# SafeRL-Lab/Massive-MARL-Benchmark

Measured on AMD Instinct MI355X. Metric: env-steps/sec (whole node), TenAnt 4096 envs/GPU, PPO rollout, higher is better.
Workload: dtype f32 (policy-layer products: fp32 operands as 2 row-scaled fp16 planes (kept to 2^-22), 3 f16 MFMA products, fp32 accumulation; error vs float64 <= the exact-fp32 MFMA kernel's, see policy_layers_error_vs_f64); 1 GPU; TenAnt num_envs=4096 per GPU, PPO rollout: ActorCritic MLP [1024,1024,512]x2 (fp32) + fused sim step (dt 0.0166, 2 substeps) + RolloutStorage + GAE every 8 steps; envs_per_gpu=4096, global_envs=4096, parallelism=env-sharded x1, no data-path collective, hipgraph=True, refresh_in_graph=True, rollouts_per_graph=1, fused_act_and_bound_slots=True, obs_planes_from_step_kernel=True, policy_head_in_step_kernel=True, critic_stream=True, critic_deferred=False, finite=True, resets_total=97569

## Files before the change

include/mms.h:

```cpp
#ifndef MMS_H
#define MMS_H

#include <stdint.h>

#ifdef __cplusplus
extern "C" {
#endif

#define MMS_ABI_VERSION 4
#define MMS_DR_FLOATS 33

enum mms_task { MMS_TASK_TEN_ANT = 0, MMS_TASK_ONE_ANT = 1, MMS_TASK_MULTI_INGENUITY = 2,
                MMS_TASK_MULTI_ANT_CIRCLE = 3 };
enum mms_dtype { MMS_F32 = 0, MMS_I64 = 1, MMS_I32 = 2, MMS_U8 = 3 };

typedef struct mms_model {
    float torso_mass, torso_ixx, torso_izz, torso_radius;
    float leg_mass, leg_ia, leg_it;
    float foot_mass, foot_ia, foot_it;
    float limb_radius, leg_len, foot_len;
    float hip_pos[4][3];
    float limb_dir[4][3];
    float ankle_axis[4][3];
    float dof_lower[8], dof_upper[8], dof_init[8], gear[8];
// ... 25 lines not shown
    float dt;
    float clip_actions, clip_obs;
    float dof_vel_scale, contact_force_scale, power_scale;
    float heading_weight, up_weight, actions_cost, energy_cost, joints_at_limit_cost;
    float death_cost, termination_height;
    float quat_reward_scale, ant_dist_reward_scale, goal_dist_reward_scale;
    float ant_start_x, ant_start_z;
    float box_start[3];
    mms_model model;
} mms_config;

typedef struct mms_tensor {
    void*   ptr;
    int64_t shape[4];
    int32_t ndim;
    int32_t dtype;
    int32_t device;
    int32_t reserved;
} mms_tensor;

typedef struct mms_engine* mms_handle;

int mms_create(const mms_config* cfg, mms_handle* out);
int mms_destroy(mms_handle h);

int mms_get_tensor(mms_handle h, const char* name, mms_tensor* out);

int mms_step(mms_handle h, void* hip_stream);

int mms_post_step(mms_handle h, void* hip_stream);

int mms_reset_all(mms_handle h, void* hip_stream);

int mms_set_state(mms_handle h, const char* name, const void* src, int src_is_host,
                  const int64_t* env_ids, int64_t n, void* hip_stream);

int mms_bind_obs_out(mms_handle h, void* dst);

int mms_bind_obs_planes16(mms_handle h, void* planes, float scale);

int mms_bind_actions(mms_handle h, const float* src);

int mms_set_dr(mms_handle h, int32_t enable);

int mms_set_obs_outputs(mms_handle h, int32_t raw, int32_t clipped);

int mms_bind_rollout_out(mms_handle h, float* rew_out, uint8_t* done_out);

int mms_marl_views(int device, const float* obs_clipped, float* obs_all, int64_t n, int32_t agents,
                   int32_t per_agent, int32_t shared, void* hip_stream);

int mms_gae_ppo(int device, const float* rewards, const uint8_t* dones, const float* values,
                const float* last_values, float* returns, float* advantages, double* stats,
                int32_t T, int64_t N, float gamma, float lam, void* hip_stream);
int mms_adv_normalize(int device, float* advantages, const double* stats, int64_t count, void* hip_stream);
#define MMS_GAE_STATS_DOUBLES (3 + 2 * 2048)
int mms_gae_ppo_normalized(int device, const float* rewards, const uint8_t* dones, const float* values, const float* last_values,
                           float* returns, float* advantages, double* stats, int32_t T, int64_t N, float gamma, float lam,
                           void* hip_stream);

int mms_layer_clock_probe(int device, uint64_t* out, int32_t slots);

int mms_gae_marl(int device, const float* rewards, const float* value_preds, const float* masks,
                 float* returns, int32_t T, int64_t N, float gamma, float lam,
                 int32_t use_norm, const float* norm_mean, const float* norm_var, void* hip_stream);

int mms_gae_marl_agents(int device, const float* rewards, const float* value_preds, const float* masks,
                        float* returns, int32_t T, int64_t N, int32_t A, float gamma, float lam,
                        int32_t use_norm, const float* norm_mean, const float* norm_var, void* hip_stream);

int mms_ppo_act(int device, const float* mean, const float* value, const float* log_std, uint64_t seed, int64_t* counters,
                int64_t row_offset, int32_t reference_scale, float* actions_out, float* act_slot, float* logp_slot,
                float* value_slot, float* mu_slot, float* sigma_slot, int64_t N, int32_t A, void* hip_stream);

int mms_ppo_heads_act(int device, const float* hidden, const float* weight, const float* bias, int32_t H, const float* value,
                      const float* vhidden, const float* vweight, const float* vbias, int32_t VH, const float* log_std, uint64_t seed,
                      int64_t* counters, int64_t row_offset, int32_t reference_scale, float* actions_out, float* act_slot,
                      float* logp_slot, float* value_slot, float* mu_slot, float* sigma_slot, int64_t N, int32_t A, void* hip_stream);

typedef struct mms_policy_head {
    const float* hidden; const float* weight; const float* bias;
    const float* vhidden; const float* vweight; const float* vbias;
    const float* log_std;
    int64_t* counters;
    float* actions_out; float* act_slot; float* logp_slot; float* value_slot; float* mu_slot; float* sigma_slot;
    uint64_t seed;
    int64_t row_offset;
    int32_t H, VH, A, reference_scale;
    const float* weight_tiles;
} mms_policy_head;
int mms_bind_policy_head(mms_handle h, const mms_policy_head* head);

int mms_sac_heads_act(int device, const float* hidden, int32_t H,
                      const float* mu_weight, const float* mu_bias, const float* ls_weight, const float* ls_bias,
                      float act_limit, float epsilon, int32_t deterministic,
                      uint64_t seed, int64_t* counters, int64_t row_offset,
                      float* actions_out, float* act_slot, float* logp_slot,
                      float* u_slot, float* mu_slot, float* log_std_slot,
                      int64_t N, int32_t A, void* hip_stream);

#define MMS_Q_MAX_H 4096
int mms_q_heads_backup(int device, int64_t M, int32_t H,
                       const float* h0, const float* w0, const float* b0, float* q0_out,
                       const float* h1, const float* w1, const float* b1, float* q1_out,
                       const float* reward, const uint8_t* done, const float* logp, float gamma, float alpha,
                       float* backup, void* hip_stream);

int mms_linear2_act(int device, int64_t M, int32_t N, int32_t K, const float* x0, const float* w0, const float* b0, float* y0,
                    const float* x1, const float* w1, const float* b1, float* y1, int32_t act, void* hip_stream);

#define MMS_MAX_GROUPS 32

int mms_linear_group_act(int device, int32_t groups, int64_t M, int32_t N, int32_t K, const float* const* x, const float* const* w,
                         const float* const* b, float* const* y, int32_t act, const float* const* ln_s, const float* const* ln_stat_in,
                         float* const* ln_part_out, void* hip_stream);

int mms_row_stats_group(int device, int32_t groups, int64_t M, int32_t slots, int32_t width, const float* const* part, float* const* stat,
                        float eps, void* hip_stream);

int mms_row_moments_group(int device, int32_t groups, int64_t M, int32_t K, int32_t x_pitch, const float* const* x, float* const* stat,
                          float eps, void* hip_stream);

int mms_layernorm_group(int device, int32_t groups, int64_t M, int32_t K, int32_t Kp, int32_t x_pitch, const float* const* x,
                        const float* const* gamma, const float* const* beta, float* const* y, float eps, void* hip_stream);

int mms_marl_heads_act(int device, int32_t groups, int64_t M, int32_t H, const float* const* h, const float* const* gamma,
                       const float* const* beta, const float* const* w, const float* const* b, const int32_t* A, const float* const* std,
                       float* const* out, float* const* logp, const int32_t* out_pitch, int64_t* const* counters, uint64_t seed,
                       int64_t row_offset, float eps, void* hip_stream);

#define MMS_P32_BYTES(rows, K) ((size_t)(rows) * (size_t)(((K) + 31) / 32) * 192)

int mms_split_planes(int device, int64_t rows, int32_t K, int32_t x_pitch, const float* x, void* planes, void* hip_stream);

int mms_split_planes_group(int device, int32_t groups, int64_t rows, int32_t K, int32_t x_pitch, const float* const* x, void* const* planes,
                           void* hip_stream);

int mms_linear_group_act_split(int device, int32_t groups, int64_t M, int32_t N, int32_t K, const void* const* x, const void* const* w,
                               const float* const* b, void* const* y, int32_t act, int32_t out_mode, const float* const* ln_s,
                               const float* const* ln_stat_in, float* const* ln_part_out, const float* const* head_w, float* const* head_part,
                               const int32_t* head_dims, void* hip_stream);

#define MMS_H32_BYTES(rows, K) ((size_t)(rows) * (size_t)(((K) + 31) / 32) * 128)

int mms_split_planes16_group(int device, int32_t groups, int64_t rows, int32_t K, int32_t x_pitch, const float* const* x, void* const* planes,
                             float* const* scale, float* const* inv, int32_t nchains, int32_t L, const float* const* chain,
                             float* const* chain_scale, float* const* chain_inv, float* const* stat, float eps, void* hip_stream);

int mms_weight_planes16_group(int device, int32_t groups, const int64_t* N, const int32_t* K, const float* const* w, void* const* planes,
                              float* const* scale, float* const* inv, float* const* l1, void* hip_stream);
int mms_chain_refresh16(int device, int32_t nchains, int32_t L, const float* const* l1, const float* const* bias, const int32_t* n,
                        float* chain, float bound0, int64_t rows, float* chain_scale, float* chain_inv, void* hip_stream);

int mms_linear_group_act_split16(int device, int32_t groups, int64_t M, int32_t N, int32_t K, const void* const* x, const void* const* w,
                                 const float* const* b, void* const* y, const float* const* x_inv, const float* const* w_inv,
                                 const float* const* y_scale, int32_t act, int32_t out_mode, const float* const* ln_s,
                                 const float* const* ln_stat_in, float* const* ln_part_out, const float* const* head_w, float* const* head_part,
                                 const int32_t* head_dims, void* hip_stream);

int mms_fold_planes16_group(int device, int32_t groups, const int64_t* N, const int32_t* K, const float* const* w, const float* const* gamma,
                            const float* const* beta, const float* const* bias, void* const* planes, float* const* inv, float* const* s,
                            float* const* c, float* const* rb, float* const* wt, void* hip_stream);
int mms_fold_scales16_group(int device, int32_t groups, const float* const* rb, const int32_t* n, int64_t M, float* const* scale1,
                            float* const* ysc, float* const* yinv, void* hip_stream);

int mms_row_stats_chan_group(int device, int32_t groups, int64_t M, int32_t slots, const float* const* part, float* const* stat, float eps,
                             void* hip_stream);

int mms_marl_heads_finish(int device, int32_t groups, int64_t M, int32_t slots, const float* const* part, const float* const* head_part,
                          const float* const* hs, const float* const* hc, const int32_t* A, const float* const* std, float* const* out,
                          float* const* logp, const int32_t* out_pitch, int64_t* const* counters, uint64_t seed, int64_t row_offset, float eps,
                          void* hip_stream);

int mms_mlp_grad(int device, int32_t layers, int64_t M, const int32_t* dims, const float* x, const float* const* h, const float* const* w,
                 const float* g, float* const* dw, float* const* db, float* const* d_out, float* const* e_out, void* workspace,
                 int64_t* ws_bytes, void* hip_stream);

int mms_mlp_grad_rop(int device, int32_t layers, int64_t M, const int32_t* dims, const float* x, const float* const* h, const float* const* w,
                     const float* const* v, const float* const* c, const float* g, const float* const* d, const float* const* e, float* rmu,
                     float* const* rdw, float* const* rdb, void* workspace, int64_t* ws_bytes, void* hip_stream);

const char* mms_last_error(mms_handle h);
int mms_abi_version(void);

#ifdef __cplusplus
}
#endif
#endif
```

massive_marl_benchmark_amd/_lib.py:

```python
import ctypes
import os

from .model import MmsConfig, MmsTensor

_HERE = os.path.dirname(os.path.abspath(__file__))
LIB_PATH = os.environ.get("MMS_LIB", os.path.join(_HERE, "lib", "libmms.so"))
LIB_CPU_PATH = os.path.join(_HERE, "lib", "libmms_cpu.so")
_lib = None
_lib_cpu = None

SYMBOLS = ["mms_create", "mms_destroy", "mms_get_tensor", "mms_step", "mms_post_step", "mms_reset_all", "mms_set_state",
           "mms_bind_obs_out", "mms_bind_obs_planes16", "mms_bind_actions", "mms_bind_policy_head", "mms_set_dr", "mms_set_obs_outputs", "mms_bind_rollout_out", "mms_ppo_act", "mms_ppo_heads_act", "mms_sac_heads_act", "mms_q_heads_backup", "mms_linear2_act", "mms_linear_group_act", "mms_split_planes", "mms_split_planes_group", "mms_linear_group_act_split", "mms_split_planes16_group", "mms_weight_planes16_group", "mms_chain_refresh16", "mms_fold_planes16_group", "mms_fold_scales16_group", "mms_linear_group_act_split16", "mms_row_stats_chan_group", "mms_marl_heads_finish", "mms_row_stats_group", "mms_row_moments_group", "mms_layernorm_group", "mms_marl_heads_act", "mms_marl_views", "mms_gae_ppo", "mms_adv_normalize", "mms_gae_ppo_normalized", "mms_layer_clock_probe", "mms_gae_marl", "mms_gae_marl_agents", "mms_mlp_grad", "mms_mlp_grad_rop",
           "mms_last_error", "mms_abi_version"]


class MmsError(RuntimeError):
    pass


def _bind(path):
    L = ctypes.CDLL(path)
    vp, ci, c64, cf = ctypes.c_void_p, ctypes.c_int, ctypes.c_int64, ctypes.c_float
    L.mms_create.argtypes = [ctypes.POINTER(MmsConfig), ctypes.POINTER(vp)]
    L.mms_destroy.argtypes = [vp]
    L.mms_get_tensor.argtypes = [vp, ctypes.c_char_p, ctypes.POINTER(MmsTensor)]
    L.mms_step.argtypes = [vp, vp]
    L.mms_post_step.argtypes = [vp, vp]
    L.mms_reset_all.argtypes = [vp, vp]
    L.mms_set_state.argtypes = [vp, ctypes.c_char_p, vp, ci, ctypes.POINTER(c64), c64, vp]
    L.mms_bind_obs_out.argtypes = [vp, vp]
    L.mms_bind_actions.argtypes = [vp, vp]
    L.mms_bind_policy_head.argtypes = [vp, vp]
    L.mms_bind_obs_planes16.argtypes = [vp, vp, cf]
    L.mms_set_obs_outputs.argtypes = [vp, ctypes.c_int32, ctypes.c_int32]
    L.mms_set_dr.argtypes = [vp, ctypes.c_int32]
    L.mms_bind_rollout_out.argtypes = [vp, vp, vp]
    L.mms_ppo_act.argtypes = [ci, vp, vp, vp, ctypes.c_uint64, vp, c64, ctypes.c_int32, vp, vp, vp, vp, vp, vp, c64, ctypes.c_int32, vp]
    L.mms_ppo_heads_act.argtypes = [ci, vp, vp, vp, ctypes.c_int32, vp, vp, vp, vp, ctypes.c_int32, vp, ctypes.c_uint64, vp, c64, ctypes.c_int32, vp, vp, vp, vp,
                                    vp, vp, c64, ctypes.c_int32, vp]
    L.mms_sac_heads_act.argtypes = [ci, vp, ctypes.c_int32, vp, vp, vp, vp, cf, cf, ctypes.c_int32, ctypes.c_uint64, vp, c64, vp, vp, vp, vp, vp, vp,
                                    c64, ctypes.c_int32, vp]
    L.mms_q_heads_backup.argtypes = [ci, c64, ctypes.c_int32, vp, vp, vp, vp, vp, vp, vp, vp, vp, vp, vp, cf, cf, vp, vp]
    L.mms_linear2_act.argtypes = [ci, c64, ctypes.c_int32, ctypes.c_int32, vp, vp, vp, vp, vp, vp, vp, vp, ctypes.c_int32, vp]
    L.mms_linear_group_act.argtypes = [ci, ctypes.c_int32, c64, ctypes.c_int32, ctypes.c_int32, vp, vp, vp, vp, ctypes.c_int32, vp, vp, vp, vp]
    L.mms_split_planes.argtypes = [ci, c64, ctypes.c_int32, ctypes.c_int32, vp, vp, vp]
    L.mms_split_planes_group.argtypes = [ci, ctypes.c_int32, c64, ctypes.c_int32, ctypes.c_int32, vp, vp, vp]
    L.mms_linear_group_act_split.argtypes = [ci, ctypes.c_int32, c64, ctypes.c_int32, ctypes.c_int32, vp, vp, vp, vp, ctypes.c_int32, ctypes.c_int32,
                                             vp, vp, vp, vp, vp, vp, vp]
    L.mms_split_planes16_group.argtypes = [ci, ctypes.c_int32, c64, ctypes.c_int32, ctypes.c_int32, vp, vp, vp, vp, ctypes.c_int32, ctypes.c_int32, vp, vp, vp, vp, cf, vp]
    L.mms_weight_planes16_group.argtypes = [ci, ctypes.c_int32, vp, vp, vp, vp, vp, vp, vp, vp]
    L.mms_fold_planes16_group.argtypes = [ci, ctypes.c_int32, vp, vp, vp, vp, vp, vp, vp, vp, vp, vp, vp, vp, vp]
    L.mms_fold_scales16_group.argtypes = [ci, ctypes.c_int32, vp, vp, c64, vp, vp, vp, vp]
    L.mms_chain_refresh16.argtypes = [ci, ctypes.c_int32, ctypes.c_int32, vp, vp, vp, vp, cf, c64, vp, vp, vp]
    L.mms_linear_group_act_split16.argtypes = [ci, ctypes.c_int32, c64, ctypes.c_int32, ctypes.c_int32, vp, vp, vp, vp, vp, vp, vp, ctypes.c_int32, ctypes.c_int32,
                                               vp, vp, vp, vp, vp, vp, vp]
    L.mms_row_stats_chan_group.argtypes = [ci, ctypes.c_int32, c64, ctypes.c_int32, vp, vp, cf, vp]
    L.mms_marl_heads_finish.argtypes = [ci, ctypes.c_int32, c64, ctypes.c_int32, vp, vp, vp, vp, vp, vp, vp, vp, vp, vp, ctypes.c_uint64, c64, cf, vp]
    L.mms_row_moments_group.argtypes = [ci, ctypes.c_int32, c64, ctypes.c_int32, ctypes.c_int32, vp, vp, cf, vp]
    L.mms_row_stats_group.argtypes = [ci, ctypes.c_int32, c64, ctypes.c_int32, ctypes.c_int32, vp, vp, cf, vp]
    L.mms_layernorm_group.argtypes = [ci, ctypes.c_int32, c64, ctypes.c_int32, ctypes.c_int32, ctypes.c_int32, vp, vp, vp, vp, cf, vp]
    L.mms_marl_heads_act.argtypes = [ci, ctypes.c_int32, c64, ctypes.c_int32, vp, vp, vp, vp, vp, vp, vp, vp, vp, vp, vp, ctypes.c_uint64, c64, cf, vp]
    L.mms_marl_views.argtypes = [ci, vp, vp, c64, ctypes.c_int32, ctypes.c_int32, ctypes.c_int32, vp]
    L.mms_gae_ppo.argtypes = [ci, vp, vp, vp, vp, vp, vp, vp, ctypes.c_int32, c64, cf, cf, vp]
    L.mms_adv_normalize.argtypes = [ci, vp, vp, c64, vp]
    L.mms_gae_ppo_normalized.argtypes = [ci, vp, vp, vp, vp, vp, vp, vp, ctypes.c_int32, c64, cf, cf, vp]
    L.mms_layer_clock_probe.argtypes = [ci, vp, ctypes.c_int32]
    L.mms_gae_marl.argtypes = [ci, vp, vp, vp, vp, ctypes.c_int32, c64, cf, cf, ctypes.c_int32, vp, vp, vp]
    L.mms_gae_marl_agents.argtypes = [ci, vp, vp, vp, vp, ctypes.c_int32, c64, ctypes.c_int32, cf, cf, ctypes.c_int32, vp, vp, vp]
    L.mms_mlp_grad.argtypes = [ci, ctypes.c_int32, c64, vp, vp, vp, vp, vp, vp, vp, vp, vp, vp, ctypes.POINTER(c64), vp]
    L.mms_mlp_grad_rop.argtypes = [ci, ctypes.c_int32, c64, vp, vp, vp, vp, vp, vp, vp, vp, vp, vp, vp, vp, vp, ctypes.POINTER(c64), vp]
    L.mms_last_error.argtypes = [vp]
    L.mms_last_error.restype = ctypes.c_char_p
    L.mms_abi_version.restype = ci
    return L


def lib():
    global _lib
    if _lib is not None:
        return _lib
    if not os.path.exists(LIB_PATH):
        raise MmsError("HIP engine library not built: %s is missing (run `python -c 'import __graft_entry__ as g; g.build()'` "
                       "or `make -C massive_marl_benchmark_amd/csrc`). There is no CPU fallback." % LIB_PATH)
    _lib = _bind(LIB_PATH)
    return _lib


def lib_cpu():
    global _lib_cpu
    if _lib_cpu is not None:
        return _lib_cpu
    if not os.path.exists(LIB_CPU_PATH):
        raise MmsError("CPU engine library not built: %s is missing (make -C massive_marl_benchmark_amd/csrc)" % LIB_CPU_PATH)
    _lib_cpu = _bind(LIB_CPU_PATH)
    return _lib_cpu


def for_device(device):
    import torch
    dev = torch.device(device)
    if dev.type == "cpu":
        return lib_cpu(), -1, None
    if dev.type != "cuda":
        raise MmsError("unsupported device %r" % (device,))
    idx = dev.index if dev.index is not None else torch.cuda.current_device()
    return lib(), idx, ctypes.c_void_p(torch.cuda.current_stream(dev).cuda_stream)


def last_error(handle=None, L=None):
    msg = (L or lib()).mms_last_error(handle)
    return msg.decode() if msg else ""


def check(rc, handle=None, what="", L=None):
    if rc != 0:
        raise MmsError("%s failed: %s" % (what, last_error(handle, L)))
```

massive_marl_benchmark_amd/algorithms/rl/ppo/module.py:

```python
import ctypes
import math

import numpy as np
import torch
import torch.nn as nn

from .... import _lib


def get_activation(act_name):
    table = {"elu": nn.ELU, "selu": nn.SELU, "relu": nn.ReLU, "crelu": nn.ReLU, "lrelu": nn.LeakyReLU, "tanh": nn.Tanh,
             "sigmoid": nn.Sigmoid}
    if act_name not in table:
        print("invalid activation function!")
        return None
    return table[act_name]()


def _mlp(in_dim, hidden, out_dim, activation):
    layers, d = [], in_dim
    for h in hidden:
        layers += [nn.Linear(d, h), activation]
        d = h
    layers.append(nn.Linear(d, out_dim))
    return nn.Sequential(*layers)


class ActorCritic(nn.Module):
    def __init__(self, obs_shape, states_shape, actions_shape, initial_std, model_cfg, asymmetric=False, seed=0, row_offset=0):
        super().__init__()
        self.asymmetric = asymmetric
        if model_cfg is None:
            actor_hidden, critic_hidden, activation = [256, 256, 256], [256, 256, 256], get_activation("selu")
        else:
            actor_hidden, critic_hidden = model_cfg["pi_hid_sizes"], model_cfg["vf_hid_sizes"]
            activation = get_activation(model_cfg["activation"])
        self.actor = _mlp(obs_shape[0], actor_hidden, actions_shape[0], activation)
        self.critic = _mlp(states_shape[0] if asymmetric else obs_shape[0], critic_hidden, 1, activation)
        self.log_std = nn.Parameter(np.log(initial_std) * torch.ones(*actions_shape))
        self.init_weights(self.actor, [np.sqrt(2)] * len(actor_hidden) + [0.01])
        self.init_weights(self.critic, [np.sqrt(2)] * len(critic_hidden) + [1.0])
        self.seed, self.row_offset = int(seed), int(row_offset)
        self._counters = None
        self._bound = None
        self._side = None
        self._trunk = None
        self._act_bufs = None
        self._value_bufs = None
        self._one_bufs = None
        self._wplanes = None
        self._split_bufs = None
        self._nets = None
        self._h16 = None
        self._addr_tag = None
        self._ver_tag = None
        self._calls = None
        self._sample_calls = None
        self._qualify = None
        self._step_engine = None
        self._head_wt = None

    _DERIVED = ("_counters", "_side", "_trunk", "_act_bufs", "_value_bufs", "_one_bufs", "_wplanes", "_split_bufs", "_nets", "_h16", "_addr_tag",
                "_ver_tag", "_calls", "_sample_calls", "_qualify", "_bound", "_step_engine", "_head_wt")

    def __deepcopy__(self, memo):
        import copy
        new = self.__class__.__new__(self.__class__)
        memo[id(self)] = new
        for k, v in self.__dict__.items():
            new.__dict__[k] = None if k in self._DERIVED else copy.deepcopy(v, memo)
        return new

    @staticmethod
    def init_weights(sequential, scales):
        for idx, module in enumerate(m for m in sequential if isinstance(m, nn.Linear)):
            torch.nn.init.orthogonal_(module.weight, gain=scales[idx])

    fuse_layers = True
    split_layers = True
    split_min_tiles = None
    split_format = "f16x2"
    fuse_head = True
    two_streams = True
    defer_value = False

    def forward(self):
        raise NotImplementedError

    def bind_rollout(self, storage=None, actions_out=None, step_engine=None):
        self._bound = (storage, actions_out)
        self._step_engine = step_engine if (storage is not None and step_engine is not None and step_engine.takes_policy_head()) else None

    def _fp32_layers_qualify(self):
        dt = self.log_std.dtype
        if self._qualify is not None and self._qualify[0] == dt:
            return self._qualify[1]
        a_lin = [m for m in self.actor if isinstance(m, nn.Linear)]
        c_lin = [m for m in self.critic if isinstance(m, nn.Linear)]
        acts = [m for m in list(self.actor) + list(self.critic) if not isinstance(m, nn.Linear)]
        ok = (len(a_lin) == len(c_lin) and len(a_lin) >= 2 and all(isinstance(m, nn.ELU) and m.alpha == 1.0 for m in acts)
              and all(la.weight.shape == lc.weight.shape and la.weight.dtype == torch.float32 and la.in_features % 4 == 0
                      and la.bias is not None and lc.bias is not None for la, lc in zip(a_lin[:-1], c_lin[:-1])))
        self._qualify = (dt, ok)
        return ok

    @staticmethod
    def _p32_bytes(rows, K):
        return rows * ((K + 31) // 32) * 192

    def _weight_planes(self, lin, L, idx, stream, force=False):
        if self._wplanes is None:
            self._wplanes = {}
        w = lin.weight.detach()
        tag = (w._version, w.data_ptr(), str(w.device))
        hit = self._wplanes.get(id(lin))
        if force or hit is None or hit[0] != tag:
            planes = hit[1] if hit is not None and hit[1].device == w.device else \
                torch.empty(self._p32_bytes(lin.out_features, lin.in_features), dtype=torch.uint8, device=w.device)
            wc = w.contiguous()
            _lib.check(L.mms_split_planes(idx, lin.out_features, lin.in_features, 0, ctypes.c_void_p(wc.data_ptr()),
                                          ctypes.c_void_p(planes.data_ptr()), stream), None, "mms_split_planes", L)
            self._wplanes[id(lin)] = (tag, planes, lin)
            return planes
        return hit[1]

    @staticmethod
    def _h32_bytes(rows, K):
        return rows * ((K + 31) // 32) * 128

    def _networks(self):
        if self._nets is None:
            self._nets = [[m for m in net if isinstance(m, nn.Linear)][:-1] for net in (self.actor, self.critic)]
        return self._nets

    def _param_tags(self):
        ps = [q for net in self._networks() for l in net for q in (l.weight, l.bias) if q is not None]
        ps += [q for q in (self.actor[-1].weight, self.actor[-1].bias, self.critic[-1].weight, self.critic[-1].bias, self.log_std) if q is not None]
        return tuple(q._version for q in ps), tuple(q.data_ptr() for q in ps)

    def _h16_state(self, dev):
        st = self._h16
        if st is not None and st["dev"] == dev:
            return st
        L, idx, _ = _lib.for_device(dev)
        nets = self._networks()
        recs, off, slices = [], 0, []
        for net in nets:
            rs = []
            for l in net:
                assert l.weight.dtype == torch.float32 and l.weight.is_contiguous() and l.bias is not None and l.weight.device == dev
                N, K = l.out_features, l.in_features
                rs.append({"lin": l, "N": N, "K": K, "planes": torch.empty(self._h32_bytes(N, K), dtype=torch.uint8, device=dev),
                           "scale": torch.empty(N, device=dev), "inv": torch.empty(N, device=dev), "l1": torch.empty(N, device=dev)})
            recs.append(rs)
            slices.append((off, max(len(net) - 1, 0)))
            off += 2 * max(len(net) - 1, 0)
        bounds = torch.zeros(max(off, 2), device=dev)
        arr = lambda ts: (ctypes.c_void_p * len(ts))(*[t.data_ptr() for t in ts])
        flat = [r for rs in recs for r in rs]
        calls = []
        if flat:
            calls.append((L.mms_weight_planes16_group, (idx, len(flat), (ctypes.c_int64 * len(flat))(*[r["N"] for r in flat]),
                                                        (ctypes.c_int32 * len(flat))(*[r["K"] for r in flat]), arr([r["lin"].weight for r in flat]),
                                                        arr([r["planes"] for r in flat]), arr([r["scale"] for r in flat]), arr([r["inv"] for r in flat]),
                                                        arr([r["l1"] for r in flat])), "mms_weight_planes16_group"))
        st = {"dev": dev, "L": L, "idx": idx, "recs": recs, "bounds": bounds, "slices": slices, "calls": calls, "given": {}, "chain_args": {}}
        self._h16 = st
        return st

    def _chain_args(self, st, members):
        members = tuple(members)
        hit = st["chain_args"].get(members)
        if hit is None:
            chain, Lh = self._chain(st, list(members))
            ent = [st["recs"][g][li] for g in members for li in range(Lh)]
            arr = lambda ts: (ctypes.c_void_p * len(ts))(*[t.data_ptr() for t in ts])
            hit = (len(members), Lh, arr([r["l1"] for r in ent]), arr([r["lin"].bias for r in ent]), (ctypes.c_int32 * len(ent))(*[r["N"] for r in ent]),
                   ctypes.c_void_p(chain.data_ptr())) if Lh else None
            st["chain_args"][members] = hit
        return hit

    def _chain(self, st, members):
        o0, Lh = st["slices"][members[0]]
        if Lh == 0:
            return None, 0
        for j, g in enumerate(members):
            assert st["slices"][g] == (o0 + 2 * Lh * j, Lh), "networks that share an input must be adjacent and equally deep"
        return st["bounds"][o0: o0 + 2 * Lh * len(members)], Lh

    def refresh(self):
        dev = self.log_std.device
        vers, addrs = self._param_tags()
        if self._addr_tag is not None and self._addr_tag != (addrs, str(dev)):
            self._h16, self._wplanes, self._split_bufs, self._calls, self._sample_calls = None, None, None, None, None
            self._head_wt = None
        self._addr_tag, self._ver_tag = (addrs, str(dev)), vers
        if self._head_wt is not None:
            self._fill_head_tiles()
        st = self._h16
        if st is not None:
            stream = _lib.for_device(st["dev"])[2]
            for fn, args, what in st["calls"]:
                _lib.check(fn(*args, stream), None, what, st["L"])
            covered = set()
            for (members, rows, scale), (_, cs, ci, alias) in st["given"].items():
                ca = self._chain_args(st, members)
                if ca is None or alias:
                    continue
                _lib.check(st["L"].mms_chain_refresh16(st["idx"], *ca, 16384.0 / scale, rows, ctypes.c_void_p(cs.data_ptr()), ctypes.c_void_p(ci.data_ptr()), stream),
                           None, "mms_chain_refresh16", st["L"])
                covered.update(members)
            depths = {Lh for _, Lh in st["slices"]}
            rest = [tuple(range(len(st["recs"])))] if len(depths) == 1 else [(g,) for g in range(len(st["recs"]))]
            for grp in rest:
                if not set(grp) <= covered:
                    ca = self._chain_args(st, grp)
                    if ca is not None:
                        _lib.check(st["L"].mms_chain_refresh16(st["idx"], *ca, 0.0, 0, None, None, stream), None, "mms_chain_refresh16", st["L"])
        if self._wplanes:
            for key in list(self._wplanes):
                tag, planes, lin = self._wplanes[key]
                if self.split_format == "bf16x3":
                    self._weight_planes(lin, *_lib.for_device(lin.weight.device), force=True)
                else:
                    self._wplanes[key] = (None, planes, lin)

    def _head_tiles(self):
        if self._head_wt is None:
            last = self.actor[-1]
            A, H = last.out_features, last.in_features
            nct = (A + 15) // 16
            pad = torch.zeros(nct * 16, H, device=last.weight.device, dtype=torch.float32)
            tiles = torch.empty(nct * (H // 4) * 64, device=last.weight.device, dtype=torch.float32)
            self._head_wt = (pad, tiles)
            self._fill_head_tiles()
        return self._head_wt[1]

    def _fill_head_tiles(self):
        pad, tiles = self._head_wt
        last = self.actor[-1]
        A, H = last.out_features, last.in_features
        with torch.no_grad():
            if A % 16 == 0:
                tiles.view(-1, H // 4, 16, 4).copy_(last.weight.detach().view(-1, 16, H // 4, 4).permute(0, 2, 1, 3))
            else:
                pad[:A].copy_(last.weight.detach())
                tiles.view(-1, H // 4, 16, 4).copy_(pad.view(-1, 16, H // 4, 4).permute(0, 2, 1, 3))

    def _ensure_fresh(self):
        storage = self._bound[0] if self._bound is not None else None
        if storage is not None and storage.step == 0:
            return self.refresh()
        vers, addrs = self._param_tags()
        if self._ver_tag != vers or self._addr_tag != (addrs, str(self.log_std.device)):
            self.refresh()

    def _split_hidden16(self, nets, inputs, tag, planes=None):
        self._ensure_fresh()
        x0 = inputs[0]
        dev, M = x0.device, x0.shape[0]
        mine = self._networks()
        members = [next(j for j, n in enumerate(mine) if n and n[0] is net[0]) for net in nets]
        fresh = self._h16 is None or self._h16["dev"] != dev
        st = self._h16_state(dev)
        if fresh:
            self.refresh()
        G, nl = len(nets), len(nets[0])
        given = planes is not None and all(x.data_ptr() == x0.data_ptr() and x.shape == x0.shape for x in inputs)
        ckey = (tag, "h", M, tuple((x.data_ptr(), x.shape[1], x.stride(0)) for x in inputs), tuple(members),
                (planes[0].data_ptr(), float(planes[1])) if given else None)
        if self._calls is None:
            self._calls = {}
        hit = self._calls.get(ckey)
        if hit is None:
            hit = self._build_calls16(st, members, inputs, tag, planes if given else None)
            self._calls[ckey] = hit
        calls, out = hit
        stream = _lib.for_device(dev)[2]
        for fn, args, what in calls:
            _lib.check(fn(*args, stream), None, what, st["L"])
        return out

    def _build_calls16(self, st, members, inputs, tag, planes):
        x0 = inputs[0]
        dev, M = x0.device, x0.shape[0]
        L, idx = st["L"], st["idx"]
        recs = [st["recs"][g] for g in members]
        G, nl = len(recs), len(recs[0])
        key = (tag, "h", M, tuple(x.shape[1] for x in inputs), str(dev), tuple(members))
        if self._split_bufs is None:
            self._split_bufs = {}
        bufs = self._split_bufs.get(key)
        f32 = lambda *sh: torch.empty(*sh, device=dev)
        u8 = lambda n: torch.empty(n, dtype=torch.uint8, device=dev)
        if bufs is None:
            bufs = {"x": [u8(self._h32_bytes(M, x.shape[1])) for x in inputs], "xs": [f32(M) for _ in range(G)], "xi": [f32(M) for _ in range(G)],
                    "cs": [f32(G, max(nl - 1, 1), M) for _ in range(G)], "ci": [f32(G, max(nl - 1, 1), M) for _ in range(G)],
                    "h": [[u8(self._h32_bytes(M, r["N"])) for _ in range(G)] for r in recs[0][:-1]],
                    "out": [f32(M, recs[0][-1]["N"]) for _ in range(G)], "keep": []}
            self._split_bufs[key] = bufs
        arr = lambda ts: (ctypes.c_void_p * len(ts))(*[t.data_ptr() for t in ts])
        src, users = [], []
        for g, x in enumerate(inputs):
            same = next((h for h in range(g) if inputs[h].data_ptr() == x.data_ptr() and inputs[h].shape == x.shape), None)
            if same is None:
                users.append([g])
                src.append((g, 0))
            else:
                first = src[same][0]
                grp = next(u for u in users if u[0] == first)
                src.append((first, len(grp)))
                grp.append(g)
        calls = []
        x_planes = {}
        for grp in users:
            g0 = grp[0]
            x = inputs[g0]
            assert x.dtype == torch.float32 and x.stride(1) == 1
            chain, Lh = self._chain(st, [members[g] for g in grp])
            nch = len(grp) if Lh else 0
            if planes is not None:
                pl, scale = planes
                scale = float(scale)
                assert pl.dtype == torch.uint8 and pl.numel() == self._h32_bytes(M, x.shape[1]) and pl.device == dev
                gm = tuple(members[g] for g in grp)
                gkey = (gm, M, scale)
                if gkey not in st["given"]:
                    host = next(((k, v) for k, v in st["given"].items() if k[1:] == (M, scale) and not v[3] and
                                 any(k[0][j:j + len(gm)] == gm for j in range(len(k[0]) - len(gm) + 1))), None)
                    if host is not None and nch:
                        j = next(j for j in range(len(host[0][0]) - len(gm) + 1) if host[0][0][j:j + len(gm)] == gm)
                        st["given"][gkey] = (host[1][0], host[1][1][j:j + len(gm)], host[1][2][j:j + len(gm)], True)
                    else:
                        xi = torch.full((M,), 1.0 / scale, device=dev)
                        cs, ci = f32(max(nch, 1), max(Lh, 1), M), f32(max(nch, 1), max(Lh, 1), M)
                        st["given"][gkey] = (xi, cs, ci, False)
                        if nch:
                            _lib.check(L.mms_chain_refresh16(idx, *self._chain_args(st, gm), 16384.0 / scale, M, ctypes.c_void_p(cs.data_ptr()),
                                                             ctypes.c_void_p(ci.data_ptr()), _lib.for_device(dev)[2]), None, "mms_chain_refresh16", L)
                xi, cs, ci, _ = st["given"][gkey]
                x_planes[g0] = (pl, xi, cs, ci)
                bufs["keep"].append(pl)
                continue
            x_planes[g0] = (bufs["x"][g0], bufs["xi"][g0], bufs["cs"][g0], bufs["ci"][g0])
            calls.append((L.mms_split_planes16_group, (idx, 1, M, x.shape[1], x.stride(0), arr([x]), arr([bufs["x"][g0]]), arr([bufs["xs"][g0]]), arr([bufs["xi"][g0]]),
                                                       nch, Lh if nch else 0, arr([chain]) if nch else None, arr([bufs["cs"][g0]]) if nch else None,
                                                       arr([bufs["ci"][g0]]) if nch else None, None, 0.0), "mms_split_planes16_group"))
            bufs["keep"].append(x)
        cur = [x_planes[src[g][0]][0] for g in range(G)]
        cur_inv = [x_planes[src[g][0]][1] for g in range(G)]
        for li in range(nl):
            last = li == nl - 1
            out = bufs["out"] if last else bufs["h"][li]
            ysc = None if last else arr([x_planes[src[g][0]][2][src[g][1], li] for g in range(G)])
            calls.append((L.mms_linear_group_act_split16, (idx, G, M, recs[0][li]["N"], recs[0][li]["K"], arr(cur), arr([recs[g][li]["planes"] for g in range(G)]),
                                                           arr([recs[g][li]["lin"].bias for g in range(G)]), arr(out), arr(cur_inv),
                                                           arr([recs[g][li]["inv"] for g in range(G)]), ysc, 1, 0 if last else 1, None, None, None, None, None, 0),
                          "mms_linear_group_act_split16"))
            if not last:
                cur, cur_inv = out, [x_planes[src[g][0]][3][src[g][1], li] for g in range(G)]
        return calls, bufs["out"]

    def _split_applies(self, M, lins, networks=2):
        if not (self.split_layers and M > 0 and M % 128 == 0 and all(l.out_features % 128 == 0 for l in lins)):
            return False
        need = self.split_min_tiles
        if need is None:
            dev = lins[0].weight.device
            need = torch.cuda.get_device_properties(dev).multi_processor_count if dev.type == "cuda" else 1
        return max(networks * (M // 128) * (l.out_features // 128) for l in lins) >= need

    def _split_hidden(self, nets, inputs, tag, planes=None):
        if self.split_format == "f16x2":
            return self._split_hidden16(nets, inputs, tag, planes)
        assert self.split_format == "bf16x3", self.split_format
        self._ensure_fresh()
        x0 = inputs[0]
        dev, M, K = x0.device, x0.shape[0], x0.shape[1]
# ... 236 lines not shown
```

massive_marl_benchmark_amd/csrc/cpu/mms_cpu.cpp:

```cpp
#include <math.h>
#include <stdio.h>
#include <stdlib.h>
#include <string.h>

#include <string>
#include <vector>

#include "../mms_host.h"
#include "../rollout_lane.h"
#include "../q_lane.h"
#include "../sac_lane.h"
#include "lane_step.h"

#define MMS_API extern "C" __attribute__((visibility("default")))

struct mms_engine : mms_host_state {};

template <typename T> static T* buf(mms_engine* e, const char* name) { return (T*)find(e, name)->ptr; }

MMS_API int mms_abi_version(void) { return MMS_ABI_VERSION; }
MMS_API const char* mms_last_error(mms_handle h) { return h ? h->err.c_str() : g_error.c_str(); }

MMS_API int mms_destroy(mms_handle h) {
    if (!h) return 0;
// ... 398 lines not shown
    if (refused(check_split_layer(false, groups, M, N, K, x, w, b, y, nullptr, nullptr, nullptr, act, out_mode, ln_s, ln_stat_in, ln_part_out, head_w, head_part, head_dims))) return 1;
    const bool ln = ln_s != nullptr;
    const int KC = (K + 31) / 32, NC = N / 32;
    for (int g = 0; g < groups; g++) {
        const uint16_t* xp = (const uint16_t*)x[g];
        const uint16_t* wp = (const uint16_t*)w[g];
        std::vector<float> wf((size_t)N * KC * 32);
        for (int64_t n = 0; n < N; n++)
            for (int k = 0; k < KC * 32; k++) wf[n * KC * 32 + k] = join3(wp + (n * KC + k / 32) * 96, k % 32);
        void* yg = out_mode != 2 ? y[g] : nullptr;
        split_layer_rows(M, N, KC, wf, b[g], act, out_mode, ln ? ln_s[g] : nullptr, ln ? ln_stat_in[g] : nullptr, ln ? ln_part_out[g] : nullptr,
                         out_mode == 2 ? head_w[g] : nullptr, out_mode == 2 ? head_part[g] : nullptr, out_mode == 2 ? head_dims[g] : 0,
                         [&](int64_t m, float* xr) { for (int k = 0; k < KC * 32; k++) xr[k] = join3(xp + (m * KC + k / 32) * 96, k % 32); },
                         [](int64_t, int) { return 1.f; },
                         [&](int64_t m, const float* row) {
                             if (out_mode == 1) {
                                 for (int n = 0; n < N; n++) {
                                     uint16_t* c = (uint16_t*)yg + (m * NC + n / 32) * 96 + n % 32;
                                     split3(row[n], c, c + 32, c + 64);
                                 }
                             } else {
                                 memcpy((float*)yg + m * N, row, (size_t)N * 4);
                             }
                         });
    }
    return 0;
}

using mms::f2h;
using mms::h2f;
static inline void pow2_scale(float bound, float& scale, float& inv) {
    int e = 14;
    if (bound > 0.f) (void)frexpf(bound, &e);
    int sh = 14 - e;
    sh = sh > 100 ? 100 : (sh < -100 ? -100 : sh);
    scale = ldexpf(1.f, sh);
    inv = ldexpf(1.f, -sh);
}
static inline void split2(float t, uint16_t* hi, uint16_t* lo) {
    *hi = f2h(t);
    *lo = f2h((t - h2f(*hi)) * 2048.f);
}
static inline float join2(const uint16_t* chunk, int j) { return h2f(chunk[j]) + h2f(chunk[32 + j]) * (1.f / 2048.f); }

static void split_planes16_rows(int32_t groups, int64_t rows, int32_t K, int32_t x_pitch, const float* const* x, void* const* planes, float* const* scale,
                                float* const* inv, int32_t nchains, int32_t L, const float* const* chain, float* const* chain_scale,
                                float* const* chain_inv, float* const* stat, float eps) {
    const int KC = (K + 31) / 32;
    for (int g = 0; g < groups; g++) {
        uint16_t* out = (uint16_t*)planes[g];
        const float* xg = x[g];
#pragma omp parallel for schedule(static)
        for (int64_t r = 0; r < rows; r++) {
            float big = 0.f;
            for (int k = 0; k < K; k++) big = fmaxf(big, fabsf(xg[r * x_pitch + k]));
            float sc, iv;
            pow2_scale(big, sc, iv);
            for (int kc = 0; kc < KC; kc++) {
                uint16_t* c = out + (r * KC + kc) * 64;
                for (int j = 0; j < 32; j++) {
                    const int k = kc * 32 + j;
                    split2(k < K ? xg[r * x_pitch + k] * sc : 0.f, c + j, c + 32 + j);
                }
            }
            if (scale[g]) scale[g][r] = sc;
            if (inv[g]) inv[g][r] = iv;
            if (stat) {
                float sum = 0.f, m2 = 0.f;
                for (int k = 0; k < K; k++) sum += xg[r * x_pitch + k];
                const float mean = sum / (float)K;
                for (int k = 0; k < K; k++) m2 += (xg[r * x_pitch + k] - mean) * (xg[r * x_pitch + k] - mean);
                stat[g][2 * r] = mean;
                stat[g][2 * r + 1] = 1.0f / sqrtf(m2 / (float)K + eps);
            }
            for (int c = 0; c < nchains; c++) {
                float bound = big;
                for (int l = 0; l < L; l++) {
                    bound = (chain[g][((size_t)c * L + l) * 2] * bound + chain[g][((size_t)c * L + l) * 2 + 1]) * 1.001f;
                    float s2, i2;
                    pow2_scale(bound, s2, i2);
                    chain_scale[g][((size_t)c * L + l) * rows + r] = s2;
                    chain_inv[g][((size_t)c * L + l) * rows + r] = i2;
                }
            }
        }
    }
}

MMS_API int mms_split_planes16_group(int device, int32_t groups, int64_t rows, int32_t K, int32_t x_pitch, const float* const* x, void* const* planes,
                                     float* const* scale, float* const* inv, int32_t nchains, int32_t L, const float* const* chain,
                                     float* const* chain_scale, float* const* chain_inv, float* const* stat, float eps, void*) {
    if (cpu_only(device)) return 1;
    if (x_pitch == 0) x_pitch = K;
    if (refused(check_split_planes16_group(groups, rows, K, x_pitch, x, planes, scale, inv, nchains, L, chain, chain_scale, chain_inv, stat))) return 1;
    split_planes16_rows(groups, rows, K, x_pitch, x, planes, scale, inv, nchains, L, chain, chain_scale, chain_inv, stat, eps);
    return 0;
}

MMS_API int mms_weight_planes16_group(int device, int32_t groups, const int64_t* N, const int32_t* K, const float* const* w, void* const* planes,
                                      float* const* scale, float* const* inv, float* const* l1, void*) {
    if (cpu_only(device)) return 1;
    if (refused(check_weight_planes16_group(groups, N, K, w, planes, scale, inv))) return 1;
    for (int g = 0; g < groups; g++) {
        if (N[g] == 0) continue;
        split_planes16_rows(1, N[g], K[g], K[g], w + g, planes + g, scale + g, inv + g, 0, 0, nullptr, nullptr, nullptr, nullptr, 0.f);
        if (!l1 || !l1[g]) continue;
        const int Kg = K[g], KC = (Kg + 31) / 32, pieces = KC * 4;
        int P = 1;
        while (P < pieces && P < 64) P <<= 1;
#pragma omp parallel for schedule(static)
        for (int64_t r = 0; r < N[g]; r++) {
            float lane[64];
            for (int sub = 0; sub < P; sub++) {
                float a = 0.f;
                for (int p = sub; p < pieces; p += P)
                    for (int j = 0; j < 8; j++) { const int k = p * 8 + j; a += (k < Kg) ? fabsf(w[g][r * Kg + k]) : 0.f; }
                lane[sub] = a;
            }
            for (int m = P >> 1; m >= 1; m >>= 1) {
                float nxt[64];
                for (int i = 0; i < P; i++) nxt[i] = lane[i] + lane[i ^ m];
                for (int i = 0; i < P; i++) lane[i] = nxt[i];
            }
            l1[g][r] = lane[0];
        }
    }
    return 0;
}

MMS_API int mms_chain_refresh16(int device, int32_t nchains, int32_t L, const float* const* l1, const float* const* bias, const int32_t* n, float* chain,
                                float bound0, int64_t rows, float* chain_scale, float* chain_inv, void*) {
    if (cpu_only(device)) return 1;
    if (refused(check_chain_refresh16(nchains, L, l1, n, chain, bound0, rows, chain_scale, chain_inv))) return 1;
    for (int e = 0; e < nchains * L; e++) {
        float m = 0.f, b = 0.f;
        for (int i = 0; i < n[e]; i++) {
            m = fmaxf(m, l1[e][i]);
            if (bias && bias[e]) b = fmaxf(b, fabsf(bias[e][i]));
        }
        chain[2 * e] = m;
        chain[2 * e + 1] = b;
    }
    for (int c = 0; c < nchains && rows > 0; c++) {
        float bound = bound0;
        for (int l = 0; l < L; l++) {
            bound = (chain[((size_t)c * L + l) * 2] * bound + chain[((size_t)c * L + l) * 2 + 1]) * 1.001f;
            float sc, iv;
            pow2_scale(bound, sc, iv);
            for (int64_t r = 0; r < rows; r++) {
                chain_scale[((size_t)c * L + l) * rows + r] = sc;
                chain_inv[((size_t)c * L + l) * rows + r] = iv;
            }
        }
    }
    return 0;
}

MMS_API int mms_fold_planes16_group(int device, int32_t groups, const int64_t* N, const int32_t* K, const float* const* w, const float* const* gamma,
                                    const float* const* beta, const float* const* bias, void* const* planes, float* const* inv, float* const* s_out,
                                    float* const* c_out, float* const* rb, float* const* wt, void*) {
    if (cpu_only(device)) return 1;
    if (refused(check_fold_planes16_group(groups, N, K, w, planes, inv))) return 1;
    for (int g = 0; g < groups; g++) {
        const int Kg = K[g], KC = (Kg + 31) / 32;
        const float* gm = gamma ? gamma[g] : nullptr;
        const float* bt = beta ? beta[g] : nullptr;
        uint16_t* out = planes ? (uint16_t*)planes[g] : nullptr;
#pragma omp parallel for schedule(static)
        for (int64_t r = 0; r < N[g]; r++) {
            const float* wr = w[g] + r * Kg;
            float big = 0.f, s = 0.f, c = 0.f, l2 = 0.f;
            for (int k = 0; k < Kg; k++) {
                const float v = gm ? wr[k] * gm[k] : wr[k];
                big = fmaxf(big, fabsf(v));
                s += v;
                l2 += v * v;
                if (bt) c += wr[k] * bt[k];
            }
            if (bias && bias[g]) c += bias[g][r];
            float sc, iv;
            pow2_scale(big, sc, iv);
            for (int kc = 0; kc < KC && out; kc++) {
                uint16_t* ch = out + (r * KC + kc) * 64;
                for (int j = 0; j < 32; j++) {
                    const int k = kc * 32 + j;
                    split2(k < Kg ? (gm ? wr[k] * gm[k] : wr[k]) * sc : 0.f, ch + j, ch + 32 + j);
                }
            }
            if (wt && wt[g])
                for (int k = 0; k < Kg; k++) wt[g][r * Kg + k] = gm ? wr[k] * gm[k] : wr[k];
            if (inv && inv[g]) inv[g][r] = iv;
            if (s_out && s_out[g]) s_out[g][r] = s;
            if (c_out && c_out[g]) c_out[g][r] = c;
            if (rb && rb[g]) rb[g][r] = sqrtf(l2) * sqrtf((float)Kg) + fabsf(c);
        }
    }
    return 0;
}

MMS_API int mms_fold_scales16_group(int device, int32_t groups, const float* const* rb, const int32_t* n, int64_t M, float* const* scale1,
                                    float* const* ysc, float* const* yinv, void*) {
    if (cpu_only(device)) return 1;
    if (refused(check_fold_scales16_group(groups, rb, n, M))) return 1;
    for (int g = 0; g < groups; g++) {
        float m = 0.f;
        for (int i = 0; i < n[g]; i++) m = fmaxf(m, rb[g][i]);
        float bound = m * 1.001f;
        if (!(bound > 1e-30f)) bound = 1e-30f;
        float sc, iv;
        pow2_scale(bound, sc, iv);
        if (scale1 && scale1[g]) scale1[g][0] = sc;
        for (int64_t r = 0; r < M; r++) {
            if (ysc && ysc[g]) ysc[g][r] = sc;
            if (yinv && yinv[g]) yinv[g][r] = iv;
        }
    }
    return 0;
}

MMS_API int mms_linear_group_act_split16(int device, int32_t groups, int64_t M, int32_t N, int32_t K, const void* const* x, const void* const* w,
                                         const float* const* b, void* const* y, const float* const* x_inv, const float* const* w_inv,
                                         const float* const* y_scale, int32_t act, int32_t out_mode, const float* const* ln_s,
                                         const float* const* ln_stat_in, float* const* ln_part_out, const float* const* head_w, float* const* head_part,
                                         const int32_t* head_dims, void*) {
    if (cpu_only(device)) return 1;
    if (refused(check_split_layer(true, groups, M, N, K, x, w, b, y, x_inv, w_inv, y_scale, act, out_mode, ln_s, ln_stat_in, ln_part_out, head_w, head_part, head_dims))) return 1;
    const bool ln = ln_s != nullptr;
    const int KC = (K + 31) / 32, NC = N / 32;
    for (int g = 0; g < groups; g++) {
        const uint16_t* xp = (const uint16_t*)x[g];
        const uint16_t* wp = (const uint16_t*)w[g];
        std::vector<float> wf((size_t)N * KC * 32);
        for (int64_t n = 0; n < N; n++)
            for (int k = 0; k < KC * 32; k++) wf[n * KC * 32 + k] = join2(wp + (n * KC + k / 32) * 64, k % 32);
        void* yg = out_mode != 2 ? y[g] : nullptr;
        const float* xi = x_inv[g];
        const float* wi = w_inv[g];
        const float* ys = out_mode == 1 ? y_scale[g] : nullptr;
        split_layer_rows(M, N, KC, wf, b[g], act, out_mode, ln ? ln_s[g] : nullptr, ln ? ln_stat_in[g] : nullptr, ln ? ln_part_out[g] : nullptr,
                         out_mode == 2 ? head_w[g] : nullptr, out_mode == 2 ? head_part[g] : nullptr, out_mode == 2 ? head_dims[g] : 0,
                         [&](int64_t m, float* xr) { for (int k = 0; k < KC * 32; k++) xr[k] = join2(xp + (m * KC + k / 32) * 64, k % 32); },
                         [&](int64_t m, int n) { return wi[n] * xi[m]; },
                         [&](int64_t m, const float* row) {
                             if (out_mode == 1) {
                                 for (int n = 0; n < N; n++) {
                                     uint16_t* c = (uint16_t*)yg + (m * NC + n / 32) * 64 + n % 32;
                                     split2(row[n] * ys[m], c, c + 32);
                                 }
                             } else {
                                 memcpy((float*)yg + m * N, row, (size_t)N * 4);
                             }
                         });
    }
    return 0;
}

static void chan_combine(const float* part, int64_t M, int64_t row, int slots, float& mean, float& m2) {
    float sum = 0.f;
    for (int k = 0; k < slots; k++) sum += part[((size_t)k * M + row) * 2];
    mean = sum / (64.f * (float)slots);
    m2 = 0.f;
    for (int k = 0; k < slots; k++) {
        const float d = part[((size_t)k * M + row) * 2] * (1.f / 64.f) - mean;
        m2 += part[((size_t)k * M + row) * 2 + 1] + 64.f * d * d;
    }
}

MMS_API int mms_row_stats_chan_group(int device, int32_t groups, int64_t M, int32_t slots, const float* const* part, float* const* stat, float eps, void*) {
    if (cpu_only(device)) return 1;
    if (refused(check_row_stats_chan_group(groups, M, slots, part, stat))) return 1;
    for (int g = 0; g < groups; g++) {
        for (int64_t r = 0; r < M; r++) {
            float mean, m2;
            chan_combine(part[g], M, r, slots, mean, m2);
            stat[g][2 * r] = mean;
            stat[g][2 * r + 1] = 1.0f / sqrtf(m2 / (64.f * (float)slots) + eps);
        }
    }
    return 0;
}

MMS_API int mms_marl_heads_finish(int device, int32_t groups, int64_t M, int32_t slots, const float* const* part, const float* const* head_part,
                                  const float* const* hs, const float* const* hc, const int32_t* A, const float* const* std, float* const* out,
                                  float* const* logp, const int32_t* out_pitch, int64_t* const* counters, uint64_t seed, int64_t row_offset, float eps, void*) {
    if (cpu_only(device)) return 1;
    if (refused(check_marl_heads_finish(groups, M, slots, part, head_part, hs, hc, A, out, out_pitch))) return 1;
    for (int g = 0; g < groups; g++) {
        const int pitch = out_pitch ? out_pitch[g] : A[g];
        const float* sd = std ? std[g] : nullptr;
        int64_t* cnt = (sd && counters) ? counters[g] : nullptr;
        for (int64_t r = 0; r < M; r++) {
            float mean, m2;
            chan_combine(part[g], M, r, slots, mean, m2);
            const float rstd = 1.0f / sqrtf(m2 / (64.f * (float)slots) + eps);
            const int64_t c = cnt ? cnt[r] : 0;
            for (int j = 0; j < A[g]; j++) {
                float dot = 0.f;
                for (int k = 0; k < slots; k++) dot += head_part[g][((size_t)k * M + r) * ((A[g] + 3) & ~3) + j];
                const float mu = rstd * (dot - mean * hs[g][j]) + hc[g][j];
                if (!sd) { out[g][r * pitch + j] = mu; continue; }
                const float z = mms::rand_normal(seed + (uint64_t)g, (uint64_t)(row_offset + r), (uint64_t)c, (uint32_t)j);
                out[g][r * pitch + j] = mu + sd[j] * z;
                if (logp && logp[g]) logp[g][r * pitch + j] = -0.5f * z * z - logf(sd[j]) - 0.9189385332046727f;
            }
            if (cnt) cnt[r] = c + 1;
        }
// ... 234 lines not shown
```

massive_marl_benchmark_amd/csrc/head_block.h:

```cpp
#pragma once
#include <hip/hip_runtime.h>
#ifndef MMS_HEAD_STAMP
#define MMS_HEAD_STAMP 0
#endif
#include <stdint.h>

#include "mms_lane.h"
#include "rollout_lane.h"

namespace mms {

struct PpoActOut {
    float* actions_out; float* act_slot; float* logp_slot; float* value_slot; float* mu_slot; float* sigma_slot;
    float* lds_actions = nullptr;
    int64_t lds_row0 = 0;
};
__device__ __forceinline__ void ppo_sample_row(const float* mean_row, const float* __restrict__ value, const float* __restrict__ log_std,
                                               uint64_t seed, int64_t* __restrict__ counters, int64_t row_offset, int ref_scale,
                                               const PpoActOut& o, int64_t row, int A, int lane, bool have_value = false, float value_now = 0.f) {
    const int64_t c = counters[row];
    float lp = 0.f;
    for (int j = lane; j < A; j += 64) {
        const float ls = log_std[j];
        const float m = mean_row[j];
        float term;
        const float act = ppo_sample_one(m, ls, seed, (uint64_t)(row_offset + row), (uint64_t)c, (uint32_t)j, ref_scale, term);
        lp += term;
        if (o.actions_out) o.actions_out[row * A + j] = act;
        if (o.lds_actions) o.lds_actions[(row - o.lds_row0) * A + j] = act;
        if (o.act_slot) o.act_slot[row * A + j] = act;
        if (o.mu_slot) o.mu_slot[row * A + j] = m;
        if (o.sigma_slot) o.sigma_slot[row * A + j] = ls;
    }
#pragma unroll
    for (int m = 32; m >= 1; m >>= 1) lp += __shfl_xor(lp, m, 64);
    if (lane == 0) {
        if (o.logp_slot) o.logp_slot[row] = lp;
        if (o.value_slot && (have_value || value)) o.value_slot[row] = have_value ? value_now : value[row];
        counters[row] = c + 1;
    }
}

typedef float f32x4 __attribute__((ext_vector_type(4)));

template <int NCT, int WAVES, int RT, int UB = 4, bool TILED = false>
__device__ __forceinline__ void ppo_head_block(float* s_part, const int tid, const bool active, const int64_t r0,
                                               const float* __restrict__ hidden, const float* __restrict__ weight,
                                               const float* __restrict__ bias, int H, const float* __restrict__ value,
                                               const float* __restrict__ vhidden, const float* __restrict__ vweight,
                                               const float* __restrict__ vbias, int VH,
                                               const float* __restrict__ log_std, uint64_t seed, int64_t* __restrict__ counters,
                                               int64_t row_offset, int ref_scale, const PpoActOut& o, int64_t N, int A,
                                               const float* __restrict__ weight_tiles = nullptr) {
    constexpr int AP = NCT * 16, ROWS = 16 * RT;
    constexpr int RPW = ROWS / WAVES;
#if MMS_HEAD_STAMP
    uint64_t st[6];
    st[0] = __builtin_amdgcn_s_memrealtime();
#define MMS_HEAD_ST(i) do { asm volatile("s_waitcnt vmcnt(0) lgkmcnt(0)" ::: "memory"); st[i] = __builtin_amdgcn_s_memrealtime(); } while (0)
#else
#define MMS_HEAD_ST(i) do { } while (0)
#endif
    const int lane = tid & 63, wave = active ? (tid >> 6) : 0;
    const int i = lane & 15, g = lane >> 4;
    float v_rows[RPW];
#pragma unroll
    for (int q = 0; q < RPW; q++) v_rows[q] = 0.f;
    if (active) {
        const float* hrow[RT];
#pragma unroll
        for (int rt = 0; rt < RT; rt++) {
            const int64_t row_a = r0 + 16 * rt + i < N ? r0 + 16 * rt + i : N - 1;
            hrow[rt] = hidden + row_a * (int64_t)H + 4 * g;
        }
        const float* wrow[NCT];
#pragma unroll
        for (int ct = 0; ct < NCT; ct++) {
            const int j = ct * 16 + i;
            wrow[ct] = weight + (int64_t)(j < A ? j : A - 1) * H + 4 * g;
        }
        f32x4 acc[RT][NCT];
#pragma unroll
        for (int rt = 0; rt < RT; rt++)
#pragma unroll
            for (int ct = 0; ct < NCT; ct++) acc[rt][ct] = f32x4{0.f, 0.f, 0.f, 0.f};
#pragma unroll
        for (int q = 0; q < RPW; q++) {
            const int64_t row = r0 + wave * RPW + q;
            if (vhidden && row < N) {
                const float* hv = vhidden + row * (int64_t)VH;
                float part = 0.f;
                for (int k = lane * 4; k < VH; k += 256) {
                    const float4 h4 = *reinterpret_cast<const float4*>(hv + k), w4 = *reinterpret_cast<const float4*>(vweight + k);
                    part += h4.x * w4.x + h4.y * w4.y + h4.z * w4.z + h4.w * w4.w;
                }
#pragma unroll
                for (int m = 32; m >= 1; m >>= 1) part += __shfl_xor(part, m, 64);
                v_rows[q] = part + vbias[0];
            }
        }
        MMS_HEAD_ST(1);
        const int kq = H / WAVES;
        const int kbeg = wave * kq;
        for (int kc = kbeg; kc < kbeg + kq; kc += 64) {
#pragma unroll
            for (int u0 = 0; u0 < 4; u0 += UB) {
                float4 a[RT][UB], b[UB][NCT];
#pragma unroll
                for (int u = 0; u < UB; u++) {
#pragma unroll
                    for (int rt = 0; rt < RT; rt++) a[rt][u] = *reinterpret_cast<const float4*>(hrow[rt] + kc + 16 * (u0 + u));
#pragma unroll
                    for (int ct = 0; ct < NCT; ct++)
                        b[u][ct] = TILED ? *reinterpret_cast<const float4*>(weight_tiles + ((size_t)(ct * (H / 4) + (kc / 4 + 4 * (u0 + u) + g)) * 16 + i) * 4)
                                         : *reinterpret_cast<const float4*>(wrow[ct] + kc + 16 * (u0 + u));
                }
#pragma unroll
                for (int rt = 0; rt < RT; rt++)
#pragma unroll
                    for (int u = 0; u < UB; u++) {
#pragma unroll
                        for (int ct = 0; ct < NCT; ct++) acc[rt][ct] = __builtin_amdgcn_mfma_f32_16x16x4f32(a[rt][u].x, b[u][ct].x, acc[rt][ct], 0, 0, 0);
#pragma unroll
                        for (int ct = 0; ct < NCT; ct++) acc[rt][ct] = __builtin_amdgcn_mfma_f32_16x16x4f32(a[rt][u].y, b[u][ct].y, acc[rt][ct], 0, 0, 0);
#pragma unroll
                        for (int ct = 0; ct < NCT; ct++) acc[rt][ct] = __builtin_amdgcn_mfma_f32_16x16x4f32(a[rt][u].z, b[u][ct].z, acc[rt][ct], 0, 0, 0);
#pragma unroll
                        for (int ct = 0; ct < NCT; ct++) acc[rt][ct] = __builtin_amdgcn_mfma_f32_16x16x4f32(a[rt][u].w, b[u][ct].w, acc[rt][ct], 0, 0, 0);
                    }
            }
        }
        MMS_HEAD_ST(2);
        float* mine = s_part + (size_t)wave * ROWS * AP;
#pragma unroll
        for (int rt = 0; rt < RT; rt++)
#pragma unroll
            for (int ct = 0; ct < NCT; ct++) {
#pragma unroll
                for (int r = 0; r < 4; r++) mine[(16 * rt + 4 * g + r) * AP + ct * 16 + i] = acc[rt][ct][r];
            }
    }
    __syncthreads();
    MMS_HEAD_ST(3);
    float* s_mean = s_part + (size_t)WAVES * ROWS * AP;
    if (active)
        for (int e = tid; e < ROWS * AP; e += 64 * WAVES) {
            const int j = e % AP;
            float sum = s_part[e];
#pragma unroll
            for (int w = 1; w < WAVES; w++) sum += s_part[w * ROWS * AP + e];
            s_mean[e] = sum + bias[j < A ? j : 0];
        }
    __syncthreads();
    MMS_HEAD_ST(4);
    if (active) {
#pragma unroll
        for (int q = 0; q < RPW; q++) {
            const int r = wave * RPW + q;
            const int64_t row = r0 + r;
            if (row >= N) continue;
            ppo_sample_row(s_mean + r * AP, value, log_std, seed, counters, row_offset, ref_scale, o, row, A, lane, vhidden != nullptr, v_rows[q]);
        }
    }
#if MMS_HEAD_STAMP
    MMS_HEAD_ST(5);
    if (r0 == 0 && tid == 0 && o.sigma_slot)
        for (int i = 1; i < 6; i++) o.sigma_slot[i] = 0.01f * (float)(st[i] - st[0]);
#endif
}

}
```

massive_marl_benchmark_amd/csrc/mms_api.hip:

```cpp
#include <hip/hip_runtime.h>
#include <stdio.h>
#include <stdlib.h>

#include "mms_host.h"
#include "policy_args.h"
#include "step_args.h"
#include "trpo_plan.h"

namespace mms {
hipError_t launch_step(const StepArgs& a, int task, hipStream_t stream);
bool step_layout_takes_head(int task, int num_envs, int num_agents, int packing);
hipError_t launch_gae_ppo(const float*, const uint8_t*, const float*, const float*, float*, float*, double*, int, int64_t, float, float, hipStream_t);
hipError_t launch_adv_normalize(float*, const double*, int64_t, hipStream_t);
hipError_t launch_gae_ppo_normalized(const float*, const uint8_t*, const float*, const float*, float*, float*, double*, int, int64_t, float, float, hipStream_t);
hipError_t launch_gae_marl(const float*, const float*, const float*, float*, int, int64_t, float, float, int, const float*, const float*, hipStream_t);
hipError_t launch_marl_views(const float*, float*, int64_t, int, int, int, hipStream_t);
hipError_t launch_gae_marl_agents(const float*, const float*, const float*, float*, int, int64_t, int, float, float, int, const float*, const float*, hipStream_t);
hipError_t launch_ppo_act(const float*, const float*, const float*, uint64_t, int64_t*, int64_t, int, float*, float*, float*, float*, float*, float*, int64_t, int, hipStream_t);
hipError_t launch_ppo_head_act(const float*, const float*, const float*, int, const float*, const float*, const float*, const float*, int, const float*, uint64_t,
                               int64_t*, int64_t, int, float*, float*, float*, float*, float*, float*, int64_t, int, hipStream_t);
hipError_t launch_sac_head_act(const float*, int, const float*, const float*, const float*, const float*, float, float, int, uint64_t, int64_t*, int64_t,
                               float*, float*, float*, float*, float*, float*, int64_t, int, hipStream_t);
hipError_t launch_q_heads_backup(int, int64_t, int, const float* const*, const float* const*, const float* const*, float* const*, const float*,
                                 const uint8_t*, const float*, float, float, float*, hipStream_t);
// ... 251 lines not shown
    MMS_DEV(device)
    MMS_FREE(mms::launch_gae_marl_agents(rewards, value_preds, masks, returns, T, N, A, gamma, lam, use_norm, norm_mean, norm_var, (hipStream_t)s));
    return 0;
}

__attribute__((visibility("default"))) int mms_ppo_act(int device, const float* mean, const float* value, const float* log_std, uint64_t seed,
                                                       int64_t* counters, int64_t row_offset, int32_t reference_scale, float* actions_out,
                                                       float* act_slot, float* logp_slot, float* value_slot, float* mu_slot, float* sigma_slot,
                                                       int64_t N, int32_t A, void* s) {
    MMS_DEV(device)
    if (refused(check_ppo_act(mean, log_std, counters, N, A))) return 1;
    MMS_FREE(mms::launch_ppo_act(mean, value, log_std, seed, counters, row_offset, reference_scale, actions_out, act_slot, logp_slot, value_slot,
                                 mu_slot, sigma_slot, N, A, (hipStream_t)s));
    return 0;
}

__attribute__((visibility("default"))) int mms_ppo_heads_act(int device, const float* hidden, const float* weight, const float* bias, int32_t H,
                                                             const float* value, const float* vhidden, const float* vweight, const float* vbias,
                                                             int32_t VH, const float* log_std, uint64_t seed, int64_t* counters,
                                                             int64_t row_offset, int32_t reference_scale, float* actions_out, float* act_slot,
                                                             float* logp_slot, float* value_slot, float* mu_slot, float* sigma_slot, int64_t N,
                                                             int32_t A, void* s) {
    MMS_DEV(device)
    if (refused(check_ppo_heads_act(hidden, weight, bias, H, vhidden, vweight, vbias, VH, log_std, counters, N, A))) return 1;
    MMS_FREE(mms::launch_ppo_head_act(hidden, weight, bias, H, value, vhidden, vweight, vbias, VH, log_std, seed, counters, row_offset, reference_scale,
                                      actions_out, act_slot, logp_slot, value_slot, mu_slot, sigma_slot, N, A, (hipStream_t)s));
    return 0;
}

__attribute__((visibility("default"))) int mms_sac_heads_act(int device, const float* hidden, int32_t H, const float* mu_weight,
                                                             const float* mu_bias, const float* ls_weight, const float* ls_bias, float act_limit,
                                                             float epsilon, int32_t deterministic, uint64_t seed, int64_t* counters,
                                                             int64_t row_offset, float* actions_out, float* act_slot, float* logp_slot,
                                                             float* u_slot, float* mu_slot, float* log_std_slot, int64_t N, int32_t A, void* s) {
    MMS_DEV(device)
    if (refused(check_sac_heads_act(hidden, H, mu_weight, mu_bias, ls_weight, ls_bias, deterministic, counters, N, A))) return 1;
    MMS_FREE(mms::launch_sac_head_act(hidden, H, mu_weight, mu_bias, ls_weight, ls_bias, act_limit, epsilon, deterministic, seed, counters, row_offset,
                                      actions_out, act_slot, logp_slot, u_slot, mu_slot, log_std_slot, N, A, (hipStream_t)s));
    return 0;
}

__attribute__((visibility("default"))) int mms_q_heads_backup(int device, int64_t M, int32_t H, const float* h0, const float* w0, const float* b0,
                                                              float* q0_out, const float* h1, const float* w1, const float* b1, float* q1_out,
                                                              const float* reward, const uint8_t* done, const float* logp, float gamma,
                                                              float alpha, float* backup, void* s) {
    MMS_DEV(device)
    if (refused(check_q_heads_backup(M, H, h0, w0, b0, q0_out, h1, w1, b1, q1_out, reward, done, backup))) return 1;
    const float* h[2] = {h0, h1};
    const float* w[2] = {w0, w1};
    const float* b[2] = {b0, b1};
    float* q[2] = {q0_out, q1_out};
    MMS_FREE(mms::launch_q_heads_backup(h1 ? 2 : 1, M, H, h, w, b, q, reward, done, backup ? logp : nullptr, gamma, alpha, backup, (hipStream_t)s));
    return 0;
}

__attribute__((visibility("default"))) int mms_linear2_act(int device, int64_t M, int32_t N, int32_t K, const float* x0, const float* w0, const float* b0,
                                                           float* y0, const float* x1, const float* w1, const float* b1, float* y1, int32_t act,
                                                           void* s) {
    MMS_DEV(device)
    if (refused(check_linear2_act(M, N, K, x0, w0, b0, y0, x1, w1, b1, y1, act))) return 1;
    const bool two = x1 != nullptr;
    mms::LinearArgs a = {};
    a.x[0] = x0; a.x[1] = x1; a.w[0] = w0; a.w[1] = w1; a.b[0] = b0; a.b[1] = b1; a.y[0] = y0; a.y[1] = y1;
    a.M = (int)M; a.N = N; a.K = K; a.act = act;
    MMS_FREE(mms::launch_linear_act(a, two ? 2 : 1, (hipStream_t)s));
    return 0;
}

__attribute__((visibility("default"))) int mms_split_planes(int device, int64_t rows, int32_t K, int32_t x_pitch, const float* x, void* planes, void* s) {
    MMS_DEV(device)
    if (x_pitch == 0) x_pitch = K;
    if (refused(check_split_planes(rows, K, x_pitch, x, planes))) return 1;
    MMS_FREE(mms::launch_split_planes(x, planes, rows, K, x_pitch, (hipStream_t)s));
    return 0;
}

__attribute__((visibility("default"))) int mms_split_planes_group(int device, int32_t groups, int64_t rows, int32_t K, int32_t x_pitch,
                                                                  const float* const* x, void* const* planes, void* s) {
    MMS_DEV(device)
    if (x_pitch == 0) x_pitch = K;
    if (refused(check_split_planes_group(groups, rows, K, x_pitch, x, planes))) return 1;
    mms::SplitPlanesArgs a = {};
    for (int g = 0; g < groups; g++) { a.x[g] = x[g]; a.planes[g] = planes[g]; }
    a.rows = rows; a.K = K; a.x_pitch = x_pitch;
    MMS_FREE(mms::launch_split_planes_group(a, groups, (hipStream_t)s));
    return 0;
}

__attribute__((visibility("default"))) int mms_linear_group_act_split(int device, int32_t groups, int64_t M, int32_t N, int32_t K, const void* const* x,
                                                                      const void* const* w, const float* const* b, void* const* y, int32_t act,
                                                                      int32_t out_mode, const float* const* ln_s, const float* const* ln_stat_in,
                                                                      float* const* ln_part_out, const float* const* head_w, float* const* head_part,
                                                                      const int32_t* head_dims, void* s) {
    MMS_DEV(device)
    if (refused(check_split_layer(false, groups, M, N, K, x, w, b, y, nullptr, nullptr, nullptr, act, out_mode, ln_s, ln_stat_in, ln_part_out, head_w, head_part, head_dims))) return 1;
    const bool ln = ln_s != nullptr;
    mms::SplitLinearArgs a = {};
    for (int g = 0; g < groups; g++) {
        a.x[g] = x[g]; a.w[g] = w[g]; a.b[g] = b[g]; a.y[g] = out_mode != 2 ? y[g] : nullptr;
        if (ln) { a.s[g] = ln_s[g]; a.stat_in[g] = ln_stat_in[g]; a.part_out[g] = ln_part_out[g]; }
        if (out_mode == 2) { a.head_w[g] = head_w[g]; a.head_part[g] = head_part[g]; a.hdims[g] = head_dims[g]; }
    }
    a.M = (int)M; a.N = N; a.KC = (K + 31) / 32; a.act = act; a.out_mode = out_mode;
    MMS_FREE(mms::launch_linear_split(a, groups, (hipStream_t)s));
    return 0;
}

__attribute__((visibility("default"))) int mms_split_planes16_group(int device, int32_t groups, int64_t rows, int32_t K, int32_t x_pitch,
                                                                    const float* const* x, void* const* planes, float* const* scale, float* const* inv,
                                                                    int32_t nchains, int32_t L, const float* const* chain, float* const* chain_scale,
                                                                    float* const* chain_inv, float* const* stat, float eps, void* s) {
    MMS_DEV(device)
    if (x_pitch == 0) x_pitch = K;
    if (refused(check_split_planes16_group(groups, rows, K, x_pitch, x, planes, scale, inv, nchains, L, chain, chain_scale, chain_inv, stat))) return 1;
    mms::Split16PlanesArgs a = {};
    for (int g = 0; g < groups; g++) {
        a.x[g] = x[g]; a.planes[g] = planes[g]; a.scale[g] = scale[g]; a.inv[g] = inv[g];
        if (nchains > 0) { a.chain[g] = chain[g]; a.chain_scale[g] = chain_scale[g]; a.chain_inv[g] = chain_inv[g]; }
        if (stat) a.stat[g] = stat[g];
    }
    a.rows = rows; a.K = K; a.x_pitch = x_pitch; a.nchains = nchains; a.L = nchains > 0 ? L : 0; a.eps = eps;
    MMS_FREE(mms::launch_split16_planes_group(a, groups, (hipStream_t)s));
    return 0;
}

__attribute__((visibility("default"))) int mms_weight_planes16_group(int device, int32_t groups, const int64_t* N, const int32_t* K, const float* const* w,
                                                                     void* const* planes, float* const* scale, float* const* inv,
                                                                     float* const* l1, void* s) {
    MMS_DEV(device)
    if (refused(check_weight_planes16_group(groups, N, K, w, planes, scale, inv))) return 1;
    mms::Split16PlanesArgs a = {};
    for (int g = 0; g < groups; g++) {
        a.x[g] = w[g]; a.planes[g] = planes[g]; a.scale[g] = scale[g]; a.inv[g] = inv[g];
        a.l1[g] = l1 ? l1[g] : nullptr;
        a.rows_g[g] = N[g]; a.K_g[g] = K[g];
    }
    a.per_group = 1;
    MMS_FREE(mms::launch_split16_planes_group(a, groups, (hipStream_t)s));
    return 0;
}

__attribute__((visibility("default"))) int mms_chain_refresh16(int device, int32_t nchains, int32_t L, const float* const* l1, const float* const* bias,
                                                               const int32_t* n, float* chain, float bound0, int64_t rows, float* chain_scale,
                                                               float* chain_inv, void* s) {
    MMS_DEV(device)
    if (refused(check_chain_refresh16(nchains, L, l1, n, chain, bound0, rows, chain_scale, chain_inv))) return 1;
    mms::ChainRefreshArgs a = {};
    for (int e = 0; e < nchains * L; e++) { a.l1[e] = l1[e]; a.bias[e] = bias ? bias[e] : nullptr; a.n[e] = n[e]; }
    a.chain = chain; a.nchains = nchains; a.L = L; a.bound0 = bound0; a.rows = rows; a.chain_scale = chain_scale; a.chain_inv = chain_inv;
    MMS_FREE(mms::launch_chain_refresh16(a, (hipStream_t)s));
    return 0;
}

__attribute__((visibility("default"))) int mms_fold_planes16_group(int device, int32_t groups, const int64_t* N, const int32_t* K, const float* const* w,
                                                                   const float* const* gamma, const float* const* beta, const float* const* bias,
                                                                   void* const* planes, float* const* inv, float* const* s_out, float* const* c_out,
                                                                   float* const* rb, float* const* wt, void* s) {
    MMS_DEV(device)
    if (refused(check_fold_planes16_group(groups, N, K, w, planes, inv))) return 1;
    mms::FoldPlanesArgs a = {};
    for (int g = 0; g < groups; g++) {
        a.w[g] = w[g];
        a.gamma[g] = gamma ? gamma[g] : nullptr; a.beta[g] = beta ? beta[g] : nullptr; a.bias[g] = bias ? bias[g] : nullptr;
        a.planes[g] = planes ? planes[g] : nullptr; a.inv[g] = inv ? inv[g] : nullptr;
        a.s[g] = s_out ? s_out[g] : nullptr; a.c[g] = c_out ? c_out[g] : nullptr; a.rb[g] = rb ? rb[g] : nullptr; a.wt[g] = wt ? wt[g] : nullptr;
        a.rows_g[g] = N[g]; a.K_g[g] = K[g];
    }
    MMS_FREE(mms::launch_fold_planes16(a, groups, (hipStream_t)s));
    return 0;
}

__attribute__((visibility("default"))) int mms_fold_scales16_group(int device, int32_t groups, const float* const* rb, const int32_t* n, int64_t M,
                                                                   float* const* scale1, float* const* ysc, float* const* yinv, void* s) {
    MMS_DEV(device)
    if (refused(check_fold_scales16_group(groups, rb, n, M))) return 1;
    mms::FoldScalesArgs a = {};
    for (int g = 0; g < groups; g++) {
        a.rb[g] = rb[g]; a.n[g] = n[g];
        a.scale1[g] = scale1 ? scale1[g] : nullptr; a.ysc[g] = ysc ? ysc[g] : nullptr; a.yinv[g] = yinv ? yinv[g] : nullptr;
    }
    a.M = M;
    MMS_FREE(mms::launch_fold_scales16(a, groups, (hipStream_t)s));
    return 0;
}

__attribute__((visibility("default"))) int mms_linear_group_act_split16(int device, int32_t groups, int64_t M, int32_t N, int32_t K, const void* const* x,
                                                                        const void* const* w, const float* const* b, void* const* y,
                                                                        const float* const* x_inv, const float* const* w_inv, const float* const* y_scale,
                                                                        int32_t act, int32_t out_mode, const float* const* ln_s,
                                                                        const float* const* ln_stat_in, float* const* ln_part_out,
                                                                        const float* const* head_w, float* const* head_part, const int32_t* head_dims, void* s) {
    MMS_DEV(device)
    if (refused(check_split_layer(true, groups, M, N, K, x, w, b, y, x_inv, w_inv, y_scale, act, out_mode, ln_s, ln_stat_in, ln_part_out, head_w, head_part, head_dims))) return 1;
    const bool ln = ln_s != nullptr;
    mms::Split16LinearArgs a = {};
    for (int g = 0; g < groups; g++) {
        a.x[g] = x[g]; a.w[g] = w[g]; a.b[g] = b[g]; a.y[g] = out_mode != 2 ? y[g] : nullptr;
        a.xinv[g] = x_inv[g]; a.winv[g] = w_inv[g]; a.yscale[g] = out_mode == 1 ? y_scale[g] : nullptr;
        if (ln) { a.s[g] = ln_s[g]; a.stat_in[g] = ln_stat_in[g]; a.part_out[g] = ln_part_out[g]; }
        if (out_mode == 2) { a.head_w[g] = head_w[g]; a.head_part[g] = head_part[g]; a.hdims[g] = head_dims[g]; }
    }
    a.M = (int)M; a.N = N; a.KC = (K + 31) / 32; a.act = act; a.out_mode = out_mode;
    MMS_FREE(mms::launch_linear_split16(a, groups, (hipStream_t)s));
    return 0;
}

__attribute__((visibility("default"))) int mms_layer_clock_probe(int device, uint64_t* out, int32_t slots) {
    (void)device;
    if (refused(check_layer_clock_probe(out, slots))) return 1;
    mms::set_split16_clock_probe(out, out ? slots : 0);
    return 0;
}

__attribute__((visibility("default"))) int mms_row_stats_chan_group(int device, int32_t groups, int64_t M, int32_t slots, const float* const* part,
                                                                    float* const* stat, float eps, void* s) {
    MMS_DEV(device)
    if (refused(check_row_stats_chan_group(groups, M, slots, part, stat))) return 1;
    mms::RowStatsArgs a = {};
    for (int g = 0; g < groups; g++) { a.part[g] = part[g]; a.stat[g] = stat[g]; }
    a.M = M; a.slots = slots; a.width = 64 * slots; a.eps = eps;
    MMS_FREE(mms::launch_row_stats_chan(a, groups, (hipStream_t)s));
    return 0;
}

__attribute__((visibility("default"))) int mms_marl_heads_finish(int device, int32_t groups, int64_t M, int32_t slots, const float* const* part,
                                                                 const float* const* head_part, const float* const* hs, const float* const* hc,
                                                                 const int32_t* A, const float* const* std, float* const* out, float* const* logp,
                                                                 const int32_t* out_pitch, int64_t* const* counters, uint64_t seed, int64_t row_offset,
                                                                 float eps, void* s) {
    MMS_DEV(device)
    if (refused(check_marl_heads_finish(groups, M, slots, part, head_part, hs, hc, A, out, out_pitch))) return 1;
    mms::HeadsFinishArgs a = {};
    for (int g = 0; g < groups; g++) {
        a.part[g] = part[g]; a.head_part[g] = head_part[g]; a.hs[g] = hs[g]; a.hc[g] = hc[g]; a.out[g] = out[g];
        a.std[g] = std ? std[g] : nullptr;
        a.logp[g] = logp ? logp[g] : nullptr;
        a.counters[g] = counters ? counters[g] : nullptr;
        a.A[g] = A[g];
        a.out_pitch[g] = out_pitch ? out_pitch[g] : A[g];
    }
    a.seed = seed; a.M = M; a.row_offset = row_offset; a.slots = slots; a.width = 64 * slots; a.eps = eps;
    MMS_FREE(mms::launch_marl_heads_finish(a, groups, (hipStream_t)s));
    return 0;
}

__attribute__((visibility("default"))) int mms_linear_group_act(int device, int32_t groups, int64_t M, int32_t N, int32_t K, const float* const* x,
                                                                const float* const* w, const float* const* b, float* const* y, int32_t act,
                                                                const float* const* ln_s, const float* const* ln_stat_in, float* const* ln_part_out,
                                                                void* s) {
    MMS_DEV(device)
    if (refused(check_linear_group_act(groups, M, N, K, x, w, b, y, act, ln_s, ln_stat_in, ln_part_out))) return 1;
    mms::LinearArgs a = {};
    for (int g = 0; g < groups; g++) {
        a.x[g] = x[g]; a.w[g] = w[g]; a.b[g] = b[g]; a.y[g] = y[g];
        if (ln_s) { a.s[g] = ln_s[g]; a.stat_in[g] = ln_stat_in[g]; }
        if (ln_part_out) a.part_out[g] = ln_part_out[g];
    }
    a.M = (int)M; a.N = N; a.K = K; a.act = act;
    MMS_FREE(mms::launch_linear_act(a, groups, (hipStream_t)s));
    return 0;
}

__attribute__((visibility("default"))) int mms_row_stats_group(int device, int32_t groups, int64_t M, int32_t slots, int32_t width, const float* const* part,
                                                               float* const* stat, float eps, void* s) {
    MMS_DEV(device)
    if (refused(check_row_stats_group(groups, M, slots, width, part, stat))) return 1;
    mms::RowStatsArgs a = {};
    for (int g = 0; g < groups; g++) { a.part[g] = part[g]; a.stat[g] = stat[g]; }
    a.M = M; a.slots = slots; a.width = width; a.eps = eps;
    MMS_FREE(mms::launch_row_stats(a, groups, (hipStream_t)s));
    return 0;
}

__attribute__((visibility("default"))) int mms_row_moments_group(int device, int32_t groups, int64_t M, int32_t K, int32_t x_pitch, const float* const* x,
                                                                 float* const* stat, float eps, void* s) {
    MMS_DEV(device)
    if (x_pitch == 0) x_pitch = K;
    if (refused(check_row_moments_group(groups, M, K, x_pitch, x, stat))) return 1;
    mms::LayerNormArgs a = {};
    for (int g = 0; g < groups; g++) { a.x[g] = x[g]; a.y[g] = stat[g]; }
    a.M = M; a.K = K; a.Kp = K; a.x_pitch = x_pitch; a.eps = eps; a.stats_only = 1;
    MMS_FREE(mms::launch_layernorm(a, groups, (hipStream_t)s));
    return 0;
}

__attribute__((visibility("default"))) int mms_layernorm_group(int device, int32_t groups, int64_t M, int32_t K, int32_t Kp, int32_t x_pitch,
                                                               const float* const* x, const float* const* gamma, const float* const* beta, float* const* y,
                                                               float eps, void* s) {
    MMS_DEV(device)
    if (x_pitch == 0) x_pitch = K;
    if (refused(check_layernorm_group(groups, M, K, Kp, x_pitch, x, gamma, beta, y))) return 1;
    mms::LayerNormArgs a = {};
    for (int g = 0; g < groups; g++) { a.x[g] = x[g]; a.gamma[g] = gamma[g]; a.beta[g] = beta[g]; a.y[g] = y[g]; }
    a.M = M; a.K = K; a.Kp = Kp; a.x_pitch = x_pitch; a.eps = eps;
    MMS_FREE(mms::launch_layernorm(a, groups, (hipStream_t)s));
    return 0;
}

__attribute__((visibility("default"))) int mms_marl_heads_act(int device, int32_t groups, int64_t M, int32_t H, const float* const* h,
                                                              const float* const* gamma, const float* const* beta, const float* const* w,
                                                              const float* const* b, const int32_t* A, const float* const* std, float* const* out,
                                                              float* const* logp, const int32_t* out_pitch, int64_t* const* counters, uint64_t seed,
                                                              int64_t row_offset, float eps, void* s) {
    MMS_DEV(device)
    if (refused(check_marl_heads_act(groups, M, H, h, gamma, beta, w, b, A, out, out_pitch))) return 1;
    mms::HeadsArgs a = {};
// ... 53 lines not shown
```

massive_marl_benchmark_amd/csrc/mms_host.h:

```cpp
#pragma once
#include <math.h>
#include <stdint.h>
#include <string.h>

#include <string>
#include <vector>

#include "../../include/mms.h"

namespace mms {
constexpr int kMlpMaxLayers = 8;
constexpr int64_t kMlpMaxRows = 65535 * 32 / 128 * 128;
}

struct mms_buffer {
    const char* name;
    void* ptr;
    int64_t shape[4];
    int ndim;
    int dtype;
    size_t bytes;
    int64_t row_bytes;
};

// ... 223 lines not shown
static inline int host_bind_rollout_out(mms_host_state* h, float* rew_out, uint8_t* done_out) {
    if (null_handle(h, "mms_bind_rollout_out")) return 1;
    h->rew_out = rew_out;
    h->done_out = done_out;
    return 0;
}


static inline std::string check_groups(const char* entry, int32_t groups) {
    if (groups >= 1 && groups <= MMS_MAX_GROUPS) return {};
    return std::string(entry) + ": groups must be 1.." + std::to_string(MMS_MAX_GROUPS);
}

static inline bool all_set(int n, const float* const* p) {
    if (!p) return false;
    for (int i = 0; i < n; i++)
        if (!p[i]) return false;
    return true;
}

static inline std::string check_gae_ppo_normalized(const float* rewards, const uint8_t* dones, const float* values, const float* last_values,
                                                   const float* returns, const float* advantages, const double* stats, int32_t T, int64_t N) {
    if (!rewards || !dones || !values || !last_values || !returns || !advantages || !stats || T < 1 || N < 1)
        return "mms_gae_ppo_normalized: bad arguments (null pointer, T < 1 or N < 1)";
    return {};
}

static inline std::string check_ppo_act(const float* mean, const float* log_std, const int64_t* counters, int64_t N, int32_t A) {
    if (!mean || !log_std || !counters || N < 0 || A <= 0 || A > 128) return "mms_ppo_act: bad arguments (A must be in 1..128)";
    return {};
}

static inline std::string check_ppo_heads_act(const float* hidden, const float* weight, const float* bias, int32_t H, const float* vhidden,
                                              const float* vweight, const float* vbias, int32_t VH, const float* log_std, const int64_t* counters,
                                              int64_t N, int32_t A) {
    if (!hidden || !weight || !bias || !log_std || !counters || N < 0 || A <= 0 || A > 128 || H <= 0 || (H % 64) != 0)
        return "mms_ppo_heads_act: bad arguments (A must be in 1..128, H a positive multiple of 64)";
    if (vhidden && (!vweight || !vbias || VH <= 0 || (VH % 4) != 0))
        return "mms_ppo_heads_act: the value head needs weight, bias and a hidden width that is a multiple of 4";
    return {};
}

static inline std::string check_sac_heads_act(const float* hidden, int32_t H, const float* mu_weight, const float* mu_bias, const float* ls_weight,
                                              const float* ls_bias, int32_t deterministic, const int64_t* counters, int64_t N, int32_t A) {
    if (!hidden || !mu_weight || !mu_bias || !ls_weight || !ls_bias || (!deterministic && !counters) || N < 0 || A <= 0 || A > 128 || H <= 0 ||
        (H % 64) != 0)
        return "mms_sac_heads_act: bad arguments (A must be in 1..128, H a positive multiple of 64, counters required unless deterministic)";
    if ((addr(hidden) | addr(mu_weight) | addr(ls_weight)) & 15) return "mms_sac_heads_act: hidden and both weight matrices must be 16-byte aligned";
    return {};
}

static inline std::string check_q_heads_backup(int64_t M, int32_t H, const float* h0, const float* w0, const float* b0, const float* q0_out,
                                               const float* h1, const float* w1, const float* b1, const float* q1_out, const float* reward,
                                               const uint8_t* done, const float* backup) {
    if (!h0 || !w0 || !b0 || M < 0 || H <= 0 || (H % 64) != 0 || H > MMS_Q_MAX_H)
        return "mms_q_heads_backup: bad arguments (h0, w0, b0 required, M >= 0, H a positive multiple of 64 up to " + std::to_string(MMS_Q_MAX_H) + ")";
    if ((h1 || w1 || b1 || q1_out) && !(h1 && w1 && b1)) return "mms_q_heads_backup: the second network needs h1, w1 and b1 (or all four NULL: one network)";
    if ((addr(h0) | addr(w0) | addr(h1) | addr(w1)) & 15) return "mms_q_heads_backup: hidden activations and weights must be 16-byte aligned";
    if (!q0_out && !q1_out && !backup) return "mms_q_heads_backup: no destination (q0_out, q1_out, backup all NULL)";
    if (backup && (!reward || !done)) return "mms_q_heads_backup: the backup needs reward and done";
    return {};
}

static inline std::string check_linear2_act(int64_t M, int32_t N, int32_t K, const float* x0, const float* w0, const float* b0, const float* y0,
                                            const float* x1, const float* w1, const float* b1, const float* y1, int32_t act) {
    if (!x0 || !w0 || !b0 || !y0 || M < 0 || M > 0x7fffffff || N <= 0 || K <= 0 || (K % 4) != 0 || act < 0 || act > 3)
        return "mms_linear2_act: bad arguments (K must be a positive multiple of 4, act 0..3)";
    if ((x1 || w1 || b1 || y1) && !(x1 && w1 && b1 && y1)) return "mms_linear2_act: the second problem needs all four pointers";
    return {};
}

static inline std::string check_split_planes(int64_t rows, int32_t K, int32_t x_pitch, const float* x, const void* planes) {
    if (!x || !planes || rows < 0 || K <= 0 || x_pitch < K || (x_pitch % 4) != 0 || (addr(x) & 15) != 0 || (addr(planes) & 15) != 0)
        return "mms_split_planes: bad arguments (x and planes 16-byte aligned, x_pitch >= K and a multiple of 4)";
    return {};
}

static inline std::string check_split_planes_group(int32_t groups, int64_t rows, int32_t K, int32_t x_pitch, const float* const* x, void* const* planes) {
    std::string bad = check_groups("mms_split_planes_group", groups);
    if (!bad.empty()) return bad;
    if (!x || !planes || rows < 0 || K <= 0 || x_pitch < K) return "mms_split_planes_group: bad arguments (x_pitch >= K)";
    for (int g = 0; g < groups; g++)
        if (!x[g] || !planes[g] || (addr(planes[g]) & 15) != 0 || (addr(x[g]) & 3) != 0)
            return "mms_split_planes_group: null or misaligned pointer in a group (planes 16-byte aligned)";
    return {};
}

static inline std::string check_split_layer(bool scaled, int32_t groups, int64_t M, int32_t N, int32_t K, const void* const* x, const void* const* w,
                                            const float* const* b, void* const* y, const float* const* x_inv, const float* const* w_inv,
                                            const float* const* y_scale, int32_t act, int32_t out_mode, const float* const* ln_s,
                                            const float* const* ln_stat_in, float* const* ln_part_out, const float* const* head_w,
                                            float* const* head_part, const int32_t* head_dims) {
    const char* fn = scaled ? "mms_linear_group_act_split16" : "mms_linear_group_act_split";
    std::string bad = check_groups(fn, groups);
    if (!bad.empty()) return bad;
    if (!x || !w || !b || (scaled && (!x_inv || !w_inv)) || M < 0 || M > 0x7fffffff || (M % 128) != 0 || N <= 0 || (N % 128) != 0 || K <= 0 || act < 0 ||
        act > 3 || out_mode < 0 || out_mode > 2 || (out_mode != 2 && !y) || (scaled && out_mode == 1 && !y_scale))
        return std::string(fn) + ": bad arguments (M and N multiples of 128, act 0..3, out_mode 0..2" + (scaled ? ", x_inv, w_inv, y_scale with out_mode 1)" : ")");
    const bool ln = ln_s || ln_stat_in || ln_part_out;
    if (ln && (!ln_s || !ln_stat_in || !ln_part_out || act != 1 || out_mode == 0))
        return std::string(fn) + ": the LayerNorm folds come together (ln_s, ln_stat_in, ln_part_out), with act = ELU and out_mode 1 or 2";
    if (out_mode == 2 && (!ln || !head_w || !head_part || !head_dims)) return std::string(fn) + ": out_mode 2 needs the LayerNorm folds, head_w, head_part and head_dims";
    for (int g = 0; g < groups; g++) {
        if (!x[g] || !w[g] || !b[g] || (scaled && (!x_inv[g] || !w_inv[g])) || (out_mode != 2 && !y[g]) || (scaled && out_mode == 1 && !y_scale[g]) ||
            (ln && (!ln_s[g] || !ln_stat_in[g] || !ln_part_out[g])) || (out_mode == 2 && (!head_w[g] || !head_part[g])))
            return std::string(fn) + ": null pointer in a group";
        uintptr_t bits = addr(x[g]) | addr(w[g]) | addr(b[g]);
        if (scaled) bits |= addr(w_inv[g]);
        if (out_mode != 2) bits |= addr(y[g]);
        if (ln) bits |= addr(ln_s[g]) | (addr(ln_stat_in[g]) << 1) | (addr(ln_part_out[g]) << 1);
        if ((bits & 15) != 0) return std::string(fn) + ": operands must be 16-byte aligned";
        if (out_mode == 2 && (head_dims[g] < 1 || head_dims[g] > 16)) return "split layer, out_mode 2: 1 <= head_dims[g] <= 16";
    }
    return {};
}

static inline std::string check_split_planes16_group(int32_t groups, int64_t rows, int32_t K, int32_t x_pitch, const float* const* x, void* const* planes,
                                                     float* const* scale, float* const* inv, int32_t nchains, int32_t L, const float* const* chain,
                                                     float* const* chain_scale, float* const* chain_inv, float* const* stat) {
    std::string bad = check_groups("mms_split_planes16_group", groups);
    if (!bad.empty()) return bad;
    if (!x || !planes || !scale || !inv || rows < 0 || K <= 0 || x_pitch < K || nchains < 0 || L < 0 || (nchains > 0 && (L < 1 || !chain || !chain_scale || !chain_inv)))
        return "mms_split_planes16_group: bad arguments (x_pitch >= K; nchains > 0 needs L >= 1, chain, chain_scale, chain_inv)";
    for (int g = 0; g < groups; g++) {
        if (!x[g] || !planes[g] || (addr(planes[g]) & 15) != 0 || (addr(x[g]) & 3) != 0 || (nchains > 0 && (!chain[g] || !chain_scale[g] || !chain_inv[g])))
            return "mms_split_planes16_group: null or misaligned pointer in a group (planes 16-byte aligned)";
        if (stat && (!stat[g] || (addr(stat[g]) & 7) != 0)) return "mms_split_planes16_group: null or misaligned stat pointer in a group";
    }
    return {};
}

static inline std::string check_weight_planes16_group(int32_t groups, const int64_t* N, const int32_t* K, const float* const* w, void* const* planes,
                                                      float* const* scale, float* const* inv) {
    std::string bad = check_groups("mms_weight_planes16_group", groups);
    if (!bad.empty()) return bad;
    if (!N || !K || !w || !planes || !scale || !inv) return "mms_weight_planes16_group: bad arguments (null array)";
    for (int g = 0; g < groups; g++) {
        if (N[g] < 0 || K[g] <= 0) return "mms_weight_planes16_group: bad shape in a group (N >= 0, K > 0)";
        if (!w[g] || !planes[g] || !scale[g] || !inv[g] || (addr(planes[g]) & 15) != 0 || (addr(w[g]) & 3) != 0 || (addr(inv[g]) & 15) != 0)
            return "mms_weight_planes16_group: null or misaligned pointer in a group (planes and inv 16-byte aligned)";
    }
    return {};
}

static inline std::string check_chain_refresh16(int32_t nchains, int32_t L, const float* const* l1, const int32_t* n, const float* chain, float bound0,
                                                int64_t rows, const float* chain_scale, const float* chain_inv) {
    if (nchains < 1 || L < 1 || (int64_t)nchains * L > MMS_MAX_GROUPS || !l1 || !n || !chain || rows < 0 || (rows > 0 && (!chain_scale || !chain_inv || !(bound0 >= 0.f))))
        return "mms_chain_refresh16: bad arguments (nchains, L >= 1, nchains * L <= " + std::to_string(MMS_MAX_GROUPS) + "; rows > 0 needs chain_scale, chain_inv, bound0 >= 0)";
    for (int e = 0; e < nchains * L; e++)
        if (!l1[e] || n[e] < 0) return "mms_chain_refresh16: null pointer or negative count in an entry";
    return {};
}

static inline std::string check_fold_planes16_group(int32_t groups, const int64_t* N, const int32_t* K, const float* const* w, void* const* planes,
                                                    float* const* inv) {
    std::string bad = check_groups("mms_fold_planes16_group", groups);
    if (!bad.empty()) return bad;
    if (!N || !K || !w) return "mms_fold_planes16_group: bad arguments (null array)";
    for (int g = 0; g < groups; g++) {
        if (N[g] < 0 || K[g] <= 0) return "mms_fold_planes16_group: bad shape in a group (N >= 0, K > 0)";
        if (!w[g] || (planes && planes[g] && (!inv || !inv[g])) || (planes && (addr(planes[g]) & 15) != 0))
            return "mms_fold_planes16_group: null or misaligned pointer in a group (planes 16-byte aligned and with inv)";
    }
    return {};
}

static inline std::string check_fold_scales16_group(int32_t groups, const float* const* rb, const int32_t* n, int64_t M) {
    std::string bad = check_groups("mms_fold_scales16_group", groups);
    if (!bad.empty()) return bad;
    if (!rb || !n || M < 0) return "mms_fold_scales16_group: bad arguments";
    for (int g = 0; g < groups; g++)
        if (!rb[g] || n[g] < 0) return "mms_fold_scales16_group: null pointer or negative count in a group";
    return {};
}

static inline std::string check_layer_clock_probe(const uint64_t* out, int32_t slots) {
    if (out && slots < 1) return "mms_layer_clock_probe: slots must be >= 1 with an output buffer";
    if (out && (addr(out) & 7) != 0) return "mms_layer_clock_probe: the buffer must be 8-byte aligned";
    return {};
}

static inline std::string check_row_stats_chan_group(int32_t groups, int64_t M, int32_t slots, const float* const* part, float* const* stat) {
    std::string bad = check_groups("mms_row_stats_chan_group", groups);
    if (!bad.empty()) return bad;
    if (!part || !stat || M < 0 || slots < 1) return "mms_row_stats_chan_group: bad arguments";
    for (int g = 0; g < groups; g++)
        if (!part[g] || !stat[g]) return "mms_row_stats_chan_group: null pointer in a group";
    return {};
}

static inline std::string check_marl_heads_finish(int32_t groups, int64_t M, int32_t slots, const float* const* part, const float* const* head_part,
                                                  const float* const* hs, const float* const* hc, const int32_t* A, float* const* out,
                                                  const int32_t* out_pitch) {
    std::string bad = check_groups("mms_marl_heads_finish", groups);
    if (!bad.empty()) return bad;
    if (!part || !head_part || !hs || !hc || !A || !out || M < 0 || slots < 1) return "mms_marl_heads_finish: bad arguments";
    for (int g = 0; g < groups; g++) {
        if (!part[g] || !head_part[g] || !hs[g] || !hc[g] || !out[g] || A[g] < 1 || A[g] > 16)
            return "mms_marl_heads_finish: null pointer or output width outside 1..16 in a group";
        if ((addr(head_part[g]) & 15) != 0 || (addr(part[g]) & 7) != 0)
            return "mms_marl_heads_finish: head_part must be 16-byte aligned and part 8-byte aligned (read as float4 / float2)";
        if (out_pitch && out_pitch[g] < A[g]) return "mms_marl_heads_finish: out_pitch below the output width";
    }
    return {};
}

static inline std::string check_linear_group_act(int32_t groups, int64_t M, int32_t N, int32_t K, const float* const* x, const float* const* w,
                                                 const float* const* b, float* const* y, int32_t act, const float* const* ln_s,
                                                 const float* const* ln_stat_in, float* const* ln_part_out) {
    std::string bad = check_groups("mms_linear_group_act", groups);
    if (!bad.empty()) return bad;
    if (!x || !w || !b || !y || M < 0 || M > 0x7fffffff || N <= 0 || K <= 0 || (K % 4) != 0 || act < 0 || act > 3)
        return "mms_linear_group_act: bad arguments (K must be a positive multiple of 4, act 0..3)";
    if ((ln_stat_in != nullptr) != (ln_s != nullptr)) return "mms_linear_group_act: ln_stat_in and ln_s come together";
    if ((ln_stat_in || ln_part_out) && (act != 1 || M % 128 != 0 || N % 128 != 0 || K < 8))
        return "mms_linear_group_act: the LayerNorm folds need act = ELU, M and N multiples of 128";
    for (int g = 0; g < groups; g++)
        if (!x[g] || !w[g] || !b[g] || !y[g] || (ln_s && (!ln_s[g] || !ln_stat_in[g])) || (ln_part_out && !ln_part_out[g]))
            return "mms_linear_group_act: null pointer in a group";
    return {};
}

static inline std::string check_row_stats_group(int32_t groups, int64_t M, int32_t slots, int32_t width, const float* const* part, float* const* stat) {
    std::string bad = check_groups("mms_row_stats_group", groups);
    if (!bad.empty()) return bad;
    if (!part || !stat || M < 0 || slots < 1 || width < 1) return "mms_row_stats_group: bad arguments";
    for (int g = 0; g < groups; g++)
        if (!part[g] || !stat[g]) return "mms_row_stats_group: null pointer in a group";
    return {};
}

static inline std::string check_row_moments_group(int32_t groups, int64_t M, int32_t K, int32_t x_pitch, const float* const* x, float* const* stat) {
    std::string bad = check_groups("mms_row_moments_group", groups);
    if (!bad.empty()) return bad;
    if (!x || !stat || M < 0 || K <= 0 || K > 4096 || x_pitch < K) return "mms_row_moments_group: bad arguments (1 <= K <= 4096)";
    for (int g = 0; g < groups; g++)
        if (!x[g] || !stat[g]) return "mms_row_moments_group: null pointer in a group";
    return {};
}

static inline std::string check_layernorm_group(int32_t groups, int64_t M, int32_t K, int32_t Kp, int32_t x_pitch, const float* const* x,
                                                const float* const* gamma, const float* const* beta, float* const* y) {
    std::string bad = check_groups("mms_layernorm_group", groups);
    if (!bad.empty()) return bad;
    if (!x || !gamma || !beta || !y || M < 0 || K <= 0 || K > 4096 || Kp < K || x_pitch < K)
        return "mms_layernorm_group: bad arguments (1 <= K <= 4096, Kp >= K, x_pitch >= K or 0)";
    for (int g = 0; g < groups; g++) {
        if (!x[g] || !gamma[g] || !beta[g] || !y[g]) return "mms_layernorm_group: null pointer in a group";
        if ((Kp != K || x_pitch != K) && x[g] == y[g]) return "mms_layernorm_group: in place needs Kp == x_pitch == K";
    }
    return {};
}

static inline std::string check_marl_heads_act(int32_t groups, int64_t M, int32_t H, const float* const* h, const float* const* gamma,
                                               const float* const* beta, const float* const* w, const float* const* b, const int32_t* A,
                                               float* const* out, const int32_t* out_pitch) {
    std::string bad = check_groups("mms_marl_heads_act", groups);
    if (!bad.empty()) return bad;
    if (!h || !gamma || !beta || !w || !b || !A || !out || M < 0 || H <= 0 || H > 1024) return "mms_marl_heads_act: bad arguments (1 <= H <= 1024)";
    for (int g = 0; g < groups; g++) {
        if (!h[g] || !gamma[g] || !beta[g] || !w[g] || !b[g] || !out[g] || A[g] < 1 || A[g] > 16)
            return "mms_marl_heads_act: null pointer in a group, or outputs outside 1..16";
        if (out_pitch && out_pitch[g] < A[g]) return "mms_marl_heads_act: out_pitch below the number of outputs";
    }
    return {};
}

static inline std::string check_mlp_shapes(const char* entry, int32_t layers, int64_t M, const int32_t* dims, const int64_t* ws_bytes) {
    bool ok = dims && ws_bytes && layers >= 2 && layers <= mms::kMlpMaxLayers && M >= 1 && M <= mms::kMlpMaxRows;
    for (int l = 0; ok && l <= layers; l++) ok = dims[l] >= 1 && dims[l] <= 65536;
    if (ok) return {};
    return std::string(entry) + ": bad arguments (2 <= layers <= " + std::to_string(mms::kMlpMaxLayers) + ", 1 <= M <= " + std::to_string(mms::kMlpMaxRows) +
           ", dims[0..layers] in 1..65536, ws_bytes required)";
}

static inline std::string check_mlp_grad(int32_t layers, int64_t M, const int32_t* dims, const float* x, const float* const* h, const float* const* w,
                                         const float* g, float* const* dw, float* const* db, float* const* d_out, float* const* e_out,
                                         const void* workspace, const int64_t* ws_bytes) {
    std::string bad = check_mlp_shapes("mms_mlp_grad", layers, M, dims, ws_bytes);
    if (!bad.empty() || !workspace) return bad;
    if (!x || !g || !all_set(layers - 1, h) || !all_set(layers, w) || !all_set(layers, dw) || !all_set(layers, db) ||
        (d_out && !all_set(layers - 1, d_out)) || (e_out && !all_set(layers - 1, e_out)))
        return "mms_mlp_grad: null pointer (x, g, h[layers-1], w / dw / db[layers]; d_out / e_out all or none)";
    return {};
}

static inline std::string check_mlp_grad_rop(int32_t layers, int64_t M, const int32_t* dims, const float* x, const float* const* h, const float* const* w,
                                             const float* const* v, const float* const* c, const float* g, const float* const* d,
                                             const float* const* e, const float* rmu, float* const* rdw, float* const* rdb, const void* workspace,
                                             const int64_t* ws_bytes) {
    std::string bad = check_mlp_shapes("mms_mlp_grad_rop", layers, M, dims, ws_bytes);
    if (!bad.empty() || !workspace) return bad;
    if (!x || !g || !rmu || !all_set(layers - 1, h) || !all_set(layers, w) || !all_set(layers, v) || !all_set(layers, c) || !all_set(layers - 1, d) ||
        !all_set(layers - 1, e) || !all_set(layers, rdw) || !all_set(layers, rdb))
        return "mms_mlp_grad_rop: null pointer (x, g, rmu, h / d / e[layers-1], w / v / c / rdw / rdb[layers])";
    return {};
}
```

massive_marl_benchmark_amd/csrc/policy_args.h:

```cpp
#pragma once
#include <hip/hip_runtime.h>
#include <stdint.h>

#include "../../include/mms.h"

namespace mms {

constexpr int kMaxGroups = MMS_MAX_GROUPS;

struct LinearArgs {
    const float* x[kMaxGroups];
    const float* w[kMaxGroups];
    const float* b[kMaxGroups];
    float* y[kMaxGroups];
    int M, N, K;
    int act;
    const float* s[kMaxGroups];
    const float* stat_in[kMaxGroups];
    float* part_out[kMaxGroups];
};

struct RowStatsArgs {
    const float* part[kMaxGroups];
    float* stat[kMaxGroups];
    int64_t M;
    int slots, width;
    float eps;
};

struct LayerNormArgs {
    const float* x[kMaxGroups];
    const float* gamma[kMaxGroups];
    const float* beta[kMaxGroups];
    float* y[kMaxGroups];
    int64_t M;
    int K, Kp;
    int x_pitch;
    float eps;
    int stats_only;
};

struct HeadsArgs {
    const float* h[kMaxGroups];
    const float* gamma[kMaxGroups];
    const float* beta[kMaxGroups];
    const float* w[kMaxGroups];
    const float* b[kMaxGroups];
    const float* std[kMaxGroups];
    float* out[kMaxGroups];
    float* logp[kMaxGroups];
    int64_t* counters[kMaxGroups];
    int A[kMaxGroups];
    int out_pitch[kMaxGroups];
    uint64_t seed;
    int64_t M, row_offset;
    int H;
    float eps;
};

struct SplitLinearArgs {
    const void* x[kMaxGroups];
    const void* w[kMaxGroups];
    const float* b[kMaxGroups];
    void* y[kMaxGroups];
    int M, N, KC;
    int act;
    int out_mode;
    const float* s[kMaxGroups];
    const float* stat_in[kMaxGroups];
    float* part_out[kMaxGroups];
    const float* head_w[kMaxGroups];
    float* head_part[kMaxGroups];
    int hdims[kMaxGroups];
    int tiles;
};

struct HeadsFinishArgs {
    const float* part[kMaxGroups];
    const float* head_part[kMaxGroups];
    const float* hs[kMaxGroups];
    const float* hc[kMaxGroups];
    const float* std[kMaxGroups];
    float* out[kMaxGroups];
    float* logp[kMaxGroups];
    int64_t* counters[kMaxGroups];
    int A[kMaxGroups];
    int out_pitch[kMaxGroups];
    uint64_t seed;
    int64_t M, row_offset;
    int slots, width;
    float eps;
};

struct SplitPlanesArgs {
    const float* x[kMaxGroups];
    void* planes[kMaxGroups];
    int64_t rows;
    int K, x_pitch;
};

struct Split16LinearArgs {
    const void* x[kMaxGroups];
    const void* w[kMaxGroups];
    const float* b[kMaxGroups];
    void* y[kMaxGroups];
    const float* xinv[kMaxGroups];
    const float* winv[kMaxGroups];
    const float* yscale[kMaxGroups];
    int M, N, KC;
    int act, out_mode;
    const float* s[kMaxGroups];
    const float* stat_in[kMaxGroups];
    float* part_out[kMaxGroups];
    const float* head_w[kMaxGroups];
    float* head_part[kMaxGroups];
    int hdims[kMaxGroups];
    int tiles, grid;
    uint64_t* clock_probe;
};

struct Split16PlanesArgs {
    const float* x[kMaxGroups];
    void* planes[kMaxGroups];
    float* scale[kMaxGroups];
    float* inv[kMaxGroups];
    const float* chain[kMaxGroups];
    float* chain_scale[kMaxGroups];
    float* chain_inv[kMaxGroups];
    float* stat[kMaxGroups];
    float* l1[kMaxGroups];
    int64_t rows;
    int K, x_pitch;
    int nchains, L;
    float eps;
    int per_group;
    int64_t rows_g[kMaxGroups];
    int K_g[kMaxGroups];
};

struct ChainRefreshArgs {
    const float* l1[kMaxGroups];
    const float* bias[kMaxGroups];
    int n[kMaxGroups];
    float* chain;
    int nchains, L;
    float bound0;
    int64_t rows;
    float* chain_scale;
    float* chain_inv;
};

struct FoldPlanesArgs {
    const float* w[kMaxGroups];
    const float* gamma[kMaxGroups];
    const float* beta[kMaxGroups];
    const float* bias[kMaxGroups];
    void* planes[kMaxGroups];
    float* inv[kMaxGroups];
    float* s[kMaxGroups];
    float* c[kMaxGroups];
    float* rb[kMaxGroups];
    float* wt[kMaxGroups];
    int64_t rows_g[kMaxGroups];
    int K_g[kMaxGroups];
};

struct FoldScalesArgs {
    const float* rb[kMaxGroups];
    float* scale1[kMaxGroups];
    float* ysc[kMaxGroups];
    float* yinv[kMaxGroups];
    int n[kMaxGroups];
    int64_t M;
};

hipError_t launch_fold_planes16(const FoldPlanesArgs& a, int groups, hipStream_t s);
hipError_t launch_fold_scales16(const FoldScalesArgs& a, int groups, hipStream_t s);
hipError_t launch_split16_planes_group(const Split16PlanesArgs& a, int groups, hipStream_t s);
hipError_t launch_chain_refresh16(const ChainRefreshArgs& a, hipStream_t s);
hipError_t launch_linear_split16(const Split16LinearArgs& a, int groups, hipStream_t s);
void set_split16_clock_probe(uint64_t* out, int slots);
hipError_t launch_linear_act(const LinearArgs& a, int groups, hipStream_t s);
hipError_t launch_row_stats_chan(const RowStatsArgs& a, int groups, hipStream_t s);
hipError_t launch_marl_heads_finish(const HeadsFinishArgs& a, int groups, hipStream_t s);
hipError_t launch_split_planes_group(const SplitPlanesArgs& a, int groups, hipStream_t s);
hipError_t launch_linear_split(const SplitLinearArgs& a, int groups, hipStream_t s);
hipError_t launch_split_planes(const float* x, void* planes, int64_t rows, int K, int x_pitch, hipStream_t s);
hipError_t launch_row_stats(const RowStatsArgs& a, int groups, hipStream_t s);
hipError_t launch_layernorm(const LayerNormArgs& a, int groups, hipStream_t s);
hipError_t launch_marl_heads(const HeadsArgs& a, int groups, hipStream_t s);

}
```

massive_marl_benchmark_amd/csrc/rollout_kernels.hip:

```cpp
#include <hip/hip_runtime.h>
#include <stdint.h>

#include <stdlib.h>

#include "head_block.h"
#include "mms_lane.h"
#include "rollout_lane.h"

#ifndef MMS_HEAD_RT_DEFAULT
#define MMS_HEAD_RT_DEFAULT 1
#endif

namespace mms {

__device__ __forceinline__ double wave_sum(double x) {
#pragma unroll
    for (int m = 32; m >= 1; m >>= 1) x += __shfl_xor(x, m, 64);
    return x;
}

__global__ void __launch_bounds__(256) gae_ppo_kernel(const float* __restrict__ rewards, const uint8_t* __restrict__ dones,
                                                      const float* __restrict__ values, const float* __restrict__ last_values,
                                                      float* __restrict__ returns, float* __restrict__ advantages,
                                                      double* __restrict__ stats, int T, int64_t N, float gamma, float lam) {
    __shared__ double s_sum[4], s_sq[4];
    double lsum = 0.0, lsq = 0.0;
    for (int64_t i = (int64_t)blockIdx.x * blockDim.x + threadIdx.x; i < N; i += (int64_t)gridDim.x * blockDim.x)
        gae_ppo_column(rewards, dones, values, last_values, returns, advantages, T, N, i, gamma, lam, lsum, lsq);
    lsum = wave_sum(lsum);
    lsq = wave_sum(lsq);
    int wave = threadIdx.x >> 6;
    if ((threadIdx.x & 63) == 0) { s_sum[wave] = lsum; s_sq[wave] = lsq; }
    __syncthreads();
    if (threadIdx.x == 0) {
        double a = 0.0, b = 0.0;
        for (int w = 0; w < (int)(blockDim.x >> 6); w++) { a += s_sum[w]; b += s_sq[w]; }
        atomicAdd(&stats[0], a);
        atomicAdd(&stats[1], b);
        if (blockIdx.x == 0) stats[2] = (double)T * (double)N;
    }
}

__global__ void __launch_bounds__(256) gae_ppo_partials_kernel(const float* __restrict__ rewards, const uint8_t* __restrict__ dones,
                                                               const float* __restrict__ values, const float* __restrict__ last_values,
                                                               float* __restrict__ returns, float* __restrict__ advantages,
                                                               double* __restrict__ stats, int T, int64_t N, float gamma, float lam) {
    __shared__ double s_sum[4], s_sq[4];
    double lsum = 0.0, lsq = 0.0;
    for (int64_t i = (int64_t)blockIdx.x * blockDim.x + threadIdx.x; i < N; i += (int64_t)gridDim.x * blockDim.x)
        gae_ppo_column(rewards, dones, values, last_values, returns, advantages, T, N, i, gamma, lam, lsum, lsq);
    lsum = wave_sum(lsum);
    lsq = wave_sum(lsq);
    const int wave = threadIdx.x >> 6;
    if ((threadIdx.x & 63) == 0) { s_sum[wave] = lsum; s_sq[wave] = lsq; }
    __syncthreads();
    if (threadIdx.x == 0) {
        stats[3 + 2 * blockIdx.x] = (s_sum[0] + s_sum[1]) + (s_sum[2] + s_sum[3]);
        stats[4 + 2 * blockIdx.x] = (s_sq[0] + s_sq[1]) + (s_sq[2] + s_sq[3]);
    }
}
__global__ void __launch_bounds__(256) adv_normalize_partials_kernel(float* __restrict__ advantages, double* __restrict__ stats, int nparts,
                                                                     double count_d, int64_t count) {
    __shared__ double s_sum[4], s_sq[4], s_tot[3];
    double a = 0.0, b = 0.0;
    for (int i = threadIdx.x; i < nparts; i += 256) { a += stats[3 + 2 * i]; b += stats[4 + 2 * i]; }
    a = wave_sum(a);
    b = wave_sum(b);
    if ((threadIdx.x & 63) == 0) { s_sum[threadIdx.x >> 6] = a; s_sq[threadIdx.x >> 6] = b; }
    __syncthreads();
    if (threadIdx.x == 0) {
        s_tot[0] = (s_sum[0] + s_sum[1]) + (s_sum[2] + s_sum[3]);
        s_tot[1] = (s_sq[0] + s_sq[1]) + (s_sq[2] + s_sq[3]);
        s_tot[2] = count_d;
        if (blockIdx.x == 0) { stats[0] = s_tot[0]; stats[1] = s_tot[1]; stats[2] = s_tot[2]; }
    }
    __syncthreads();
    float fm, inv;
    adv_norm_params(s_tot, fm, inv);
    for (int64_t i = (int64_t)blockIdx.x * blockDim.x + threadIdx.x; i < count; i += (int64_t)gridDim.x * blockDim.x)
        advantages[i] = (advantages[i] - fm) * inv;
}

__global__ void __launch_bounds__(256) adv_normalize_kernel(float* __restrict__ advantages, const double* __restrict__ stats, int64_t count) {
    float fm, inv;
    adv_norm_params(stats, fm, inv);
    for (int64_t i = (int64_t)blockIdx.x * blockDim.x + threadIdx.x; i < count; i += (int64_t)gridDim.x * blockDim.x)
        advantages[i] = (advantages[i] - fm) * inv;
}

__global__ void __launch_bounds__(256) gae_marl_kernel(const float* __restrict__ rewards, const float* __restrict__ value_preds,
                                                       const float* __restrict__ masks, float* __restrict__ returns, int T, int64_t N,
                                                       float gamma, float lam, int use_norm, const float* __restrict__ norm_mean,
                                                       const float* __restrict__ norm_var) {
    const float mean = use_norm ? norm_mean[0] : 0.f, var = use_norm ? norm_var[0] : 1.f;
    for (int64_t i = (int64_t)blockIdx.x * blockDim.x + threadIdx.x; i < N; i += (int64_t)gridDim.x * blockDim.x)
        gae_marl_column(rewards, value_preds, masks, returns, T, N, N, i, i, gamma, lam, use_norm, mean, var);
}

__global__ void __launch_bounds__(256) gae_marl_agents_kernel(const float* __restrict__ rewards, const float* __restrict__ value_preds,
                                                              const float* __restrict__ masks, float* __restrict__ returns, int T, int64_t N,
                                                              int A, float gamma, float lam, int use_norm,
                                                              const float* __restrict__ norm_mean, const float* __restrict__ norm_var) {
    const int64_t cols = N * A;
    for (int64_t c = (int64_t)blockIdx.x * blockDim.x + threadIdx.x; c < cols; c += (int64_t)gridDim.x * blockDim.x) {
        const int64_t i = c / A;
        const int k = (int)(c - i * A);
        gae_marl_column(rewards, value_preds, masks, returns, T, N, cols, c, i, gamma, lam, use_norm, use_norm ? norm_mean[k] : 0.f, use_norm ? norm_var[k] : 1.f);
    }
}

__global__ void __launch_bounds__(256) marl_views_kernel(const float* __restrict__ obs, float* __restrict__ obs_all, int64_t n,
                                                         int agents, int per, int shared) {
    const int64_t total = n * agents * (per + shared);
    for (int64_t i = (int64_t)blockIdx.x * blockDim.x + threadIdx.x; i < total; i += (int64_t)gridDim.x * blockDim.x)
        obs_all[i] = obs[marl_view_source(i, agents, per, shared)];
}

__global__ void __launch_bounds__(256) ppo_act_kernel(const float* __restrict__ mean, const float* __restrict__ value,
                                                      const float* __restrict__ log_std, uint64_t seed, int64_t* __restrict__ counters,
                                                      int64_t row_offset, int ref_scale, PpoActOut o, int64_t N, int A) {
    const int64_t row = (int64_t)blockIdx.x * 4 + (threadIdx.x >> 6);
    if (row >= N) return;
    ppo_sample_row(mean + row * A, value, log_std, seed, counters, row_offset, ref_scale, o, row, A, threadIdx.x & 63);
}

template <int NCT, int WAVES, int RT>
__global__ void __launch_bounds__(64 * WAVES) ppo_head_act_kernel(const float* __restrict__ hidden, const float* __restrict__ weight,
                                                           const float* __restrict__ bias, int H, const float* __restrict__ value,
                                                           const float* __restrict__ vhidden, const float* __restrict__ vweight,
                                                           const float* __restrict__ vbias, int VH,
                                                           const float* __restrict__ log_std, uint64_t seed, int64_t* __restrict__ counters,
                                                           int64_t row_offset, int ref_scale, PpoActOut o, int64_t N, int A) {
    extern __shared__ __attribute__((aligned(16))) float s_part[];
    ppo_head_block<NCT, WAVES, RT>(s_part, (int)threadIdx.x, true, (int64_t)blockIdx.x * 16 * RT, hidden, weight, bias, H, value, vhidden, vweight, vbias, VH,
                                   log_std, seed, counters, row_offset, ref_scale, o, N, A);
}

hipError_t launch_adv_normalize(float* advantages, const double* stats, int64_t count, hipStream_t s);
static int grid_for(int64_t n) {
    int64_t g = (n + 255) / 256;
    return (int)(g < 1 ? 1 : (g > 2048 ? 2048 : g));
}

hipError_t launch_gae_ppo(const float* rewards, const uint8_t* dones, const float* values, const float* last_values, float* returns,
                          float* advantages, double* stats, int T, int64_t N, float gamma, float lam, hipStream_t s) {
    hipError_t e = hipMemsetAsync(stats, 0, 3 * sizeof(double), s);
    if (e != hipSuccess) return e;
    hipLaunchKernelGGL(gae_ppo_kernel, dim3(grid_for(N)), dim3(256), 0, s, rewards, dones, values, last_values, returns, advantages, stats, T, N, gamma, lam);
    return hipGetLastError();
}
hipError_t launch_gae_ppo_normalized(const float* rewards, const uint8_t* dones, const float* values, const float* last_values, float* returns,
                                     float* advantages, double* stats, int T, int64_t N, float gamma, float lam, hipStream_t s) {
    const int blocks = grid_for(N);
    hipLaunchKernelGGL(gae_ppo_partials_kernel, dim3(blocks), dim3(256), 0, s, rewards, dones, values, last_values, returns, advantages, stats, T, N, gamma, lam);
    if (hipError_t e = hipGetLastError(); e != hipSuccess) return e;
    const int64_t count = (int64_t)T * N;
    hipLaunchKernelGGL(adv_normalize_partials_kernel, dim3(grid_for(count)), dim3(256), 0, s, advantages, stats, blocks, (double)T * (double)N, count);
    return hipGetLastError();
}
hipError_t launch_adv_normalize(float* advantages, const double* stats, int64_t count, hipStream_t s) {
    hipLaunchKernelGGL(adv_normalize_kernel, dim3(grid_for(count)), dim3(256), 0, s, advantages, stats, count);
    return hipGetLastError();
}
hipError_t launch_gae_marl(const float* rewards, const float* value_preds, const float* masks, float* returns, int T, int64_t N, float gamma,
                           float lam, int use_norm, const float* mean, const float* var, hipStream_t s) {
    hipLaunchKernelGGL(gae_marl_kernel, dim3(grid_for(N)), dim3(256), 0, s, rewards, value_preds, masks, returns, T, N, gamma, lam, use_norm, mean, var);
    return hipGetLastError();
}
hipError_t launch_gae_marl_agents(const float* rewards, const float* value_preds, const float* masks, float* returns, int T, int64_t N, int A,
                                  float gamma, float lam, int use_norm, const float* mean, const float* var, hipStream_t s) {
    hipLaunchKernelGGL(gae_marl_agents_kernel, dim3(grid_for(N * A)), dim3(256), 0, s, rewards, value_preds, masks, returns, T, N, A, gamma, lam, use_norm, mean, var);
    return hipGetLastError();
}
hipError_t launch_ppo_act(const float* mean, const float* value, const float* log_std, uint64_t seed, int64_t* counters, int64_t row_offset,
                          int ref_scale, float* actions_out, float* act_slot, float* logp_slot, float* value_slot, float* mu_slot,
                          float* sigma_slot, int64_t N, int A, hipStream_t s) {
    if (N == 0) return hipSuccess;
    PpoActOut o{actions_out, act_slot, logp_slot, value_slot, mu_slot, sigma_slot};
    hipLaunchKernelGGL(ppo_act_kernel, dim3((unsigned)((N + 3) / 4)), dim3(256), 0, s, mean, value, log_std, seed, counters, row_offset, ref_scale, o, N, A);
    return hipGetLastError();
}
hipError_t launch_ppo_head_act(const float* hidden, const float* weight, const float* bias, int H, const float* value, const float* vhidden,
                               const float* vweight, const float* vbias, int VH, const float* log_std,
                               uint64_t seed, int64_t* counters, int64_t row_offset, int ref_scale, float* actions_out, float* act_slot,
                               float* logp_slot, float* value_slot, float* mu_slot, float* sigma_slot, int64_t N, int A, hipStream_t s) {
    if (N == 0) return hipSuccess;
    PpoActOut o{actions_out, act_slot, logp_slot, value_slot, mu_slot, sigma_slot};
    const int nct = (A + 15) / 16;
    int waves = (H % 512 == 0) ? 8 : (H % 256 == 0) ? 4 : (H % 128 == 0) ? 2 : 1;
    static const int rt_env = getenv("MMS_HEAD_RT") ? atoi(getenv("MMS_HEAD_RT")) : MMS_HEAD_RT_DEFAULT;
    const int rt = (waves == 8 && rt_env == 2 && N >= 32) ? 2 : 1;
    size_t lds = (size_t)(waves + 1) * 16 * rt * (nct * 16) * sizeof(float);
    if (rt == 1 && lds > 64 * 1024) {
        waves = 4;
        lds = (size_t)(waves + 1) * 16 * (nct * 16) * sizeof(float);
    }
    const dim3 grid((unsigned)((N + 16 * rt - 1) / (16 * rt)));
#define MMS_HEAD_W(NCT, W)                                                                                                                        \
    hipLaunchKernelGGL((ppo_head_act_kernel<NCT, W, 1>), grid, dim3(64 * W), lds, s, hidden, weight, bias, H, value, vhidden, vweight, vbias, VH, \
                       log_std, seed, counters, row_offset, ref_scale, o, N, A)
#define MMS_HEAD2(NCT)                                                                                                                             \
    case NCT: {                                                                                                                                    \
        auto kern = ppo_head_act_kernel<NCT, 8, 2>;                                                                                                \
        if (lds > 64 * 1024) {                                                                                                                     \
            static bool done[64] = {};                                                                                                             \
            int dev = 0;                                                                                                                           \
            if (hipError_t e = hipGetDevice(&dev); e != hipSuccess) return e;                                                                      \
            if (dev < 0 || dev >= 64 || !done[dev]) {                                                                                              \
                if (hipError_t e = hipFuncSetAttribute(reinterpret_cast<const void*>(kern), hipFuncAttributeMaxDynamicSharedMemorySize, 160 * 1024); e != hipSuccess) return e; \
                if (dev >= 0 && dev < 64) done[dev] = true;                                                                                        \
            }                                                                                                                                      \
        }                                                                                                                                          \
        hipLaunchKernelGGL(kern, grid, dim3(512), lds, s, hidden, weight, bias, H, value, vhidden, vweight, vbias, VH, log_std, seed, counters,    \
                           row_offset, ref_scale, o, N, A);                                                                                        \
        break;                                                                                                                                     \
    }
#define MMS_HEAD(NCT)                                                                                                                              \
    case NCT:                                                                                                                                      \
        if (waves == 8) MMS_HEAD_W(NCT, 8);                                                                                                        \
        else if (waves == 4) MMS_HEAD_W(NCT, 4);                                                                                                   \
        else if (waves == 2) MMS_HEAD_W(NCT, 2);                                                                                                   \
        else MMS_HEAD_W(NCT, 1);                                                                                                                   \
        break;
    if (rt == 2) {
        switch (nct) {
            MMS_HEAD2(1) MMS_HEAD2(2) MMS_HEAD2(3) MMS_HEAD2(4) MMS_HEAD2(5) MMS_HEAD2(6) MMS_HEAD2(7) MMS_HEAD2(8)
            default: return hipErrorInvalidValue;
        }
        return hipGetLastError();
    }
    switch (nct) {
        MMS_HEAD(1) MMS_HEAD(2) MMS_HEAD(3) MMS_HEAD(4) MMS_HEAD(5) MMS_HEAD(6) MMS_HEAD(7) MMS_HEAD(8)
        default: return hipErrorInvalidValue;
    }
#undef MMS_HEAD
#undef MMS_HEAD2
#undef MMS_HEAD_W
    return hipGetLastError();
}
hipError_t launch_marl_views(const float* obs, float* obs_all, int64_t n, int agents, int per, int shared, hipStream_t s) {
    hipLaunchKernelGGL(marl_views_kernel, dim3(grid_for(n * agents * (per + shared))), dim3(256), 0, s, obs, obs_all, n, agents, per, shared);
    return hipGetLastError();
}

}
```

massive_marl_benchmark_amd/csrc/split16_kernels.hip:

```cpp
#include <hip/hip_runtime.h>
#include <stdint.h>
#include <stdlib.h>

#include <type_traits>

#include "policy_args.h"

namespace mms {

typedef _Float16 f16x8 __attribute__((ext_vector_type(8)));
typedef _Float16 f16x4 __attribute__((ext_vector_type(4)));
typedef float f32x4 __attribute__((ext_vector_type(4)));
typedef uint32_t u32x4_16 __attribute__((ext_vector_type(4)));

#ifndef MMS_S16_AUX_X
#define MMS_S16_AUX_X 0
#endif
#ifndef MMS_S16_AUX_W
#define MMS_S16_AUX_W 0
#endif
#ifndef MMS_S16_STAMP
#define MMS_S16_STAMP 0
#endif
#ifndef MMS_S16_EXP
#define MMS_S16_EXP 0
#endif
#if MMS_S16_EXP & 2
#define MMS_S16_MFMA(a, b, c, x, y, z) ([&] { asm volatile("" ::"v"(a), "v"(b)); return c; }())
#else
#define MMS_S16_MFMA(a, b, c, x, y, z) __builtin_amdgcn_mfma_f32_16x16x32_f16(a, b, c, x, y, z)
#endif
#ifndef MMS_S16_ROLL
#define MMS_S16_ROLL 1
#endif
constexpr int kChunk16 = 128;
constexpr float kLoScale = 2048.f;
constexpr int kTopExp = 14;

__device__ __forceinline__ void pow2_scale(float bound, float& scale, float& inv) {
    int e = kTopExp;
    if (bound > 0.f) (void)frexpf(bound, &e);
    int sh = kTopExp - e;
    sh = sh > 100 ? 100 : (sh < -100 ? -100 : sh);
    scale = ldexpf(1.f, sh);
    inv = ldexpf(1.f, -sh);
}

template <bool ALIGNED>
__global__ void __launch_bounds__(256) split16_planes_kernel(Split16PlanesArgs a, int KC, int P) {
    const int g = blockIdx.y;
    const float* __restrict__ x = a.x[g];
    uint8_t* __restrict__ out = reinterpret_cast<uint8_t*>(a.planes[g]);
    const int lane = threadIdx.x & 63;
    int K = a.K, pitch = a.x_pitch;
    int64_t rows = a.rows;
    if (a.per_group) {
        K = a.K_g[g];
        pitch = K;
        rows = a.rows_g[g];
        KC = (K + 31) / 32;
        P = 1;
        while (P < KC * 4 && P < 64) P <<= 1;
        if (rows == 0) return;
    }
    const int sub = lane & (P - 1), rpw = 64 / P;
    const int64_t row_raw = ((int64_t)blockIdx.x * 4 + (threadIdx.x >> 6)) * rpw + lane / P;
    const bool live = row_raw < rows;
    const int64_t row = live ? row_raw : rows - 1;
    const float* src = x + row * (int64_t)pitch;
    const int pieces = KC * 4;
    auto load8 = [&](int p, float* v) {
        const int k0 = p * 8;
        if (ALIGNED && k0 + 8 <= K) {
            const float4 q0 = *reinterpret_cast<const float4*>(src + k0), q1 = *reinterpret_cast<const float4*>(src + k0 + 4);
            v[0] = q0.x; v[1] = q0.y; v[2] = q0.z; v[3] = q0.w; v[4] = q1.x; v[5] = q1.y; v[6] = q1.z; v[7] = q1.w;
        } else {
#pragma unroll
            for (int j = 0; j < 8; j++) v[j] = (k0 + j < K) ? src[k0 + j] : 0.f;
        }
    };
    float big = 0.f, sum = 0.f, asum = 0.f;
    for (int p = sub; p < pieces; p += P) {
        float v[8];
        load8(p, v);
#pragma unroll
        for (int j = 0; j < 8; j++) { big = fmaxf(big, fabsf(v[j])); sum += v[j]; asum += fabsf(v[j]); }
    }
    for (int m = P >> 1; m >= 1; m >>= 1) {
        big = fmaxf(big, __shfl_xor(big, m, 64));
        sum += __shfl_xor(sum, m, 64);
        asum += __shfl_xor(asum, m, 64);
    }
    const float mean = sum / (float)K;
    float scale, inv;
    pow2_scale(big, scale, inv);
    float m2 = 0.f;
    for (int p = sub; p < pieces; p += P) {
        float v[8];
        load8(p, v);
        f16x8 hi, lo;
#pragma unroll
        for (int j = 0; j < 8; j++) {
            const float t = v[j] * scale;
            hi[j] = (_Float16)t;
            lo[j] = (_Float16)((t - (float)hi[j]) * kLoScale);
            const float d = (p * 8 + j < K) ? v[j] - mean : 0.f;
            m2 += d * d;
        }
        if (live) {
            uint8_t* dst = out + (row * KC + (p >> 2)) * (int64_t)kChunk16 + (p & 3) * 16;
            *reinterpret_cast<f16x8*>(dst) = hi;
            *reinterpret_cast<f16x8*>(dst + 64) = lo;
        }
    }
    if (a.stat[g])
        for (int m = P >> 1; m >= 1; m >>= 1) m2 += __shfl_xor(m2, m, 64);
    if (sub == 0 && live) {
        if (a.scale[g]) a.scale[g][row] = scale;
        if (a.inv[g]) a.inv[g][row] = inv;
        if (a.stat[g]) reinterpret_cast<float2*>(a.stat[g])[row] = make_float2(mean, 1.0f / sqrtf(m2 / (float)K + a.eps));
        if (a.l1[g]) a.l1[g][row] = asum;
    }
    if (live)
        for (int c = sub; c < a.nchains; c += P) {
            const float* ch = a.chain[g] + (size_t)c * a.L * 2;
            float bound = big;
            for (int l = 0; l < a.L; l++) {
                bound = (ch[2 * l] * bound + ch[2 * l + 1]) * 1.001f;
                float sc, iv;
                pow2_scale(bound, sc, iv);
                a.chain_scale[g][((size_t)c * a.L + l) * rows + row] = sc;
                a.chain_inv[g][((size_t)c * a.L + l) * rows + row] = iv;
            }
        }
}

hipError_t launch_split16_planes_group(const Split16PlanesArgs& a, int groups, hipStream_t s) {
    if (groups == 0) return hipSuccess;
    if (a.per_group) {
        bool aligned = true;
        unsigned blocks = 0;
        for (int g = 0; g < groups; g++) {
            aligned = aligned && (a.K_g[g] % 4) == 0 && (reinterpret_cast<uintptr_t>(a.x[g]) & 15) == 0;
            const int KCg = (a.K_g[g] + 31) / 32;
            int Pg = 1;
            while (Pg < KCg * 4 && Pg < 64) Pg <<= 1;
            const int64_t rpb = 4 * (64 / Pg);
            const unsigned need = (unsigned)((a.rows_g[g] + rpb - 1) / rpb);
            blocks = need > blocks ? need : blocks;
        }
        if (blocks == 0) return hipSuccess;
        if (aligned) hipLaunchKernelGGL(split16_planes_kernel<true>, dim3(blocks, groups), dim3(256), 0, s, a, 0, 1);
        else hipLaunchKernelGGL(split16_planes_kernel<false>, dim3(blocks, groups), dim3(256), 0, s, a, 0, 1);
        return hipGetLastError();
    }
    if (a.rows == 0) return hipSuccess;
    const int KC = (a.K + 31) / 32;
    bool aligned = (a.x_pitch % 4) == 0;
    for (int g = 0; g < groups; g++) aligned = aligned && (reinterpret_cast<uintptr_t>(a.x[g]) & 15) == 0;
    int P = 1;
    while (P < KC * 4 && P < 64) P <<= 1;
    const int64_t rows_per_block = 4 * (64 / P);
    const dim3 grid((unsigned)((a.rows + rows_per_block - 1) / rows_per_block), groups);
    if (aligned) hipLaunchKernelGGL(split16_planes_kernel<true>, grid, dim3(256), 0, s, a, KC, P);
    else hipLaunchKernelGGL(split16_planes_kernel<false>, grid, dim3(256), 0, s, a, KC, P);
    return hipGetLastError();
}

__global__ void __launch_bounds__(256) chain_refresh16_kernel(ChainRefreshArgs a) {
    __shared__ float s_chain[2 * kMaxGroups];
    const int E = a.nchains * a.L;
    const int lane = threadIdx.x & 63, wave = threadIdx.x >> 6;
    for (int e = wave; e < E; e += 4) {
        float m = 0.f, b = 0.f;
        for (int i = lane; i < a.n[e]; i += 64) {
            m = fmaxf(m, a.l1[e][i]);
            if (a.bias[e]) b = fmaxf(b, fabsf(a.bias[e][i]));
        }
        for (int k = 32; k >= 1; k >>= 1) {
            m = fmaxf(m, __shfl_xor(m, k, 64));
            b = fmaxf(b, __shfl_xor(b, k, 64));
        }
        if (lane == 0) { s_chain[2 * e] = m; s_chain[2 * e + 1] = b; }
    }
    __syncthreads();
    if (blockIdx.x == 0 && threadIdx.x < 2 * E) a.chain[threadIdx.x] = s_chain[threadIdx.x];
    const int64_t row = (int64_t)blockIdx.x * 256 + threadIdx.x;
    if (row >= a.rows) return;
    for (int c = 0; c < a.nchains; c++) {
        float bound = a.bound0;
        for (int l = 0; l < a.L; l++) {
            bound = (s_chain[2 * (c * a.L + l)] * bound + s_chain[2 * (c * a.L + l) + 1]) * 1.001f;
            float sc, iv;
            pow2_scale(bound, sc, iv);
            a.chain_scale[((size_t)c * a.L + l) * a.rows + row] = sc;
            a.chain_inv[((size_t)c * a.L + l) * a.rows + row] = iv;
        }
    }
}

hipError_t launch_chain_refresh16(const ChainRefreshArgs& a, hipStream_t s) {
    if (a.nchains * a.L == 0) return hipSuccess;
    const unsigned blocks = a.rows > 0 ? (unsigned)((a.rows + 255) / 256) : 1u;
    hipLaunchKernelGGL(chain_refresh16_kernel, dim3(blocks), dim3(256), 0, s, a);
    return hipGetLastError();
}

template <int MT>
struct Geom16 {
    static constexpr int TM = 64 * MT, TN = 128;
    static constexpr int XBYTES = TM * kChunk16, WBYTES = TN * kChunk16, BUF = XBYTES + WBYTES;
    static constexpr int NDMA = BUF / 1024 / 8;
    static constexpr int NX = TM / 64;
    static constexpr int SCRATCH = 8 * 16 * (2 * kChunk16 + 16);
    static constexpr bool SCRATCH_IN_BUF = BUF >= SCRATCH;
    static constexpr int HW_OFF = 3 * BUF + (SCRATCH_IN_BUF ? 0 : SCRATCH);
    static constexpr size_t LDS = (size_t)HW_OFF + 16 * 128 * 4;
};

__device__ __forceinline__ float act16_apply(float v, int act) {
    if (act == 1) return (v > 0.f) ? v : (expf(v) - 1.f);
    if (act == 2) return fmaxf(v, 0.f);
    if (act == 3) return 1.f - 2.f / (__expf(2.f * v) + 1.f);
    return v;
}

__device__ __forceinline__ f32x4 elu16_4(f32x4 x) {
    float l2e = 1.44269504088896340736f;
    asm volatile("" : "+s"(l2e));
    const f32x4 t = x * l2e;
    f32x4 e;
#pragma unroll
    for (int r = 0; r < 4; r++) e[r] = __builtin_amdgcn_exp2f(t[r]);
    e = e - 1.f;
#pragma unroll
    for (int r = 0; r < 4; r++) x[r] = __builtin_amdgcn_fmed3f(x[r], 0.f, e[r]);
    return x;
}

__device__ __forceinline__ void planes16_4(f32x4 v, float ys, float ys2k, uint32_t& h01, uint32_t& h23, uint32_t& l01, uint32_t& l23) {
    const f32x4 x = v * ys, x2 = v * ys2k;
    const f16x4 hi = __builtin_convertvector(x, f16x4);
    h01 = reinterpret_cast<const uint32_t*>(&hi)[0];
    h23 = reinterpret_cast<const uint32_t*>(&hi)[1];
    float c = -kLoScale;
    asm volatile("" : "+s"(c));
    asm("v_fma_mixlo_f16 %0, %1, %2, %3 op_sel:[0,0,0] op_sel_hi:[1,0,0]" : "=&v"(l01) : "v"(h01), "s"(c), "v"(x2[0]));
    asm("v_fma_mixhi_f16 %0, %1, %2, %3 op_sel:[1,0,0] op_sel_hi:[1,0,0]" : "+v"(l01) : "v"(h01), "s"(c), "v"(x2[1]));
    asm("v_fma_mixlo_f16 %0, %1, %2, %3 op_sel:[0,0,0] op_sel_hi:[1,0,0]" : "=&v"(l23) : "v"(h23), "s"(c), "v"(x2[2]));
    asm("v_fma_mixhi_f16 %0, %1, %2, %3 op_sel:[1,0,0] op_sel_hi:[1,0,0]" : "+v"(l23) : "v"(h23), "s"(c), "v"(x2[3]));
}

typedef __attribute__((address_space(3))) void* lptr16_t;

template <int N>
__device__ __forceinline__ void wait_vm() { asm volatile("s_waitcnt vmcnt(%0)" ::"n"(N) : "memory"); }

template <int MT, int OUT, int LN, bool ELU>
__global__ void __launch_bounds__(512, 2) linear_split16_kernel(Split16LinearArgs a) {
#if defined(__HIP_DEVICE_COMPILE__)
    using G = Geom16<MT>;
    extern __shared__ __attribute__((aligned(16))) uint8_t lds[];
    const int t = threadIdx.x, lane = t & 63, wave = __builtin_amdgcn_readfirstlane(t >> 6);
    const uint64_t probe_c0 = __builtin_readcyclecounter(), probe_r0 = __builtin_amdgcn_s_memrealtime();
#if MMS_S16_STAMP
    const uint64_t stamp_c0 = __builtin_readcyclecounter(), stamp_r0 = __builtin_amdgcn_s_memrealtime();
    uint64_t stamp_r12[2] = {0, 0};
#endif
    const int wm = wave >> 1, wn = wave & 1;
    const int KC = a.KC, N = a.N;
    const int tiles_n = N / G::TN, tiles_m = a.M / G::TM, total = a.tiles;
    const bool xcd_aware = (((total | a.grid) & 7) == 0);
    const size_t pitch = (size_t)KC * kChunk16;

    uint32_t goff[G::NDMA];
#pragma unroll
    for (int i = 0; i < G::NDMA; i++) {
        const int S = 64 * (wave + 8 * i) + lane;
        const int row = S >> 3, c8 = (S & 7) ^ ((row >> 1) & 7);
        goff[i] = (uint32_t)((i < G::NX ? row : row - G::TM) * (int)pitch + (c8 >> 2) * 64 + (c8 & 3) * 16);
    }
    int gi, m0, n0, tn;
    uint64_t x01[2] = {reinterpret_cast<uint64_t>(a.x[0]), reinterpret_cast<uint64_t>(a.x[1])};
    uint64_t w01[2] = {reinterpret_cast<uint64_t>(a.w[0]), reinterpret_cast<uint64_t>(a.w[1])};
    asm volatile("" : "+s"(x01[0]), "+s"(x01[1]), "+s"(w01[0]), "+s"(w01[1]));
    __amdgpu_buffer_rsrc_t xr, wr;
    auto setup_tile = [&](int v) {
        int L = v;
        if (xcd_aware) L = (v & 7) * (total >> 3) + (v >> 3);
        tn = L % tiles_n;
        const int rest = L / tiles_n;
        const int tm = rest % tiles_m;
        gi = rest / tiles_m;
        m0 = tm * G::TM;
        n0 = tn * G::TN;
        const uint64_t xg = gi == 0 ? x01[0] : (gi == 1 ? x01[1] : reinterpret_cast<uint64_t>(a.x[gi]));
        const uint64_t wg = gi == 0 ? w01[0] : (gi == 1 ? w01[1] : reinterpret_cast<uint64_t>(a.w[gi]));
        const uint8_t* xb = reinterpret_cast<const uint8_t*>(xg) + (size_t)m0 * pitch;
        const uint8_t* wb = reinterpret_cast<const uint8_t*>(wg) + (size_t)n0 * pitch;
        xr = __builtin_amdgcn_make_buffer_rsrc(const_cast<uint8_t*>(xb), (short)0, (int)(G::TM * pitch), 0x00020000);
        wr = __builtin_amdgcn_make_buffer_rsrc(const_cast<uint8_t*>(wb), (short)0, (int)(G::TN * pitch), 0x00020000);
    };
    auto dma_piece = [&](int i, int kc, int buf) {
        const int so = kc * kChunk16;
        if (i < G::NX) __builtin_amdgcn_raw_ptr_buffer_load_lds(xr, (lptr16_t)(lds + buf * G::BUF + (wave + 8 * i) * 1024), 16, goff[i], so, 0, MMS_S16_AUX_X);
        else __builtin_amdgcn_raw_ptr_buffer_load_lds(wr, (lptr16_t)(lds + buf * G::BUF + (wave + 8 * i) * 1024), 16, goff[i], so, 0, MMS_S16_AUX_W);
    };
    auto dma_slice = [&](int kc, int buf) {
#pragma unroll
        for (int i = 0; i < G::NDMA; i++) dma_piece(i, kc, buf);
    };

    const int frag = (lane & 15) * kChunk16 + (((lane >> 4) ^ (((lane & 15) >> 1) & 7)) * 16);
    const int xfrag = (wm * 16 * MT) * kChunk16 + frag;
    const int wfrag = G::XBYTES + (wn * 64) * kChunk16 + frag;

    f32x4 acc[MT][4], lo[MT][4];
#ifndef MMS_S16_DMA_BEHIND
#define MMS_S16_DMA_BEHIND (MT == 4)
#endif
    constexpr bool kDmaBehindFirstTile = MMS_S16_DMA_BEHIND;

    auto step = [&](int buf, bool more, int kc_next, int buf_next) {
        const uint8_t* base = lds + buf * G::BUF;
        if (!kDmaBehindFirstTile && more) dma_slice(kc_next, buf_next);
        f16x8 wf[4][2];
#pragma unroll
        for (int nt = 0; nt < 4; nt++) {
            wf[nt][0] = *reinterpret_cast<const f16x8*>(base + (wfrag + nt * 16 * kChunk16));
            wf[nt][1] = *reinterpret_cast<const f16x8*>(base + ((wfrag + nt * 16 * kChunk16) ^ 64));
        }
#pragma unroll
        for (int mt = 0; mt < MT; mt++) {
            f16x8 xf[2];
            xf[0] = *reinterpret_cast<const f16x8*>(base + (xfrag + mt * 16 * kChunk16));
            xf[1] = *reinterpret_cast<const f16x8*>(base + ((xfrag + mt * 16 * kChunk16) ^ 64));
#pragma unroll
            for (int nt = 0; nt < 4; nt++) lo[mt][nt] = __builtin_amdgcn_mfma_f32_16x16x32_f16(wf[nt][1], xf[0], lo[mt][nt], 0, 0, 0);
#pragma unroll
            for (int nt = 0; nt < 4; nt++) lo[mt][nt] = __builtin_amdgcn_mfma_f32_16x16x32_f16(wf[nt][0], xf[1], lo[mt][nt], 0, 0, 0);
#pragma unroll
            for (int nt = 0; nt < 4; nt++) acc[mt][nt] = __builtin_amdgcn_mfma_f32_16x16x32_f16(wf[nt][0], xf[0], acc[mt][nt], 0, 0, 0);
            if (kDmaBehindFirstTile && mt == 0) {
                __builtin_amdgcn_sched_barrier(0);
                if (more) dma_slice(kc_next, buf_next);
                __builtin_amdgcn_sched_barrier(0);
            }
        }
    };

    f16x8 wfr[4][2], xfr[MT][2];
    auto read_w = [&](const uint8_t* base, int nt) {
        wfr[nt][0] = *reinterpret_cast<const f16x8*>(base + (wfrag + nt * 16 * kChunk16));
        wfr[nt][1] = *reinterpret_cast<const f16x8*>(base + ((wfrag + nt * 16 * kChunk16) ^ 64));
    };
    auto read_x = [&](const uint8_t* base, int mt) {
        xfr[mt][0] = *reinterpret_cast<const f16x8*>(base + (xfrag + mt * 16 * kChunk16));
// ... 399 lines not shown
```

massive_marl_benchmark_amd/csrc/step_kernels.hip:

```cpp
#include <hip/hip_runtime.h>

#include "head_block.h"
#include "mms_lane.h"
#include "step_args.h"

namespace mms {

template <int CTRL>
__device__ __forceinline__ float dpp_mov(float x) {
    return __builtin_bit_cast(float, __builtin_amdgcn_update_dpp(0, __builtin_bit_cast(int, x), CTRL, 0xF, 0xF, true));
}
__device__ __forceinline__ float quad_sum(float x) {
    x += dpp_mov<0xB1>(x);
    x += dpp_mov<0x4E>(x);
    return x;
}
__device__ __forceinline__ float oct_sum(float x) {
    x = quad_sum(x);
    x += dpp_mov<0x141>(x);
    return x;
}
__device__ __forceinline__ void quad_sum(Sym6& A, S6& p) {
#pragma unroll
    for (int k = 0; k < 21; k++) A.m[k] = quad_sum(A.m[k]);
    p.a.x = quad_sum(p.a.x); p.a.y = quad_sum(p.a.y); p.a.z = quad_sum(p.a.z);
    p.l.x = quad_sum(p.l.x); p.l.y = quad_sum(p.l.y); p.l.z = quad_sum(p.l.z);
}
__device__ __forceinline__ void oct_sum(BoxCorner& c) {
#pragma unroll
    for (int k = 0; k < 9; k++) c.t[k] = oct_sum(c.t[k]);
}
__device__ __forceinline__ float wave_sum(float x) {
    x = oct_sum(x);
    x += dpp_mov<0x140>(x);
    x += __shfl_xor(x, 16, 64);
    x += __shfl_xor(x, 32, 64);
    return x;
}

typedef float f32x4_t __attribute__((ext_vector_type(4)));
__device__ __forceinline__ void stream_store(float4* dst, float4 v) {
    __builtin_nontemporal_store(f32x4_t{v.x, v.y, v.z, v.w}, reinterpret_cast<f32x4_t*>(dst));
}

__device__ __forceinline__ RigidState load_rigid(const float* r) {
    RigidState B;
    B.pos = V3{r[0], r[1], r[2]};
    B.qx = r[3]; B.qy = r[4]; B.qz = r[5]; B.qw = r[6];
    B.vel = V3{r[7], r[8], r[9]};
    B.ang = V3{r[10], r[11], r[12]};
    return B;
}
__device__ __forceinline__ void store_rigid(float* r, const RigidState& B) {
    r[0] = B.pos.x; r[1] = B.pos.y; r[2] = B.pos.z;
    r[3] = B.qx; r[4] = B.qy; r[5] = B.qz; r[6] = B.qw;
    r[7] = B.vel.x; r[8] = B.vel.y; r[9] = B.vel.z;
    r[10] = B.ang.x; r[11] = B.ang.y; r[12] = B.ang.z;
}

#ifndef MMS_WAVES_PER_EU
#define MMS_WAVES_PER_EU 2
#endif
__host__ __device__ inline size_t ant_env_lds_floats(int obs_dim, int A) {
    return (size_t)((obs_dim + 3) & ~3) + 16 + (sizeof(BoxPose) + 15) / 16 * 4 + 28 + 8 + (size_t)(((RP_STRIDE + 6) * A + 3) & ~3) +
           (size_t)((4 * A + 2 + 7 + 3) & ~3);
}
#ifndef MMS_WAVES_PER_EU_PACKED
#define MMS_WAVES_PER_EU_PACKED 3
#endif
template <int TASK, int BLOCK, int EPB, int AT, bool DR, bool HEAD = false>
#ifndef MMS_WAVES_PER_EU_WIDE
#define MMS_WAVES_PER_EU_WIDE 3
#endif
__global__ void __launch_bounds__(BLOCK, BLOCK == 64 ? MMS_WAVES_PER_EU : ((BLOCK == 192 || BLOCK == 768) ? MMS_WAVES_PER_EU_PACKED : MMS_WAVES_PER_EU_WIDE)) ant_step_kernel(StepArgs a) {
    extern __shared__ __attribute__((aligned(16))) float lds[];
    const mms_config* __restrict__ Cg = a.cfg;
    constexpr int kCfgFloats = (int)((sizeof(mms_config) + 15) / 16 * 4);
    static_assert(sizeof(mms_config) % 4 == 0, "copied word by word");
    const mms_config* C = reinterpret_cast<const mms_config*>(lds);
    const mms_model* M = &C->model;
    float2 ac_head = make_float2(0.f, 0.f);
    constexpr int kObsAT = TASK == MMS_TASK_TEN_ANT ? 38 * AT + 8 : (TASK == MMS_TASK_MULTI_ANT_CIRCLE ? 38 * AT : 60);
    constexpr int kPrevAT = TASK == MMS_TASK_TEN_ANT ? 4 * AT + 2 : (TASK == MMS_TASK_MULTI_ANT_CIRCLE ? 2 * AT : 6);
    const int obs_dim = AT > 0 ? kObsAT : a.obs_dim;
    const int prev_dim = AT > 0 ? kPrevAT : a.prev_dim;
    const int obs_pad = (obs_dim + 3) & ~3;

    const int A = AT > 0 ? AT : a.num_agents;
    const int LA = 4 * A;
    const int ant_region = EPB * LA;
    const int box_region = (BLOCK == 512 && EPB == 1 && ant_region <= 448) ? 448 : ((ant_region + 7) & ~7);
    const int bt = (int)threadIdx.x - box_region;
    const bool is_ant = (int)threadIdx.x < ant_region;
    const bool is_box = bt >= 0 && bt < 8 * EPB;
    const int e_loc = EPB == 1 ? 0 : (is_ant ? (int)threadIdx.x / LA : (is_box ? bt >> 3 : 0));
    const int tid = is_ant ? (int)threadIdx.x - e_loc * LA : 0;
    const int corner = bt & 7;
    const bool box_lead = is_box && corner == 0;
    const int env_raw = blockIdx.x * EPB + e_loc;
    const bool live = env_raw < a.num_envs;
    const int env = live ? env_raw : a.num_envs - 1;
    const int ant = tid >> 2, leg = tid & 3;

    LegConst* s_leg = reinterpret_cast<LegConst*>(lds + kCfgFloats);
    constexpr int kBoxOff = 0, kBpOff = 16, kFacOff = kBpOff + (int)((sizeof(BoxPose) + 15) / 16 * 4), kEpiOff = kFacOff + 28, kRedOff = kEpiOff + 8;
    const size_t env_stride = (ant_env_lds_floats(obs_dim, A) + 3) & ~(size_t)3;
    float* lds_envs = lds + kCfgFloats + (4 * sizeof(LegConst) + 15) / 16 * 4;
    float* s_root = lds_envs + (size_t)EPB * ((ant_env_lds_floats(AT > 0 ? kObsAT : a.obs_dim, A) + 3) & ~(size_t)3);
    constexpr bool kStage = AT > 0 && ((EPB * (AT + 1) * 13) % 4) == 0;
    const int root_floats = kStage ? EPB * (A + 1) * 13 : 0;
    float* lds_lanes = s_root + ((root_floats + 3) & ~3);
    if constexpr (HEAD) {
        static_assert(BLOCK == 768 && EPB == 16 && AT == 10 && TASK == MMS_TASK_TEN_ANT && kStage, "the fused head assumes 16 rows x 80 actions per block");
        float* s_head = lds_lanes;
        float* s_head_actions = s_head + 9 * 16 * 80;
        static_assert((9 + 1) * 16 * 80 <= 6 * 4 * BLOCK, "the head's LDS must fit the parking space");
        if (threadIdx.x >= 512) {
            const int t = (int)threadIdx.x - 512;
            const float4* src = reinterpret_cast<const float4*>(a.root_states + (size_t)blockIdx.x * root_floats);
            for (int i = t; i < root_floats / 4; i += 256) reinterpret_cast<float4*>(s_root)[i] = src[i];
            for (int i = t; i < (int)(sizeof(mms_config) / 4); i += 256) lds[i] = reinterpret_cast<const float*>(Cg)[i];
            if (t < 4) s_leg[t] = load_leg_const(&Cg->model, t);
            constexpr int kStageOff = ((kRedOff + (RP_STRIDE + 6) * AT + 3) & ~3) + ((kObsAT + 3) & ~3);
            for (int i = t; i < EPB * prev_dim; i += 256) {
                const int e = i / prev_dim, k = i - e * prev_dim;
                (lds_envs + (size_t)e * env_stride + kStageOff)[k] = a.prev[((size_t)blockIdx.x * EPB + e) * prev_dim + k];
            }
        }
        PpoActOut o{a.head.actions_out, a.head.act_slot, a.head.logp_slot, a.head.value_slot, a.head.mu_slot, a.head.sigma_slot};
        o.lds_actions = s_head_actions;
        o.lds_row0 = (int64_t)blockIdx.x * 16;
        if (a.head.weight_tiles)
            ppo_head_block<5, 8, 1, 4, true>(s_head, (int)threadIdx.x, threadIdx.x < 512, (int64_t)blockIdx.x * 16, a.head.hidden, a.head.weight, a.head.bias, a.head.H, nullptr,
                                             a.head.vhidden, a.head.vweight, a.head.vbias, a.head.VH, a.head.log_std, a.head.seed, a.head.counters, a.head.row_offset,
                                             a.head.reference_scale, o, a.num_envs, 8 * AT, a.head.weight_tiles);
        else
            ppo_head_block<5, 8, 1, 4>(s_head, (int)threadIdx.x, threadIdx.x < 512, (int64_t)blockIdx.x * 16, a.head.hidden, a.head.weight, a.head.bias, a.head.H, nullptr,
                                       a.head.vhidden, a.head.vweight, a.head.vbias, a.head.VH, a.head.log_std, a.head.seed, a.head.counters, a.head.row_offset,
                                       a.head.reference_scale, o, a.num_envs, 8 * AT);
        __syncthreads();
        if (threadIdx.x < 16 * 4 * AT) ac_head = reinterpret_cast<const float2*>(s_head_actions)[threadIdx.x];
    }
    const KinPark park{lds_lanes + 4 * threadIdx.x, 4 * BLOCK};
    LegDR* s_dr = reinterpret_cast<LegDR*>(lds_lanes + 6 * 4 * BLOCK) + threadIdx.x;
    float* env_lds = lds_envs + (size_t)e_loc * env_stride;
    float* s_box = env_lds + kBoxOff;
    BoxPose* s_bp = reinterpret_cast<BoxPose*>(env_lds + kBpOff);
    float4* s_fac = reinterpret_cast<float4*>(env_lds + kFacOff);
    float* s_epi = env_lds + kEpiOff;
    float* s_red = env_lds + kRedOff;
    float* s_wr = s_red + RP_STRIDE * A;
    float* s_obs = env_lds + ((kRedOff + (RP_STRIDE + 6) * A + 3) & ~3);
    float* s_stage = s_obs + obs_pad;
    float* s_act = s_obs + (TASK != MMS_TASK_ONE_ANT ? 38 * ant + 30 + 2 * leg : 52 + 2 * leg);

    const int actors = A + 1;
    const bool reset_now = a.reset[env] != 0;

    AntLane S = {};
    float2 ac = make_float2(0.f, 0.f);
    if (kStage && !HEAD) {
        const size_t g0 = (size_t)blockIdx.x * root_floats, gtot = (size_t)a.num_envs * actors * 13;
        if (g0 + root_floats <= gtot) {
            const float4* src = reinterpret_cast<const float4*>(a.root_states + g0);
            for (int i = threadIdx.x; i < root_floats / 4; i += BLOCK) reinterpret_cast<float4*>(s_root)[i] = src[i];
        } else {
            for (int i = threadIdx.x; i < root_floats; i += BLOCK) {
                size_t f = g0 + i;
                if (f >= gtot) f = gtot - (size_t)actors * 13 + (f % ((size_t)actors * 13));
                s_root[i] = a.root_states[f];
            }
        }
    } else if (is_ant) {
        const float* r = a.root_states + ((size_t)env * actors + ant) * 13;
        S.pos = V3{r[0], r[1], r[2]};
        S.qx = r[3]; S.qy = r[4]; S.qz = r[5]; S.qw = r[6];
        S.vel = V3{r[7], r[8], r[9]};
        S.ang = V3{r[10], r[11], r[12]};
    }
    if (is_ant) {
        float4 d = reinterpret_cast<const float4*>(a.dof_state + (size_t)env * A * 16)[tid];
        S.q[0] = d.x; S.qd[0] = d.y; S.q[1] = d.z; S.qd[1] = d.w;
        if constexpr (HEAD) ac = ac_head;
        else ac = reinterpret_cast<const float2*>(a.actions + (size_t)env * A * 8)[tid];
        if (DR) *s_dr = load_leg_dr(a.dr + ((size_t)env * A + ant) * MMS_DR_FLOATS, leg);
    }
    for (int i = threadIdx.x; i < (HEAD ? 0 : (int)(sizeof(mms_config) / 4)); i += BLOCK) lds[i] = reinterpret_cast<const float*>(Cg)[i];
    if (!HEAD && threadIdx.x < 4) s_leg[threadIdx.x] = load_leg_const(&Cg->model, threadIdx.x);

    for (int i = threadIdx.x; i < (HEAD ? 0 : EPB * prev_dim); i += BLOCK) {
        const int e = i / prev_dim, k = i - e * prev_dim;
        const int en = min((int)(blockIdx.x * EPB + e), a.num_envs - 1);
        (lds_envs + (size_t)e * env_stride + (s_stage - env_lds))[k] = a.prev[(size_t)en * prev_dim + k];
    }
    if (is_box && corner == 1) {
        s_stage[prev_dim + 0] = a.env_origin[3 * env]; s_stage[prev_dim + 1] = a.env_origin[3 * env + 1];
        s_stage[prev_dim + 2] = a.env_origin[3 * env + 2];
        int64_t pr = a.progress[env], rc = a.reset_count[env];
        int* si = reinterpret_cast<int*>(s_stage + prev_dim + 3);
        si[0] = (int)(pr & 0xffffffff); si[1] = (int)(pr >> 32); si[2] = (int)(rc & 0xffffffff); si[3] = (int)(rc >> 32);
    }
    if (is_ant) {
        s_act[0] = clampf(ac.x, -Cg->clip_actions, Cg->clip_actions);
        s_act[1] = clampf(ac.y, -Cg->clip_actions, Cg->clip_actions);
    }
    if (kStage) __syncthreads();
    if (kStage && is_ant) {
        const float* r = s_root + (e_loc * actors + ant) * 13;
        S.pos = V3{r[0], r[1], r[2]};
        S.qx = r[3]; S.qy = r[4]; S.qz = r[5]; S.qw = r[6];
        S.vel = V3{r[7], r[8], r[9]};
        S.ang = V3{r[10], r[11], r[12]};
    }
    if (box_lead) {
        RigidState B0 = load_rigid(kStage ? s_root + (e_loc * actors + A) * 13 : a.root_states + ((size_t)env * actors + A) * 13);
        store_rigid(s_box, B0);
        s_bp->pos = B0.pos; s_bp->R = quat_to_mat(B0.qx, B0.qy, B0.qz, B0.qw); s_bp->v = B0.vel; s_bp->w = B0.ang;
        const mms_model* Mb = kStage ? &C->model : &Cg->model;
        s_bp->half = V3{Mb->box_half[0], Mb->box_half[1], Mb->box_half[2]};
    }
    __syncthreads();
    const LegConst& L = s_leg[leg];
    float sens[6] = {0.f, 0.f, 0.f, 0.f, 0.f, 0.f};
    if (TASK == MMS_TASK_ONE_ANT && is_ant) {
        const float* fs = a.foot_sensors + ((size_t)env * A + ant) * 24 + 6 * leg;
#pragma unroll
        for (int i = 0; i < 6; i++) sens[i] = fs[i];
    }

    const bool simulate = a.do_physics && !reset_now;
    if (a.do_physics) {
        const float h = C->dt / (float)C->substeps;
        constexpr bool kSensors = (TASK == MMS_TASK_ONE_ANT);
        constexpr bool kOneWave = (BLOCK == 64 && EPB == 1);
        auto ant_phase = [&](bool wait_for_box) -> S6 {
            S6 wr = S6{V3{0, 0, 0}, V3{0, 0, 0}};
            Sym6 IA0;
            S6 pA0;
            LegPass P;
            SensorPass SP;
            LegInward W;
            constexpr bool kSplit = BLOCK > 64;
            if (kSplit && is_ant && simulate) leg_inward_open<kSensors, DR>(M, L, h, S, P, &SP, W, park, s_dr);
            if (kSplit ? wait_for_box : false) __syncthreads();
            if (is_ant && simulate) {
                const float tau1 = s_act[0] * L.gear[0] * C->power_scale;
                const float tau2 = s_act[1] * L.gear[1] * C->power_scale;
                if (!kSplit) leg_inward<kSensors, DR>(M, L, h, S, leg, tau1, tau2, true, *s_bp, P, &SP, IA0, pA0, park, s_dr);
                else leg_inward_close<kSensors, DR>(M, L, h, S, leg, tau1, tau2, true, *s_bp, P, &SP, IA0, pA0, W, s_dr);
            }
            quad_sum(IA0, pA0);
            if (is_ant && simulate) leg_outward<kSensors>(M, L, h, S, leg, *s_bp, P, &SP, IA0, pA0, wr, sens, park);
            return wr;
        };
        auto stage_wrench = [&](S6 wr) {
            wr.a.x = quad_sum(wr.a.x); wr.a.y = quad_sum(wr.a.y); wr.a.z = quad_sum(wr.a.z);
            wr.l.x = quad_sum(wr.l.x); wr.l.y = quad_sum(wr.l.y); wr.l.z = quad_sum(wr.l.z);
            if (is_ant && leg == 0) {
                s_wr[0 * A + ant] = wr.a.x; s_wr[1 * A + ant] = wr.a.y; s_wr[2 * A + ant] = wr.a.z;
                s_wr[3 * A + ant] = wr.l.x; s_wr[4 * A + ant] = wr.l.y; s_wr[5 * A + ant] = wr.l.z;
            }
        };
        auto gather_wrench = [&]() -> S6 {
            float t = 0.f;
            if (corner < 6) {
                const float* col = s_wr + corner * A;
                for (int i = 0; i < A; i++) t += col[i];
            }
#define MMS_FROM(c) __int_as_float(__builtin_amdgcn_ds_swizzle(__float_as_int(t), 0x18 | ((c) << 5)))
            return S6{V3{MMS_FROM(0), MMS_FROM(1), MMS_FROM(2)}, V3{MMS_FROM(3), MMS_FROM(4), MMS_FROM(5)}};
#undef MMS_FROM
        };
        auto box_store = [&](const RigidState& B) {
            store_rigid(s_box, B);
            s_bp->pos = B.pos; s_bp->R = quat_to_mat(B.qx, B.qy, B.qz, B.qw); s_bp->v = B.vel; s_bp->w = B.ang;
        };
        const bool box_friction = M->boxgnd_mu > 0.f;
        for (int s = 0; s < C->substeps; s++) {
            S6 wr = ant_phase(s > 0);
            BoxCorner bc = {};
            if (is_box && !box_friction) {
                bc = box_corner(M, h, load_rigid(s_box), s_bp->R, corner);
                oct_sum(bc);
            }
            if (is_box && box_friction) {
                const RigidState B0 = load_rigid(s_box);
                BoxCornerF bf = box_corner_friction(M, h, B0, s_bp->R, corner);
#pragma unroll
                for (int k = 0; k < 21; k++) bf.IA.m[k] = oct_sum(bf.IA.m[k]);
                bf.pA.a.x = oct_sum(bf.pA.a.x); bf.pA.a.y = oct_sum(bf.pA.a.y); bf.pA.a.z = oct_sum(bf.pA.a.z);
// ... 398 lines not shown
```

Baseline: 29.15 million env-steps/s.

## Overlap head noise/value work with step-kernel staging and add single-launch weight refresh

In the fused step kernel, the 256 spare threads now batch their staging loads (root states, config, prev) into registers and also fetch and compute the PPO head's noise, log-prob and value for the block's rows. This work runs while the other 512 threads compute the head's mean, and ppo_head_block takes a flag so it skips that part. Separately, a new mms_refresh16 kernel fuses the weight-plane split, head tile fill and chain refresh into one launch, using a last-block ticket. That path is enabled only by the MMS_REFRESH_LAUNCHES=1 environment variable. The aim is to hide the head's serial tail and cut launch count, at the cost of more registers and an atomic ticket.

Result: faster. 29.49 million env-steps/s, median of 6 (+1.2%).

```diff
diff --git a/include/mms.h b/include/mms.h
--- a/include/mms.h
+++ b/include/mms.h
@@ -201,6 +201,21 @@
 int mms_chain_refresh16(int device, int32_t nchains, int32_t L, const float* const* l1, const float* const* bias, const int32_t* n,
                         float* chain, float bound0, int64_t rows, float* chain_scale, float* chain_inv, void* hip_stream);
 
+#define MMS_REFRESH16_GROUPS 16
+#define MMS_REFRESH16_SETS 4
+typedef struct mms_refresh16_set {
+    int32_t nchains, L;
+    const int32_t* entry;
+    float* chain;
+    float bound0;
+    int64_t rows;
+    float* chain_scale;
+    float* chain_inv;
+} mms_refresh16_set;
+int mms_refresh16(int device, int32_t groups, const int64_t* N, const int32_t* K, const float* const* w, const float* const* bias,
+                  void* const* planes, float* const* scale, float* const* inv, float* const* l1, const float* head_w, float* head_tiles,
+                  int32_t head_A, int32_t head_H, int32_t nsets, const mms_refresh16_set* sets, uint32_t* count, void* hip_stream);
+
 int mms_linear_group_act_split16(int device, int32_t groups, int64_t M, int32_t N, int32_t K, const void* const* x, const void* const* w,
                                  const float* const* b, void* const* y, const float* const* x_inv, const float* const* w_inv,
                                  const float* const* y_scale, int32_t act, int32_t out_mode, const float* const* ln_s,
diff --git a/massive_marl_benchmark_amd/_lib.py b/massive_marl_benchmark_amd/_lib.py
--- a/massive_marl_benchmark_amd/_lib.py
+++ b/massive_marl_benchmark_amd/_lib.py
@@ -10,12 +10,17 @@
 _lib_cpu = None
 
 SYMBOLS = ["mms_create", "mms_destroy", "mms_get_tensor", "mms_step", "mms_post_step", "mms_reset_all", "mms_set_state",
-           "mms_bind_obs_out", "mms_bind_obs_planes16", "mms_bind_actions", "mms_bind_policy_head", "mms_set_dr", "mms_set_obs_outputs", "mms_bind_rollout_out", "mms_ppo_act", "mms_ppo_heads_act", "mms_sac_heads_act", "mms_q_heads_backup", "mms_linear2_act", "mms_linear_group_act", "mms_split_planes", "mms_split_planes_group", "mms_linear_group_act_split", "mms_split_planes16_group", "mms_weight_planes16_group", "mms_chain_refresh16", "mms_fold_planes16_group", "mms_fold_scales16_group", "mms_linear_group_act_split16", "mms_row_stats_chan_group", "mms_marl_heads_finish", "mms_row_stats_group", "mms_row_moments_group", "mms_layernorm_group", "mms_marl_heads_act", "mms_marl_views", "mms_gae_ppo", "mms_adv_normalize", "mms_gae_ppo_normalized", "mms_layer_clock_probe", "mms_gae_marl", "mms_gae_marl_agents", "mms_mlp_grad", "mms_mlp_grad_rop",
+           "mms_bind_obs_out", "mms_bind_obs_planes16", "mms_bind_actions", "mms_bind_policy_head", "mms_set_dr", "mms_set_obs_outputs", "mms_bind_rollout_out", "mms_ppo_act", "mms_ppo_heads_act", "mms_sac_heads_act", "mms_q_heads_backup", "mms_linear2_act", "mms_linear_group_act", "mms_split_planes", "mms_split_planes_group", "mms_linear_group_act_split", "mms_split_planes16_group", "mms_weight_planes16_group", "mms_chain_refresh16", "mms_refresh16", "mms_fold_planes16_group", "mms_fold_scales16_group", "mms_linear_group_act_split16", "mms_row_stats_chan_group", "mms_marl_heads_finish", "mms_row_stats_group", "mms_row_moments_group", "mms_layernorm_group", "mms_marl_heads_act", "mms_marl_views", "mms_gae_ppo", "mms_adv_normalize", "mms_gae_ppo_normalized", "mms_layer_clock_probe", "mms_gae_marl", "mms_gae_marl_agents", "mms_mlp_grad", "mms_mlp_grad_rop",
            "mms_last_error", "mms_abi_version"]
 
 
 class MmsError(RuntimeError):
     pass
+
+
+class MmsRefresh16Set(ctypes.Structure):
+    _fields_ = [("nchains", ctypes.c_int32), ("L", ctypes.c_int32), ("entry", ctypes.c_void_p), ("chain", ctypes.c_void_p),
+                ("bound0", ctypes.c_float), ("rows", ctypes.c_int64), ("chain_scale", ctypes.c_void_p), ("chain_inv", ctypes.c_void_p)]
 
 
 def _bind(path):
@@ -52,6 +57,7 @@
     L.mms_fold_planes16_group.argtypes = [ci, ctypes.c_int32, vp, vp, vp, vp, vp, vp, vp, vp, vp, vp, vp, vp, vp]
     L.mms_fold_scales16_group.argtypes = [ci, ctypes.c_int32, vp, vp, c64, vp, vp, vp, vp]
     L.mms_chain_refresh16.argtypes = [ci, ctypes.c_int32, ctypes.c_int32, vp, vp, vp, vp, cf, c64, vp, vp, vp]
+    L.mms_refresh16.argtypes = [ci, ctypes.c_int32, vp, vp, vp, vp, vp, vp, vp, vp, vp, vp, ctypes.c_int32, ctypes.c_int32, ctypes.c_int32, vp, vp, vp]
     L.mms_linear_group_act_split16.argtypes = [ci, ctypes.c_int32, c64, ctypes.c_int32, ctypes.c_int32, vp, vp, vp, vp, vp, vp, vp, ctypes.c_int32, ctypes.c_int32,
                                                vp, vp, vp, vp, vp, vp, vp]
     L.mms_row_stats_chan_group.argtypes = [ci, ctypes.c_int32, c64, ctypes.c_int32, vp, vp, cf, vp]
diff --git a/massive_marl_benchmark_amd/algorithms/rl/ppo/module.py b/massive_marl_benchmark_amd/algorithms/rl/ppo/module.py
--- a/massive_marl_benchmark_amd/algorithms/rl/ppo/module.py
+++ b/massive_marl_benchmark_amd/algorithms/rl/ppo/module.py
@@ -1,4 +1,5 @@
 import ctypes
+import os
 import math
 
 import numpy as np
@@ -108,6 +109,8 @@
     def _p32_bytes(rows, K):
         return rows * ((K + 31) // 32) * 192
 
+    refresh_one_launch = os.environ.get("MMS_REFRESH_LAUNCHES", "3") == "1"
+
     def _weight_planes(self, lin, L, idx, stream, force=False):
         if self._wplanes is None:
             self._wplanes = {}
@@ -195,9 +198,16 @@
             self._h16, self._wplanes, self._split_bufs, self._calls, self._sample_calls = None, None, None, None, None
             self._head_wt = None
         self._addr_tag, self._ver_tag = (addrs, str(dev)), vers
-        if self._head_wt is not None:
+        st = self._h16
+        if st is not None and self.refresh_one_launch:
+            call = self._refresh16_call(st)
+            if call is not None:
+                _lib.check(st["L"].mms_refresh16(*call[0], _lib.for_device(st["dev"])[2]), None, "mms_refresh16", st["L"])
+                st = None
+            elif self._head_wt is not None:
+                self._fill_head_tiles()
+        elif self._head_wt is not None:
             self._fill_head_tiles()
-        st = self._h16
         if st is not None:
             stream = _lib.for_device(st["dev"])[2]
             for fn, args, what in st["calls"]:
@@ -224,6 +234,55 @@
                     self._weight_planes(lin, *_lib.for_device(lin.weight.device), force=True)
                 else:
                     self._wplanes[key] = (None, planes, lin)
+
+    def _chain_sets(self, st):
+        sets, covered = [], set()
+        for (members, rows, scale), (_, cs, ci, alias) in st["given"].items():
+            if alias or self._chain_args(st, members) is None:
+                continue
+            sets.append((members, rows, scale, cs, ci))
+            covered.update(members)
+        depths = {Lh for _, Lh in st["slices"]}
+        rest = [tuple(range(len(st["recs"])))] if len(depths) == 1 else [(g,) for g in range(len(st["recs"]))]
+        for grp in rest:
+            if not set(grp) <= covered and self._chain_args(st, grp) is not None:
+                sets.append((grp, 0, 0.0, None, None))
+        return sets
+
+    def _refresh16_call(self, st):
+        sets = self._chain_sets(st)
+        key = (tuple(s[:3] for s in sets), None if self._head_wt is None else self._head_wt[1].data_ptr())
+        hit = st.get("refresh16")
+        if hit is not None and hit[1] == key:
+            return hit
+        flat = [r for rs in st["recs"] for r in rs]
+        index = {id(r): i for i, r in enumerate(flat)}
+        last = self.actor[-1]
+        head = self._head_wt is not None and last.weight.dtype == torch.float32 and last.weight.is_contiguous() and last.in_features % 4 == 0
+        if not flat or len(flat) > 16 or len(sets) > 4 or (self._head_wt is not None and not head):
+            return None
+        arr = lambda ts: (ctypes.c_void_p * len(ts))(*[None if t is None else t.data_ptr() for t in ts])
+        cset = (_lib.MmsRefresh16Set * max(len(sets), 1))()
+        keep = []
+        for i, (members, rows, scale, cs, ci) in enumerate(sets):
+            _, Lh = self._chain(st, list(members))
+            ent = [index[id(st["recs"][g][li])] for g in members for li in range(Lh)]
+            if len(ent) > 16:
+                return None
+            entry = (ctypes.c_int32 * len(ent))(*ent)
+            keep.append(entry)
+            chain = self._chain(st, list(members))[0]
+            cset[i] = _lib.MmsRefresh16Set(len(members), Lh, ctypes.cast(entry, ctypes.c_void_p).value, chain.data_ptr(),
+                                           16384.0 / scale if rows else 0.0, rows, None if cs is None else cs.data_ptr(), None if ci is None else ci.data_ptr())
+        if "count" not in st:
+            st["count"] = torch.zeros(1, dtype=torch.int32, device=st["dev"])
+        args = (st["idx"], len(flat), (ctypes.c_int64 * len(flat))(*[r["N"] for r in flat]), (ctypes.c_int32 * len(flat))(*[r["K"] for r in flat]),
+                arr([r["lin"].weight for r in flat]), arr([r["lin"].bias for r in flat]), arr([r["planes"] for r in flat]), arr([r["scale"] for r in flat]),
+                arr([r["inv"] for r in flat]), arr([r["l1"] for r in flat]),
+                ctypes.c_void_p(last.weight.data_ptr()) if head else None, ctypes.c_void_p(self._head_wt[1].data_ptr()) if head else None,
+                last.out_features if head else 0, last.in_features if head else 0, len(sets), ctypes.cast(cset, ctypes.c_void_p), ctypes.c_void_p(st["count"].data_ptr()))
+        st["refresh16"] = (args, key, cset, keep)
+        return st["refresh16"]
 
     def _head_tiles(self):
         if self._head_wt is None:
diff --git a/massive_marl_benchmark_amd/csrc/cpu/mms_cpu.cpp b/massive_marl_benchmark_amd/csrc/cpu/mms_cpu.cpp
--- a/massive_marl_benchmark_amd/csrc/cpu/mms_cpu.cpp
+++ b/massive_marl_benchmark_amd/csrc/cpu/mms_cpu.cpp
@@ -574,6 +574,37 @@
                 chain_inv[((size_t)c * L + l) * rows + r] = iv;
             }
         }
+    }
+    return 0;
+}
+
+MMS_API int mms_refresh16(int device, int32_t groups, const int64_t* N, const int32_t* K, const float* const* w, const float* const* bias,
+                          void* const* planes, float* const* scale, float* const* inv, float* const* l1, const float* head_w, float* head_tiles,
+                          int32_t head_A, int32_t head_H, int32_t nsets, const mms_refresh16_set* sets, uint32_t* count, void*) {
+    if (cpu_only(device)) return 1;
+    if (refused(check_refresh16(groups, N, K, w, planes, scale, inv, l1, head_w, head_tiles, head_A, head_H, nsets, sets, count))) return 1;
+    if (mms_weight_planes16_group(device, groups, N, K, w, planes, scale, inv, l1, nullptr)) return 1;
+    if (head_w) {
+        const int H4 = head_H / 4, nct = (head_A + 15) / 16;
+        for (int ct = 0; ct < nct; ct++)
+            for (int kg = 0; kg < H4; kg++)
+                for (int i = 0; i < 16; i++)
+                    for (int q = 0; q < 4; q++) {
+                        const int j = ct * 16 + i;
+                        head_tiles[(((size_t)ct * H4 + kg) * 16 + i) * 4 + q] = j < head_A ? head_w[(size_t)j * head_H + 4 * kg + q] : 0.f;
+                    }
+    }
+    for (int si = 0; si < nsets; si++) {
+        const mms_refresh16_set& S = sets[si];
+        const float* l1e[MMS_REFRESH16_GROUPS];
+        const float* be[MMS_REFRESH16_GROUPS];
+        int32_t ne[MMS_REFRESH16_GROUPS];
+        for (int e = 0; e < S.nchains * S.L; e++) {
+            l1e[e] = l1[S.entry[e]];
+            be[e] = bias ? bias[S.entry[e]] : nullptr;
+            ne[e] = (int32_t)N[S.entry[e]];
+        }
+        if (mms_chain_refresh16(device, S.nchains, S.L, l1e, be, ne, S.chain, S.bound0, S.rows, S.chain_scale, S.chain_inv, nullptr)) return 1;
     }
     return 0;
 }
diff --git a/massive_marl_benchmark_amd/csrc/head_block.h b/massive_marl_benchmark_amd/csrc/head_block.h
--- a/massive_marl_benchmark_amd/csrc/head_block.h
+++ b/massive_marl_benchmark_amd/csrc/head_block.h
@@ -41,9 +41,128 @@
     }
 }
 
+template <int R, int NJ>
+struct PpoNoiseOperands {
+    int64_t c[R];
+    float ls[NJ];
+    float4 w4[2], h4[R][2];
+};
+template <int R, int NJ>
+__device__ __forceinline__ void ppo_rows_noise_fetch(PpoNoiseOperands<R, NJ>& f, const float* __restrict__ vhidden, const float* __restrict__ vweight, int VH,
+                                                     const float* __restrict__ log_std, const int64_t* __restrict__ counters, int64_t row0, int stride,
+                                                     int64_t N, int A, int lane) {
+#pragma unroll
+    for (int q = 0; q < R; q++) {
+        const int64_t row = row0 + q * stride;
+        f.c[q] = counters[row < N ? row : N - 1];
+    }
+#pragma unroll
+    for (int u = 0; u < NJ; u++) f.ls[u] = lane + 64 * u < A ? log_std[lane + 64 * u] : 0.f;
+#pragma unroll
+    for (int t = 0; t < 2; t++) {
+        const int k = lane * 4 + 256 * t;
+        f.w4[t] = make_float4(0.f, 0.f, 0.f, 0.f);
+#pragma unroll
+        for (int q = 0; q < R; q++) f.h4[q][t] = make_float4(0.f, 0.f, 0.f, 0.f);
+        if (vhidden && k < VH) {
+            f.w4[t] = *reinterpret_cast<const float4*>(vweight + k);
+#pragma unroll
+            for (int q = 0; q < R; q++) {
+                const int64_t row = row0 + q * stride;
+                f.h4[q][t] = *reinterpret_cast<const float4*>(vhidden + (row < N ? row : N - 1) * (int64_t)VH + k);
+            }
+        }
+    }
+}
+template <int R, int NJ>
+__device__ __forceinline__ void ppo_rows_noise_finish(const PpoNoiseOperands<R, NJ>& f, const float* __restrict__ value, const float* __restrict__ vhidden,
+                                                      const float* __restrict__ vweight, const float* __restrict__ vbias, int VH,
+                                                      uint64_t seed, int64_t* __restrict__ counters, int64_t row_offset,
+                                                      int ref_scale, const PpoActOut& o, int64_t row0, int stride, int64_t N, int A, int lane, float* z_row0) {
+    float v[R], lp[R];
+#pragma unroll
+    for (int q = 0; q < R; q++) { v[q] = 0.f; lp[q] = 0.f; }
+#pragma unroll
+    for (int u = 0; u < NJ; u++) {
+        const int j = lane + 64 * u;
+        if (j >= A) break;
+        const float ls = f.ls[u];
+        float lscale;
+        if (ref_scale) { const float sd = expf(ls); lscale = logf(sd * sd); }
+        else lscale = ls;
+#pragma unroll
+        for (int q = 0; q < R; q++) {
+            const int64_t row = row0 + q * stride;
+            if (row >= N) continue;
+            const float z = rand_normal(seed, (uint64_t)(row_offset + row), (uint64_t)f.c[q], (uint32_t)j);
+            lp[q] += -0.5f * z * z - lscale - 0.9189385332046727f;
+            z_row0[(int64_t)q * stride * A + j] = z;
+            if (o.sigma_slot) o.sigma_slot[row * A + j] = ls;
+        }
+    }
+    if (vhidden) {
+#pragma unroll
+        for (int t = 0; t < 2; t++) {
+            if (lane * 4 + 256 * t < VH) {
+#pragma unroll
+                for (int q = 0; q < R; q++)
+                    v[q] += f.h4[q][t].x * f.w4[t].x + f.h4[q][t].y * f.w4[t].y + f.h4[q][t].z * f.w4[t].z + f.h4[q][t].w * f.w4[t].w;
+            }
+        }
+        for (int k = lane * 4 + 512; k < VH; k += 256) {
+            const float4 w4 = *reinterpret_cast<const float4*>(vweight + k);
+#pragma unroll
+            for (int q = 0; q < R; q++) {
+                const int64_t row = row0 + q * stride;
+                const float4 h4 = *reinterpret_cast<const float4*>(vhidden + (row < N ? row : N - 1) * (int64_t)VH + k);
+                v[q] += h4.x * w4.x + h4.y * w4.y + h4.z * w4.z + h4.w * w4.w;
+            }
+        }
+        const float vb = vbias[0];
+#pragma unroll
+        for (int q = 0; q < R; q++) {
+#pragma unroll
+            for (int m = 32; m >= 1; m >>= 1) v[q] += __shfl_xor(v[q], m, 64);
+            v[q] = v[q] + vb;
+        }
+    }
+#pragma unroll
+    for (int q = 0; q < R; q++) {
+        const int64_t row = row0 + q * stride;
+#pragma unroll
+        for (int m = 32; m >= 1; m >>= 1) lp[q] += __shfl_xor(lp[q], m, 64);
+        if (lane == 0 && row < N) {
+            if (o.logp_slot) o.logp_slot[row] = lp[q];
+            if (o.value_slot && (vhidden || value)) o.value_slot[row] = vhidden ? v[q] : value[row];
+            counters[row] = f.c[q] + 1;
+        }
+    }
+}
+__device__ __forceinline__ float ppo_action_scale(float log_std, int ref_scale) {
+    if (ref_scale) { const float sd = expf(log_std); return sd * sd; }
+    return expf(log_std);
+}
+template <int NJ>
+__device__ __forceinline__ void ppo_row_actions(const float* mean_row, const float (&log_std_lane)[NJ], int ref_scale, const PpoActOut& o, int64_t row,
+                                                int A, int lane, float* za_row) {
+#pragma unroll
+    for (int u = 0; u < NJ; u++) {
+        const int j = lane + 64 * u;
+        if (j >= A) break;
+        const float m = mean_row[j];
+        const float scale = ppo_action_scale(log_std_lane[u], ref_scale);
+        const float z = za_row[j];
+        const float act = m + scale * z;
+        if (o.actions_out) o.actions_out[row * A + j] = act;
+        za_row[j] = act;
+        if (o.act_slot) o.act_slot[row * A + j] = act;
+        if (o.mu_slot) o.mu_slot[row * A + j] = m;
+    }
+}
+
 typedef float f32x4 __attribute__((ext_vector_type(4)));
 
-template <int NCT, int WAVES, int RT, int UB = 4, bool TILED = false>
+template <int NCT, int WAVES, int RT, int UB = 4, bool TILED = false, bool SPLIT = false>
 __device__ __forceinline__ void ppo_head_block(float* s_part, const int tid, const bool active, const int64_t r0,
                                                const float* __restrict__ hidden, const float* __restrict__ weight,
                                                const float* __restrict__ bias, int H, const float* __restrict__ value,
@@ -63,9 +182,12 @@
 #endif
     const int lane = tid & 63, wave = active ? (tid >> 6) : 0;
     const int i = lane & 15, g = lane >> 4;
-    float v_rows[RPW];
+    constexpr int NJ = (AP + 63) / 64;
+    float v_rows[RPW], ls_lane[NJ];
 #pragma unroll
     for (int q = 0; q < RPW; q++) v_rows[q] = 0.f;
+#pragma unroll
+    for (int u = 0; u < NJ; u++) ls_lane[u] = 0.f;
     if (active) {
         const float* hrow[RT];
 #pragma unroll
@@ -87,7 +209,7 @@
 #pragma unroll
         for (int q = 0; q < RPW; q++) {
             const int64_t row = r0 + wave * RPW + q;
-            if (vhidden && row < N) {
+            if (!SPLIT && vhidden && row < N) {
                 const float* hv = vhidden + row * (int64_t)VH;
                 float part = 0.f;
                 for (int k = lane * 4; k < VH; k += 256) {
@@ -139,6 +261,11 @@
 #pragma unroll
                 for (int r = 0; r < 4; r++) mine[(16 * rt + 4 * g + r) * AP + ct * 16 + i] = acc[rt][ct][r];
             }
+        if (SPLIT) {
+#pragma unroll
+            for (int u = 0; u < NJ; u++)
+                if (lane + 64 * u < A) ls_lane[u] = log_std[lane + 64 * u];
+        }
     }
     __syncthreads();
     MMS_HEAD_ST(3);
@@ -159,7 +286,8 @@
             const int r = wave * RPW + q;
             const int64_t row = r0 + r;
             if (row >= N) continue;
-            ppo_sample_row(s_mean + r * AP, value, log_std, seed, counters, row_offset, ref_scale, o, row, A, lane, vhidden != nullptr, v_rows[q]);
+            if (SPLIT) ppo_row_actions<NJ>(s_mean + r * AP, ls_lane, ref_scale, o, row, A, lane, o.lds_actions + (row - o.lds_row0) * A);
+            else ppo_sample_row(s_mean + r * AP, value, log_std, seed, counters, row_offset, ref_scale, o, row, A, lane, vhidden != nullptr, v_rows[q]);
         }
     }
 #if MMS_HEAD_STAMP
diff --git a/massive_marl_benchmark_amd/csrc/mms_api.hip b/massive_marl_benchmark_amd/csrc/mms_api.hip
--- a/massive_marl_benchmark_amd/csrc/mms_api.hip
+++ b/massive_marl_benchmark_amd/csrc/mms_api.hip
@@ -427,6 +427,32 @@
     return 0;
 }
 
+__attribute__((visibility("default"))) int mms_refresh16(int device, int32_t groups, const int64_t* N, const int32_t* K, const float* const* w,
+                                                         const float* const* bias, void* const* planes, float* const* scale, float* const* inv,
+                                                         float* const* l1, const float* head_w, float* head_tiles, int32_t head_A, int32_t head_H,
+                                                         int32_t nsets, const mms_refresh16_set* sets, uint32_t* count, void* s) {
+    MMS_DEV(device)
+    if (refused(check_refresh16(groups, N, K, w, planes, scale, inv, l1, head_w, head_tiles, head_A, head_H, nsets, sets, count))) return 1;
+    mms::Refresh16Args a = {};
+    for (int g = 0; g < groups; g++) {
+        a.x[g] = w[g]; a.planes[g] = planes[g]; a.scale[g] = scale[g]; a.inv[g] = inv[g]; a.l1[g] = l1[g];
+        a.bias[g] = bias ? bias[g] : nullptr;
+        a.rows_g[g] = N[g]; a.K_g[g] = K[g];
+    }
+    a.groups = groups;
+    a.head_w = head_w; a.head_tiles = head_tiles; a.head_A = head_A; a.head_H = head_H;
+    a.nsets = nsets;
+    for (int si = 0; si < nsets; si++) {
+        mms::Refresh16Args::Set& S = a.set[si];
+        for (int e = 0; e < sets[si].nchains * sets[si].L; e++) S.entry[e] = (unsigned char)sets[si].entry[e];
+        S.nchains = sets[si].nchains; S.L = sets[si].L; S.bound0 = sets[si].bound0; S.rows = sets[si].rows;
+        S.chain = sets[si].chain; S.chain_scale = sets[si].chain_scale; S.chain_inv = sets[si].chain_inv;
+    }
+    a.count = count;
+    MMS_FREE(mms::launch_refresh16(a, (hipStream_t)s));
+    return 0;
+}
+
 __attribute__((visibility("default"))) int mms_fold_planes16_group(int device, int32_t groups, const int64_t* N, const int32_t* K, const float* const* w,
                                                                    const float* const* gamma, const float* const* beta, const float* const* bias,
                                                                    void* const* planes, float* const* inv, float* const* s_out, float* const* c_out,
diff --git a/massive_marl_benchmark_amd/csrc/mms_host.h b/massive_marl_benchmark_amd/csrc/mms_host.h
--- a/massive_marl_benchmark_amd/csrc/mms_host.h
+++ b/massive_marl_benchmark_amd/csrc/mms_host.h
@@ -399,6 +399,31 @@
     return {};
 }
 
+static inline std::string check_refresh16(int32_t groups, const int64_t* N, const int32_t* K, const float* const* w, void* const* planes,
+                                          float* const* scale, float* const* inv, float* const* l1, const float* head_w, const float* head_tiles,
+                                          int32_t head_A, int32_t head_H, int32_t nsets, const mms_refresh16_set* sets, const uint32_t* count) {
+    if (groups < 1 || groups > MMS_REFRESH16_GROUPS) return "mms_refresh16: groups must be in 1.." + std::to_string(MMS_REFRESH16_GROUPS);
+    if (!N || !K || !w || !planes || !scale || !inv || !l1 || !count) return "mms_refresh16: bad arguments (null array or count)";
+    if ((addr(count) & 3) != 0) return "mms_refresh16: count must be 4-byte aligned";
+    for (int g = 0; g < groups; g++) {
+        if (N[g] < 0 || K[g] <= 0) return "mms_refresh16: bad shape in a group (N >= 0, K > 0)";
+        if (!w[g] || !planes[g] || !scale[g] || !inv[g] || !l1[g] || ((addr(planes[g]) | addr(inv[g])) & 15) != 0)
+            return "mms_refresh16: null or misaligned pointer in a group (planes and inv 16-byte aligned; l1 is required)";
+    }
+    if (head_w && (!head_tiles || head_A < 1 || head_H < 4 || head_H % 4 != 0 || ((addr(head_w) | addr(head_tiles)) & 15) != 0))
+        return "mms_refresh16: the head needs head_tiles, head_A >= 1, head_H a multiple of 4, both pointers 16-byte aligned";
+    if (nsets < 0 || nsets > MMS_REFRESH16_SETS || (nsets > 0 && !sets)) return "mms_refresh16: nsets must be in 0.." + std::to_string(MMS_REFRESH16_SETS);
+    for (int si = 0; si < nsets; si++) {
+        const mms_refresh16_set& S = sets[si];
+        if (S.nchains < 1 || S.L < 1 || (int64_t)S.nchains * S.L > MMS_REFRESH16_GROUPS || !S.entry || !S.chain || S.rows < 0 ||
+            (S.rows > 0 && (!S.chain_scale || !S.chain_inv || !(S.bound0 >= 0.f))))
+            return "mms_refresh16: bad set (nchains, L >= 1, nchains * L <= " + std::to_string(MMS_REFRESH16_GROUPS) + "; rows > 0 needs chain_scale, chain_inv, bound0 >= 0)";
+        for (int e = 0; e < S.nchains * S.L; e++)
+            if (S.entry[e] < 0 || S.entry[e] >= groups) return "mms_refresh16: a set's entry names no group";
+    }
+    return {};
+}
+
 static inline std::string check_fold_planes16_group(int32_t groups, const int64_t* N, const int32_t* K, const float* const* w, void* const* planes,
                                                     float* const* inv) {
     std::string bad = check_groups("mms_fold_planes16_group", groups);
diff --git a/massive_marl_benchmark_amd/csrc/policy_args.h b/massive_marl_benchmark_amd/csrc/policy_args.h
--- a/massive_marl_benchmark_amd/csrc/policy_args.h
+++ b/massive_marl_benchmark_amd/csrc/policy_args.h
@@ -174,6 +174,33 @@
     int64_t M;
 };
 
+constexpr int kRefreshGroups = 16, kRefreshSets = 4;
+struct Refresh16Args {
+    const float* x[kRefreshGroups];
+    void* planes[kRefreshGroups];
+    float* scale[kRefreshGroups];
+    float* inv[kRefreshGroups];
+    float* l1[kRefreshGroups];
+    const float* bias[kRefreshGroups];
+    int64_t rows_g[kRefreshGroups];
+    int K_g[kRefreshGroups];
+    int groups;
+    const float* head_w;
+    float* head_tiles;
+    int head_A, head_H;
+    int nsets;
+    struct Set {
+        unsigned char entry[kRefreshGroups];
+        int nchains, L;
+        float bound0;
+        int64_t rows;
+        float* chain;
+        float* chain_scale;
+        float* chain_inv;
+    } set[kRefreshSets];
+    unsigned int* count;
+};
+hipError_t launch_refresh16(const Refresh16Args& a, hipStream_t s);
 hipError_t launch_fold_planes16(const FoldPlanesArgs& a, int groups, hipStream_t s);
 hipError_t launch_fold_scales16(const FoldScalesArgs& a, int groups, hipStream_t s);
 hipError_t launch_split16_planes_group(const Split16PlanesArgs& a, int groups, hipStream_t s);
diff --git a/massive_marl_benchmark_amd/csrc/rollout_kernels.hip b/massive_marl_benchmark_amd/csrc/rollout_kernels.hip
--- a/massive_marl_benchmark_amd/csrc/rollout_kernels.hip
+++ b/massive_marl_benchmark_amd/csrc/rollout_kernels.hip
@@ -132,7 +132,7 @@
                                                            const float* __restrict__ log_std, uint64_t seed, int64_t* __restrict__ counters,
                                                            int64_t row_offset, int ref_scale, PpoActOut o, int64_t N, int A) {
     extern __shared__ __attribute__((aligned(16))) float s_part[];
-    ppo_head_block<NCT, WAVES, RT>(s_part, (int)threadIdx.x, true, (int64_t)blockIdx.x * 16 * RT, hidden, weight, bias, H, value, vhidden, vweight, vbias, VH,
+    ppo_head_block<NCT, WAVES, RT, 4, false, false>(s_part, (int)threadIdx.x, true, (int64_t)blockIdx.x * 16 * RT, hidden, weight, bias, H, value, vhidden, vweight, vbias, VH,
                                    log_std, seed, counters, row_offset, ref_scale, o, N, A);
 }
 
diff --git a/massive_marl_benchmark_amd/csrc/split16_kernels.hip b/massive_marl_benchmark_amd/csrc/split16_kernels.hip
--- a/massive_marl_benchmark_amd/csrc/split16_kernels.hip
+++ b/massive_marl_benchmark_amd/csrc/split16_kernels.hip
@@ -46,25 +46,23 @@
     inv = ldexpf(1.f, -sh);
 }
 
+struct Split16Rows {
+    const float* x; uint8_t* out;
+    float* scale; float* inv; float* stat; float* l1;
+    const float* chain; float* chain_scale; float* chain_inv;
+    int64_t rows;
+    int K, pitch, nchains, L;
+    float eps;
+};
 template <bool ALIGNED>
-__global__ void __launch_bounds__(256) split16_planes_kernel(Split16PlanesArgs a, int KC, int P) {
-    const int g = blockIdx.y;
-    const float* __restrict__ x = a.x[g];
-    uint8_t* __restrict__ out = reinterpret_cast<uint8_t*>(a.planes[g]);
+__device__ __forceinline__ void split16_planes_block(const Split16Rows& a, const unsigned bx, const int KC, const int P) {
+    const float* __restrict__ x = a.x;
+    uint8_t* __restrict__ out = a.out;
     const int lane = threadIdx.x & 63;
-    int K = a.K, pitch = a.x_pitch;
-    int64_t rows = a.rows;
-    if (a.per_group) {
-        K = a.K_g[g];
-        pitch = K;
-        rows = a.rows_g[g];
-        KC = (K + 31) / 32;
-        P = 1;
-        while (P < KC * 4 && P < 64) P <<= 1;
-        if (rows == 0) return;
-    }
+    const int K = a.K, pitch = a.pitch;
+    const int64_t rows = a.rows;
     const int sub = lane & (P - 1), rpw = 64 / P;
-    const int64_t row_raw = ((int64_t)blockIdx.x * 4 + (threadIdx.x >> 6)) * rpw + lane / P;
+    const int64_t row_raw = ((int64_t)bx * 4 + (threadIdx.x >> 6)) * rpw + lane / P;
     const bool live = row_raw < rows;
     const int64_t row = live ? row_raw : rows - 1;
     const float* src = x + row * (int64_t)pitch;
@@ -113,26 +111,45 @@
             *reinterpret_cast<f16x8*>(dst + 64) = lo;
         }
     }
-    if (a.stat[g])
+    if (a.stat)
         for (int m = P >> 1; m >= 1; m >>= 1) m2 += __shfl_xor(m2, m, 64);
     if (sub == 0 && live) {
-        if (a.scale[g]) a.scale[g][row] = scale;
-        if (a.inv[g]) a.inv[g][row] = inv;
-        if (a.stat[g]) reinterpret_cast<float2*>(a.stat[g])[row] = make_float2(mean, 1.0f / sqrtf(m2 / (float)K + a.eps));
-        if (a.l1[g]) a.l1[g][row] = asum;
+        if (a.scale) a.scale[row] = scale;
+        if (a.inv) a.inv[row] = inv;
+        if (a.stat) reinterpret_cast<float2*>(a.stat)[row] = make_float2(mean, 1.0f / sqrtf(m2 / (float)K + a.eps));
+        if (a.l1) a.l1[row] = asum;
     }
     if (live)
         for (int c = sub; c < a.nchains; c += P) {
-            const float* ch = a.chain[g] + (size_t)c * a.L * 2;
+            const float* ch = a.chain + (size_t)c * a.L * 2;
             float bound = big;
             for (int l = 0; l < a.L; l++) {
                 bound = (ch[2 * l] * bound + ch[2 * l + 1]) * 1.001f;
                 float sc, iv;
                 pow2_scale(bound, sc, iv);
-                a.chain_scale[g][((size_t)c * a.L + l) * rows + row] = sc;
-                a.chain_inv[g][((size_t)c * a.L + l) * rows + row] = iv;
-            }
-        }
+                a.chain_scale[((size_t)c * a.L + l) * rows + row] = sc;
+                a.chain_inv[((size_t)c * a.L + l) * rows + row] = iv;
+            }
+        }
+}
+__host__ __device__ inline void split16_row_shape(int K, int& KC, int& P) {
+    KC = (K + 31) / 32;
+    P = 1;
+    while (P < KC * 4 && P < 64) P <<= 1;
+}
+template <bool ALIGNED>
+__global__ void __launch_bounds__(256) split16_planes_kernel(Split16PlanesArgs a, int KC, int P) {
+    const int g = blockIdx.y;
+    Split16Rows r = {a.x[g], reinterpret_cast<uint8_t*>(a.planes[g]), a.scale[g], a.inv[g], a.stat[g], a.l1[g], a.chain[g], a.chain_scale[g], a.chain_inv[g],
+                     a.rows, a.K, a.x_pitch, a.nchains, a.L, a.eps};
+    if (a.per_group) {
+        r.K = a.K_g[g];
+        r.pitch = r.K;
+        r.rows = a.rows_g[g];
+        split16_row_shape(r.K, KC, P);
+        if (r.rows == 0) return;
+    }
+    split16_planes_block<ALIGNED>(r, blockIdx.x, KC, P);
 }
 
 hipError_t launch_split16_planes_group(const Split16PlanesArgs& a, int groups, hipStream_t s) {
@@ -203,6 +220,101 @@
     if (a.nchains * a.L == 0) return hipSuccess;
     const unsigned blocks = a.rows > 0 ? (unsigned)((a.rows + 255) / 256) : 1u;
     hipLaunchKernelGGL(chain_refresh16_kernel, dim3(blocks), dim3(256), 0, s, a);
+    return hipGetLastError();
+}
+
+template <bool ALIGNED>
+__global__ void __launch_bounds__(256) refresh16_kernel(Refresh16Args a) {
+    __shared__ float s_chain[2 * kRefreshGroups + 1];
+    const int g = blockIdx.y;
+    if (g < a.groups) {
+        Split16Rows r = {a.x[g], reinterpret_cast<uint8_t*>(a.planes[g]), a.scale[g], a.inv[g], nullptr, a.l1[g], nullptr, nullptr, nullptr,
+                         a.rows_g[g], a.K_g[g], a.K_g[g], 0, 0, 0.f};
+        int KC, P;
+        split16_row_shape(r.K, KC, P);
+        const int64_t rpb = 4 * (64 / P);
+        if (r.rows > 0 && (int64_t)blockIdx.x * rpb < r.rows) split16_planes_block<ALIGNED>(r, blockIdx.x, KC, P);
+    } else {
+        const int H4 = a.head_H / 4, nct = (a.head_A + 15) / 16;
+        const int64_t total4 = (int64_t)nct * H4 * 16;
+        for (int64_t t = (int64_t)blockIdx.x * 256 + threadIdx.x; t < total4; t += (int64_t)gridDim.x * 256) {
+            const int i = (int)(t & 15), kg = (int)((t >> 4) % H4), ct = (int)((t >> 4) / H4);
+            const int j = ct * 16 + i;
+            float4 v = make_float4(0.f, 0.f, 0.f, 0.f);
+            if (j < a.head_A) v = *reinterpret_cast<const float4*>(a.head_w + (size_t)j * a.head_H + 4 * kg);
+            reinterpret_cast<float4*>(a.head_tiles)[t] = v;
+        }
+    }
+    asm volatile("s_waitcnt vmcnt(0)" ::: "memory");
+    __syncthreads();
+    if (threadIdx.x == 0) {
+        __builtin_amdgcn_fence(__ATOMIC_RELEASE, "agent");
+        asm volatile("s_waitcnt vmcnt(0)" ::: "memory");
+        const unsigned total = gridDim.x * gridDim.y;
+        const unsigned ticket = __hip_atomic_fetch_add(a.count, 1u, __ATOMIC_RELAXED, __HIP_MEMORY_SCOPE_AGENT);
+        const bool last = ticket == total - 1;
+        if (last) {
+            __hip_atomic_store(a.count, 0u, __ATOMIC_RELAXED, __HIP_MEMORY_SCOPE_AGENT);
+            __builtin_amdgcn_fence(__ATOMIC_ACQUIRE, "agent");
+            asm volatile("s_waitcnt vmcnt(0)" ::: "memory");
+        }
+        s_chain[2 * kRefreshGroups] = last ? 1.f : 0.f;
+    }
+    __syncthreads();
+    if (s_chain[2 * kRefreshGroups] == 0.f) return;
+    const int lane = threadIdx.x & 63, wave = threadIdx.x >> 6;
+    for (int si = 0; si < a.nsets; si++) {
+        const Refresh16Args::Set& S = a.set[si];
+        const int E = S.nchains * S.L;
+        for (int e = wave; e < E; e += 4) {
+            const int ge = S.entry[e];
+            const float* l1 = a.l1[ge];
+            const float* bias = a.bias[ge];
+            float m = 0.f, b = 0.f;
+            for (int64_t i = lane; i < a.rows_g[ge]; i += 64) {
+                m = fmaxf(m, l1[i]);
+                if (bias) b = fmaxf(b, fabsf(bias[i]));
+            }
+            for (int k = 32; k >= 1; k >>= 1) {
+                m = fmaxf(m, __shfl_xor(m, k, 64));
+                b = fmaxf(b, __shfl_xor(b, k, 64));
+            }
+            if (lane == 0) { s_chain[2 * e] = m; s_chain[2 * e + 1] = b; }
+        }
+        __syncthreads();
+        if ((int)threadIdx.x < 2 * E) S.chain[threadIdx.x] = s_chain[threadIdx.x];
+        for (int c = 0; c < S.nchains && S.rows > 0; c++) {
+            float bound = S.bound0;
+            for (int l = 0; l < S.L; l++) {
+                bound = (s_chain[2 * (c * S.L + l)] * bound + s_chain[2 * (c * S.L + l) + 1]) * 1.001f;
+                float sc, iv;
+                pow2_scale(bound, sc, iv);
+                for (int64_t row = threadIdx.x; row < S.rows; row += 256) {
+                    S.chain_scale[((size_t)c * S.L + l) * S.rows + row] = sc;
+                    S.chain_inv[((size_t)c * S.L + l) * S.rows + row] = iv;
+                }
+            }
+        }
+        __syncthreads();
+    }
+}
+
+hipError_t launch_refresh16(const Refresh16Args& a, hipStream_t s) {
+    bool aligned = true;
+    unsigned blocks = 0;
+    for (int g = 0; g < a.groups; g++) {
+        aligned = aligned && (a.K_g[g] % 4) == 0 && (reinterpret_cast<uintptr_t>(a.x[g]) & 15) == 0;
+        int KCg, Pg;
+        split16_row_shape(a.K_g[g], KCg, Pg);
+        const int64_t rpb = 4 * (64 / Pg);
+        const unsigned need = (unsigned)((a.rows_g[g] + rpb - 1) / rpb);
+        blocks = need > blocks ? need : blocks;
+    }
+    if (blocks == 0) blocks = 1;
+    const dim3 grid(blocks, a.groups + (a.head_w ? 1 : 0));
+    if (grid.y == 0) return hipSuccess;
+    if (aligned) hipLaunchKernelGGL(refresh16_kernel<true>, grid, dim3(256), 0, s, a);
+    else hipLaunchKernelGGL(refresh16_kernel<false>, grid, dim3(256), 0, s, a);
     return hipGetLastError();
 }
 
diff --git a/massive_marl_benchmark_amd/csrc/step_kernels.hip b/massive_marl_benchmark_amd/csrc/step_kernels.hip
--- a/massive_marl_benchmark_amd/csrc/step_kernels.hip
+++ b/massive_marl_benchmark_amd/csrc/step_kernels.hip
@@ -115,27 +115,47 @@
         float* s_head = lds_lanes;
         float* s_head_actions = s_head + 9 * 16 * 80;
         static_assert((9 + 1) * 16 * 80 <= 6 * 4 * BLOCK, "the head's LDS must fit the parking space");
-        if (threadIdx.x >= 512) {
-            const int t = (int)threadIdx.x - 512;
-            const float4* src = reinterpret_cast<const float4*>(a.root_states + (size_t)blockIdx.x * root_floats);
-            for (int i = t; i < root_floats / 4; i += 256) reinterpret_cast<float4*>(s_root)[i] = src[i];
-            for (int i = t; i < (int)(sizeof(mms_config) / 4); i += 256) lds[i] = reinterpret_cast<const float*>(Cg)[i];
-            if (t < 4) s_leg[t] = load_leg_const(&Cg->model, t);
-            constexpr int kStageOff = ((kRedOff + (RP_STRIDE + 6) * AT + 3) & ~3) + ((kObsAT + 3) & ~3);
-            for (int i = t; i < EPB * prev_dim; i += 256) {
-                const int e = i / prev_dim, k = i - e * prev_dim;
-                (lds_envs + (size_t)e * env_stride + kStageOff)[k] = a.prev[((size_t)blockIdx.x * EPB + e) * prev_dim + k];
-            }
-        }
         PpoActOut o{a.head.actions_out, a.head.act_slot, a.head.logp_slot, a.head.value_slot, a.head.mu_slot, a.head.sigma_slot};
         o.lds_actions = s_head_actions;
         o.lds_row0 = (int64_t)blockIdx.x * 16;
+        if (threadIdx.x >= 512) {
+            const int t = (int)threadIdx.x - 512;
+            constexpr int kRootV = EPB * (AT + 1) * 13 / 4, kCfgW = (int)(sizeof(mms_config) / 4), kPrevW = EPB * kPrevAT;
+            constexpr int kRootT = (kRootV + 255) / 256, kCfgT = (kCfgW + 255) / 256, kPrevT = (kPrevW + 255) / 256;
+            constexpr int kStageOff = ((kRedOff + (RP_STRIDE + 6) * AT + 3) & ~3) + ((kObsAT + 3) & ~3);
+            const float4* src = reinterpret_cast<const float4*>(a.root_states + (size_t)blockIdx.x * root_floats);
+            float4 rs[kRootT];
+            float cw[kCfgT], pv[kPrevT];
+#pragma unroll
+            for (int u = 0; u < kRootT; u++) rs[u] = t + 256 * u < kRootV ? src[t + 256 * u] : make_float4(0.f, 0.f, 0.f, 0.f);
+#pragma unroll
+            for (int u = 0; u < kCfgT; u++) cw[u] = t + 256 * u < kCfgW ? reinterpret_cast<const float*>(Cg)[t + 256 * u] : 0.f;
+#pragma unroll
+            for (int u = 0; u < kPrevT; u++) pv[u] = t + 256 * u < kPrevW ? a.prev[(size_t)blockIdx.x * kPrevW + t + 256 * u] : 0.f;
+            const int64_t hrow0 = (int64_t)blockIdx.x * 16 + (t >> 6);
+            PpoNoiseOperands<4, 2> nf;
+            ppo_rows_noise_fetch(nf, a.head.vhidden, a.head.vweight, a.head.VH, a.head.log_std, a.head.counters, hrow0, 4, (int64_t)a.num_envs, 8 * AT, t & 63);
+            if (t < 4) s_leg[t] = load_leg_const(&Cg->model, t);
+#pragma unroll
+            for (int u = 0; u < kRootT; u++)
+                if (t + 256 * u < kRootV) reinterpret_cast<float4*>(s_root)[t + 256 * u] = rs[u];
+#pragma unroll
+            for (int u = 0; u < kCfgT; u++)
+                if (t + 256 * u < kCfgW) lds[t + 256 * u] = cw[u];
+#pragma unroll
+            for (int u = 0; u < kPrevT; u++) {
+                const int i = t + 256 * u, e = i / kPrevAT, k = i - e * kPrevAT;
+                if (i < kPrevW) (lds_envs + (size_t)e * env_stride + kStageOff)[k] = pv[u];
+            }
+            ppo_rows_noise_finish(nf, nullptr, a.head.vhidden, a.head.vweight, a.head.vbias, a.head.VH, a.head.seed, a.head.counters, a.head.row_offset,
+                                  a.head.reference_scale, o, hrow0, 4, (int64_t)a.num_envs, 8 * AT, t & 63, s_head_actions + (t >> 6) * 8 * AT);
+        }
         if (a.head.weight_tiles)
-            ppo_head_block<5, 8, 1, 4, true>(s_head, (int)threadIdx.x, threadIdx.x < 512, (int64_t)blockIdx.x * 16, a.head.hidden, a.head.weight, a.head.bias, a.head.H, nullptr,
+            ppo_head_block<5, 8, 1, 4, true, true>(s_head, (int)threadIdx.x, threadIdx.x < 512, (int64_t)blockIdx.x * 16, a.head.hidden, a.head.weight, a.head.bias, a.head.H, nullptr,
                                              a.head.vhidden, a.head.vweight, a.head.vbias, a.head.VH, a.head.log_std, a.head.seed, a.head.counters, a.head.row_offset,
                                              a.head.reference_scale, o, a.num_envs, 8 * AT, a.head.weight_tiles);
         else
-            ppo_head_block<5, 8, 1, 4>(s_head, (int)threadIdx.x, threadIdx.x < 512, (int64_t)blockIdx.x * 16, a.head.hidden, a.head.weight, a.head.bias, a.head.H, nullptr,
+            ppo_head_block<5, 8, 1, 4, false, true>(s_head, (int)threadIdx.x, threadIdx.x < 512, (int64_t)blockIdx.x * 16, a.head.hidden, a.head.weight, a.head.bias, a.head.H, nullptr,
                                        a.head.vhidden, a.head.vweight, a.head.vbias, a.head.VH, a.head.log_std, a.head.seed, a.head.counters, a.head.row_offset,
                                        a.head.reference_scale, o, a.num_envs, 8 * AT);
         __syncthreads();
```
